# nvaccess/NVSpeechPlayer

Measured on AMD Instinct MI355X. Metric: audio samples/sec (whole node) at 22.05 kHz Klatt synth, batch-N utterances, higher is better.
Workload: dtype f64

## Files before the change

nvspeechplayer_amd/csrc/klatt_batchplan.h:

```cpp
#pragma once

#include <stddef.h>
#include <stdint.h>

#include <algorithm>
#include <numeric>
#include <unordered_map>
#include <utility>
#include <vector>

#include "klatt_consts.h"

namespace klatt {


template <class Meta>
inline bool list_length(const Meta* meta, long long n, uint32_t& length)
{
    unsigned long long len = 0;
    for (long long k = 0; k < n; ++k) {
        const unsigned long long m = meta[k].minSamples, f = meta[k].fadeSamples;
        len += std::max(m, f + 1) + 1;
    }
    length = len >= 0xFFFFFFFFull ? 0u : (uint32_t)len;
    return len < 0xFFFFFFFFull;
}

template <class Meta>
inline unsigned long long list_timing(const Meta* meta, long long n)
{
    unsigned long long h = 0x9E3779B97F4A7C15ull ^ (unsigned long long)n;
    for (long long k = 0; k < n; ++k) {
        h ^= ((unsigned long long)meta[k].minSamples << 32) ^ meta[k].fadeSamples ^ ((unsigned long long)(meta[k].flags & FRAME_NULL) << 63);
        h *= 0xFF51AFD7ED558CCDull; h ^= h >> 29;
    }
    return h;
}

template <class Meta, class Facts>
inline void classify_list(const Meta* meta, const Facts* facts, long long n, uint32_t& flags, unsigned char& shape)
{
    uint32_t fl = 0;
    for (long long k = 0; k < n; ++k)
        if (!(meta[k].flags & FRAME_NULL)) fl |= facts[k].flags;
    const bool finite = !(fl & FACT_NONFINITE), needsNoise = (fl & FACT_NOISE) || !finite;
    flags = (needsNoise ? UTT_NEEDS_NOISE : (!(fl & FACT_NASAL) ? UTT_NO_NASAL : 0u)) | (fl & kUttPresent);
    shape = finite ? (!(fl & FACT_UNBOUNDED) ? 3 : 1) : 0;
}


struct ListTable {
    std::vector<uint32_t> lens;
    std::vector<unsigned long long> timing;
    std::vector<uint32_t> flags;
    std::vector<unsigned char> shape;
    std::vector<uint32_t> weight;
    long long size() const { return (long long)flags.size(); }
    unsigned long long run_key(long long l) const { return timing[(size_t)l] ^ ((unsigned long long)lens[(size_t)l] * 0x9E3779B97F4A7C15ull); }
};

struct RouteOptions {
    int tracks = 1, direct = 1, layout = -1;
    bool fast = false;
    bool sortByLength = true;
    bool noTracks = false;
    int cus = 256;
    long long nFrames = 0;
    bool want_tracks() const { return tracks && !noTracks; }
    bool want_direct() const { return direct && layout != 0 && nFrames > 0 && nFrames < 0xFFFFFFFFll; }
    bool plans() const { return (want_tracks() || want_direct()) && nFrames > 0; }
};

constexpr long long kRunMin = 32;

struct RunShare {
    long long total = 0, inRuns = 0;
    std::unordered_map<unsigned long long, long long> runOf;
};
template <class Pred>
inline RunShare run_share(const ListTable& lists, Pred pred)
{
    RunShare s;
    for (long long l = 0; l < lists.size(); ++l)
        if (pred(l)) { s.total += lists.weight[(size_t)l]; s.runOf[lists.run_key(l)] += lists.weight[(size_t)l]; }
    for (const auto& kv : s.runOf) if (kv.second >= kRunMin) s.inRuns += kv.second;
    return s;
}

using Rerouted = std::vector<std::pair<long long, uint32_t>>;
inline Rerouted reroute_lonely_quiet(ListTable& lists, const RouteOptions& o)
{
    Rerouted rerouted;
    if (!o.plans() || o.layout != -1) return rerouted;
    auto quiet = [&](long long l) { return !(lists.flags[(size_t)l] & UTT_NEEDS_NOISE); };
    const RunShare runs = run_share(lists, quiet);
    if (runs.runOf.size() <= 1) return rerouted;
    for (long long l = 0; l < lists.size(); ++l)
        if (quiet(l) && runs.runOf.at(lists.run_key(l)) < kRunMin) {
            rerouted.emplace_back(l, lists.flags[(size_t)l]);
            lists.flags[(size_t)l] = (lists.flags[(size_t)l] | UTT_NEEDS_NOISE) & ~UTT_NO_NASAL;
        }
    return rerouted;
}

inline std::vector<unsigned char> eligible_lists(const ListTable& lists, const RouteOptions& o)
{
    std::vector<unsigned char> eligible;
    if (!o.plans()) return eligible;
    eligible.assign((size_t)lists.size(), 0);
    for (long long l = 0; l < lists.size(); ++l)
        if ((lists.flags[(size_t)l] & UTT_NEEDS_NOISE) && lists.weight[(size_t)l]) eligible[(size_t)l] = lists.shape[(size_t)l];
    return eligible;
}

inline bool tracks_pay(const ListTable& lists, const unsigned char* eligible, const unsigned char* tracked, unsigned long long trackBytes, const RouteOptions& o)
{
    if (!(o.want_direct() && o.direct == 1 && o.fast && trackBytes > (128ull << 20))) return true;
    long long direct = 0;
    const RunShare runs = run_share(lists, [&](long long l) { return tracked[l] != 0; });
    for (long long l = 0; l < lists.size(); ++l)
        if (tracked[l] && (eligible[l] & 2)) direct += lists.weight[(size_t)l];
    const long long groups = (runs.total + kLanes - 1) / kLanes;
    return !(o.sortByLength && runs.inRuns * 2 <= runs.total && direct == runs.total && groups > o.cus);
}

inline void mark_tracked(ListTable& lists, const unsigned char* tracked, const uint32_t* kinds)
{
    for (long long l = 0; l < lists.size(); ++l)
        if (tracked[l]) lists.flags[(size_t)l] |= UTT_TRACKED | (kinds[l] << kUttKindShift);
}

inline bool route_direct(ListTable& lists, const unsigned char* eligible, const RouteOptions& o)
{
    auto candidate = [&](long long l) { return (eligible[l] & 2) && !(lists.flags[(size_t)l] & UTT_TRACKED); };
    const RunShare runs = run_share(lists, candidate);
    const bool aligned = o.sortByLength && runs.inRuns * 2 > runs.total;
    const bool take = o.direct == 1 ? (!aligned || o.fast) : true;
    if (take)
        for (long long l = 0; l < lists.size(); ++l)
// ... 61 lines not shown
            if (order[(size_t)(w + i)] == kNoUtt) { order[(size_t)(w + i)] = live[(size_t)next]; next = (next + 1) % nLive; }
    }
}

template <class FlagsOf>
inline LanePacking pack_lanes(long long nUtt, FlagsOf flagsOf, const uint32_t* lens, const unsigned long long* timing, bool sortByLength, int width = kLanes)
{
    LanePacking p;
    std::vector<uint32_t>& order = p.order;
    order.resize((size_t)nUtt);
    std::iota(order.begin(), order.end(), 0u);
    auto quietEnd = std::stable_partition(order.begin(), order.end(), [&](uint32_t x) { return !(flagsOf(x) & UTT_NEEDS_NOISE); });
    p.nQuiet = quietEnd - order.begin();
    auto noNasalEnd = std::stable_partition(order.begin(), quietEnd, [&](uint32_t x) { return (flagsOf(x) & UTT_NO_NASAL) != 0; });
    p.nNoNasal = noNasalEnd - order.begin();
    auto trackedEnd = std::stable_partition(quietEnd, order.end(), [&](uint32_t x) { return (flagsOf(x) & UTT_TRACKED) != 0; });
    p.nTrackedUtt = trackedEnd - quietEnd;
    p.nTracked = p.nTrackedUtt;
    auto directEnd = std::stable_partition(trackedEnd, order.end(), [&](uint32_t x) { return (flagsOf(x) & UTT_DIRECT) != 0; });
    p.nDirectSlots = directEnd - trackedEnd;
    const bool untrackedFollow = directEnd != order.end();
    if (sortByLength) {
        auto before = [&](uint32_t x, uint32_t y) { return lens[x] != lens[y] ? lens[x] > lens[y] : timing[x] < timing[y]; };
        std::stable_sort(order.begin(), noNasalEnd, before);
        std::stable_sort(noNasalEnd, quietEnd, before);
        std::stable_sort(quietEnd, trackedEnd, before);
        std::stable_sort(trackedEnd, directEnd, before);
        std::stable_sort(directEnd, order.end(), before);
        const uint32_t* const o = order.data();
        const size_t q = (size_t)p.nQuiet, t = q + (size_t)p.nTrackedUtt, d = t + (size_t)p.nDirectSlots;
        std::vector<uint32_t> tracked, direct(o + t, o + d), untracked;
        pad_runs(o + q, o + t, lens, timing, width, tracked);
        if (!tracked.empty() && t != order.size()) tracked.insert(tracked.end(), lanes_to_boundary(tracked.size(), width), kNoUtt);
        if (!direct.empty() && untrackedFollow) direct.insert(direct.end(), lanes_to_boundary(direct.size(), width), kNoUtt);
        pad_runs(o + d, o + order.size(), lens, timing, width, untracked);
        p.nTracked = (long long)tracked.size();
        p.nDirectSlots = (long long)direct.size();
        order.resize(q);
        order.insert(order.end(), tracked.begin(), tracked.end());
        order.insert(order.end(), direct.begin(), direct.end());
        order.insert(order.end(), untracked.begin(), untracked.end());
    } else if (p.nDirectSlots > 0 && (untrackedFollow || p.nTrackedUtt > 0)) {
        const size_t padT = p.nTrackedUtt > 0 ? lanes_to_boundary((size_t)p.nTrackedUtt, width) : 0;
        order.insert(order.begin() + p.nQuiet + p.nTrackedUtt, padT, kNoUtt);
        p.nTracked = p.nTrackedUtt + (long long)padT;
        if (untrackedFollow) {
            const size_t padD = lanes_to_boundary((size_t)p.nDirectSlots, width);
            order.insert(order.begin() + p.nQuiet + p.nTracked + p.nDirectSlots, padD, kNoUtt);
            p.nDirectSlots += (long long)padD;
        }
    }
    p.nNoNasalSlots = p.nNoNasal + fill_tail(order, 0, p.nNoNasal, width);
    p.nQuietSlots = p.nQuiet + (p.nNoNasalSlots - p.nNoNasal);
    p.nQuietSlots += fill_tail(order, p.nNoNasalSlots, p.nQuietSlots, width);
    const long long noisy = (long long)order.size() - p.nQuietSlots;
    if (noisy % width != 0) {
        const long long ext = width - noisy % width;
        const long long untracked = noisy - p.nTracked - p.nDirectSlots;
        if (untracked <= 0) { if (p.nDirectSlots > 0) p.nDirectSlots += ext; else p.nTracked += ext; }
        order.insert(order.end(), (size_t)ext, kNoUtt);
    }
    fill_sparse_wavefronts(order, p.nQuietSlots, width);
    return p;
}

template <class FlagsOf>
inline void dead_wave_counts(const uint32_t* order, long long first, long long n, FlagsOf flagsOf, int built, long long counts[3], int width = kLanes)
{
    counts[0] = counts[1] = counts[2] = 0;
    for (long long w = first; w < first + n; w += width) {
        uint32_t present = 0;
        bool any = false;
        for (long long s = w; s < std::min(w + width, first + n); ++s)
            if (order[s] != kNoUtt) { present |= flagsOf(order[s]); any = true; }
        if (!any) continue;
        const bool noTurb = !(present & UTT_TURBULENCE), noAsp = noTurb && !(present & UTT_ASPIRATION);
        const int body = ((built & 4) && noAsp) ? 2 : (((built & 2) && noTurb) ? 1 : 0);
        counts[0] += ((built & 1) && !(present & UTT_PARALLEL1)) ? 1 : 0;
        counts[1] += body >= 1 ? 1 : 0;
        counts[2] += body >= 2 ? 1 : 0;
    }
}

}
```

nvspeechplayer_amd/csrc/klatt_consts.h:

```cpp
#pragma once

#include <stdint.h>

namespace klatt {

constexpr int kLanes = 64;

constexpr uint32_t FRAME_NULL = 1u;
constexpr uint32_t UTT_NEEDS_NOISE = 1u;
constexpr uint32_t UTT_NO_NASAL = 2u;
constexpr uint32_t UTT_TRACKED = 4u;
constexpr uint32_t UTT_DIRECT = 8u;
constexpr uint32_t UTT_TURBULENCE = 16u;
constexpr uint32_t UTT_ASPIRATION = 32u;
constexpr uint32_t UTT_PARALLEL1 = 64u;
constexpr uint32_t kUttPresent = UTT_TURBULENCE | UTT_ASPIRATION | UTT_PARALLEL1;
constexpr int kUttKindShift = 8;

constexpr uint32_t FACT_NOISE = 1u;
constexpr uint32_t FACT_NONFINITE = 2u;
constexpr uint32_t FACT_NASAL = 4u;
constexpr uint32_t FACT_UNBOUNDED = 8u;
constexpr uint32_t FACT_TURBULENCE = UTT_TURBULENCE;
constexpr uint32_t FACT_ASPIRATION = UTT_ASPIRATION;
constexpr uint32_t FACT_PARALLEL1 = UTT_PARALLEL1;

}
```

nvspeechplayer_amd/csrc/klatt_device.h:

```cpp
#pragma once

#include <hip/hip_runtime.h>
#include <stdint.h>
#include <type_traits>

#include "klatt_consts.h"
#include "klatt_layout.h"
#include "klatt_math.h"

namespace klatt {

constexpr int kTile = 32;
constexpr int kTileStride = kTile * 2 + 8;
constexpr int kSlots = 45;
constexpr int kBlock = 16;
constexpr int kStateDoubles = 240;

constexpr int MODE_EXACT = 0;
constexpr int MODE_FAST = 1;

constexpr int kTrackStages = 4;
#ifndef KLATT_FLAT_LAYOUT
#define KLATT_FLAT_LAYOUT 2
#endif
__host__ __device__ constexpr uint32_t track_stage_kinds(int s)
{
    return KLATT_FLAT_LAYOUT == 2 ? (s == 0 ? 0xF04003u : s == 1 ? 0x0000FCu : s == 2 ? 0x01B000u : 0x0E0F00u)
                                  : (s == 0 ? 0xF00000u : s == 1 ? 0x00403Fu : s == 2 ? 0x01B0C0u : 0x0E0F00u);
}
__host__ __device__ constexpr uint32_t track_stage_entries(int s)
{
    return KLATT_FLAT_LAYOUT == 2 ? (s == 0 ? 8u : s == 1 ? 6u : s == 2 ? 4u : 7u) : (s == 0 ? 4u : s == 1 ? 8u : s == 2 ? 6u : 7u);
}
constexpr int kTrackAntiStage = KLATT_FLAT_LAYOUT == 2 ? 0 : 1;
__host__ __device__ inline uint32_t track_stage_slots(uint32_t mask, int s) { return (uint32_t)__builtin_popcount(mask & track_stage_kinds(s)) + (s == kTrackAntiStage ? (mask & 1u) : 0u); }
__host__ __device__ inline uint32_t track_part(uint32_t mask, uint32_t F, int s)
{
    uint32_t at = 0;
    for (int k = 0; k < s; ++k) at += track_stage_entries(k) + (F - 1u) * track_stage_slots(mask, k);
    return at;
}

struct DirectHdr {
    uint32_t fadeSamples;
    uint32_t span;
    uint32_t bits;
    uint32_t pad;
};
constexpr uint32_t kDirectBwShift = 8, kDirectClsShift = 14, kDirectAllBits = 0x3FFFFFFu;
constexpr int kDirectStages = 8;
#ifndef KLATT_DIRECT_FAST_LAYOUT
#define KLATT_DIRECT_FAST_LAYOUT 1
#endif
__host__ __device__ constexpr int direct_layout(int mode) { return mode == MODE_FAST ? KLATT_DIRECT_FAST_LAYOUT : 0; }
__host__ __device__ constexpr int direct_stage_res(int s, int L = 0)
{
    return L == 1 ? (s < 2 ? 0 : (s == 3 || s == 4) ? 3 : 2) : (s == 0 ? 0 : 2);
}
__host__ __device__ constexpr int direct_stage_gains(int s, int L = 0)
{
    return L == 1 ? (s == 0 ? 1 : s == 1 ? 3 : s == 2 ? 1 : s == 5 ? 2 : s == 6 ? 1 : s == 7 ? 2 : 0)
                  : (s == 0 ? 4 : s == 1 ? 1 : s == 5 ? 2 : s == 6 ? 1 : s == 7 ? 2 : 0);
}
__host__ __device__ constexpr int direct_stage_entries(int s, int L = 0) { return 4 * direct_stage_res(s, L) + 3 * direct_stage_gains(s, L); }
__host__ __device__ constexpr int direct_stage_first(int s, int L = 0) { int at = 0; for (int k = 0; k < s; ++k) at += direct_stage_entries(k, L); return at; }
constexpr int kDirectEntries = direct_stage_first(kDirectStages);
static_assert(direct_stage_first(kDirectStages, 1) == kDirectEntries, "both layouts hold the same kinds");
__host__ __device__ constexpr int direct_stage_kind(int s, int e, int L = 0)
{
    constexpr int k0[kDirectStages][4] = {{20, 21, 22, 23}, {0, 1, 14, -1}, {2, 3, -1, -1}, {4, 5, -1, -1}, {6, 7, -1, -1}, {8, 9, 17, 18}, {10, 11, 19, -1}, {12, 13, 15, 16}};
    constexpr int k1[kDirectStages][4] = {{20, -1, -1, -1}, {21, 22, 23, -1}, {0, 1, 14, -1}, {2, 3, 4, -1}, {5, 6, 7, -1}, {8, 9, 17, 18}, {10, 11, 19, -1}, {12, 13, 15, 16}};
    return L == 1 ? k1[s][e] : k0[s][e];
}

struct KernelArgs {
    const DirectHdr* directHdr;
    const double2* directRec;
    const uint32_t* directFirst;
    uint32_t nDirect;
    const FlatRef* flatRef;
    const SourceRef* sourceRef;
    uint32_t trackBytes;
    const double2* track;
    const double* frames;
    const FrameMeta* meta;
    const UttDesc* utt;
    const uint32_t* order;
    int16_t* pcm;
    UttResult* result;
    double* state;
    double* const* statePtrs;
    const uint32_t* control;
    long long nSlots;
    uint32_t maxSamples;
    uint32_t ringMask;
    int sampleRate;
    double sampleRateF;
    double invSampleRate;
    double negPiOverSr;
    double twoPiOverSr;
    unsigned long long* debug;
    uint32_t* deadWaves;
    uint32_t deadTerms;
};

__device__ constexpr int kResF[kNumRes] = {13, 14, 12, 11, 10, 9, 8, 7, 25, 26, 27, 28, 29, 30};
__device__ constexpr int kResB[kNumRes] = {21, 22, 20, 19, 18, 17, 16, 15, 31, 32, 33, 34, 35, 36};
constexpr int kNumHot = 17;
__device__ constexpr int kHot[kNumHot] = {1, 2, 3, 4, 5, 6, 23, 24, 37, 38, 39, 40, 41, 42, 43, 44, 45};


__device__ __forceinline__ double div_by(double x, double b, double y)
{
    double q = x * y;
    double r = __builtin_fma(-b, q, x);
    return __builtin_fma(r, y, q);
}

__device__ __forceinline__ double frac_toward_zero(double x) { return x - __builtin_trunc(x); }

__device__ __forceinline__ double fade_value(double from, double to, double ratio)
{
    double v = from + ((to - from) * ratio);
    return (to != to) ? from : v;
}

__device__ __forceinline__ uint32_t mix32(uint32_t x)
{
    x ^= x >> 16; x *= 0x7FEB352Du; x ^= x >> 15; x *= 0x846CA68Bu; x ^= x >> 16;
    return x;
}
__device__ __forceinline__ uint32_t noise_key(uint32_t seed) { return mix32(seed ^ 0x9E3779B9u); }
__device__ __forceinline__ uint32_t noise_inc(uint32_t seed) { return (mix32(seed + 0x85EBCA6Bu) << 1) | 1u; }
constexpr uint32_t kNoiseA = 1664525u;
constexpr uint32_t kNoiseA2 = kNoiseA * kNoiseA;
__device__ __forceinline__ uint32_t noise_inc2(uint32_t inc) { return (kNoiseA + 1u) * inc; }
__device__ __forceinline__ uint32_t noise_step(uint32_t s, uint32_t inc) { return s * kNoiseA + inc; }
__device__ __forceinline__ uint32_t noise_step2(uint32_t s, uint32_t inc2) { return s * kNoiseA2 + inc2; }
__device__ __forceinline__ uint32_t noise_first(uint32_t key, uint32_t inc) { return noise_step(key, inc); }
__device__ __forceinline__ double noise_uniform(uint32_t s)
{
    const double r = (double)(s >> 1);
    return __builtin_fma(r, 0x1.00000002p-31, r * 0x1p-93);
}

template <int MODE>
__device__ __forceinline__ double dot3(double a, double x, double b, double y, double c, double z)
{
    if (MODE == MODE_FAST) return __builtin_fma(c, z, __builtin_fma(b, y, a * x));
    return a * x + b * y + c * z;
}

#ifdef KLATT_SIGNAL_F32
typedef float sig_t;
#else
typedef double sig_t;
#endif
template <int MODE>
__device__ __forceinline__ float dot3(float a, float x, float b, float y, float c, float z)
{
    return __builtin_fmaf(c, z, __builtin_fmaf(b, y, a * x));
}
__device__ __forceinline__ float fade_value(float from, float to, float ratio)
{
    float v = from + ((to - from) * ratio);
    return (to != to) ? from : v;
}

struct Coef { double a, b, c; };
enum { COEF_UNREDUCED = 0, COEF_QUADRANT_M1 = 1, COEF_UNKNOWN = 2 };
#ifndef KLATT_COLD_CALL
#define KLATT_COLD_CALL 2
#endif
struct RadCos { double rad, cs; };
#if KLATT_COLD_CALL
__device__ __attribute__((noinline)) RadCos exp_cos_reduced(double ex, double th)
{
    RadCos o;
#if KLATT_COLD_CALL == 1
    if (__builtin_fabs(ex) <= 700.0 && __builtin_fabs(th) <= 1.0e4) { o.rad = fast_exp(ex); o.cs = fast_cos(th); }
    else
#endif
    { o.rad = exp(ex); o.cs = cos(th); }
    return o;
}
#endif
// ... 451 lines not shown
```

nvspeechplayer_amd/csrc/klatt_engine.hip:

```cpp
#include "klatt_device.h"
#include "klatt_systolic.h"
#include "klatt_lanepipe.h"
#include "klatt_tracks.h"
#include "klatt_direct.h"
#include "klatt_plan.h"
#include "klatt_timeline.h"
#include "klatt_align.h"
#include "klatt_source.h"
#include "klatt_response.h"
#include "klatt_stems.h"
#include "klatt_spectrum.h"
#include "klatt_resample.h"
#include "klatt_convolve.h"
#include "klatt_filter.h"
#include "klatt_codec.h"
#include "klatt_lpc.h"
#include "klatt_pitch.h"
#include "klatt_tempo.h"
#include "klatt_mix.h"
#include "klatt_export.h"
#include "klatt_batchplan.h"
#include "klatt_hostpool.h"
#include "klatt_trackplan.h"
#include "klatt_live.h"
// ... 417 lines not shown
    switch (mode) {
    case MODE_EXACT: rc = go(klatt_lanepipe<MODE_EXACT, CH, WPS>); break;
    case MODE_FAST: rc = go(klatt_lanepipe<MODE_FAST, CH, WPS>); break;
    default: set_error("unknown arithmetic mode %d", mode); return -1;
    }
    if (rc) return rc;
    HIP_TRY(hipGetLastError());
    return 0;
}

#ifndef KLATT_NOISY_CH
#define KLATT_NOISY_CH 8
#endif
struct GroupPlan { bool systolic; int chunk; };
GroupPlan plan_group(int layout, bool noisy, long long nUttBatch, long long nNoisyBatch, int cus)
{
    const long long groups = (nUttBatch + kLanes - 1) / kLanes + 1;
    GroupPlan p;
    p.systolic = layout != 0;
    (void)nNoisyBatch;
    p.chunk = noisy ? (groups <= cus ? 16 : 8)
                    : (groups <= cus ? 32 : 16);
    return p;
}

template <bool STREAM, bool NOISE>
int launch(const KernelArgs& a, int mode, long long nWaves, hipStream_t stream)
{
    if (nWaves <= 0) return 0;
    if (nWaves > 0x7FFFFFFF) { set_error("too many wavefronts: %lld", nWaves); return -1; }
    constexpr int ldsBytes = LdsLayout<STREAM>::kBytes;
    auto go = [&](auto kernel) -> int {
        if (ensure_lds_limit(reinterpret_cast<const void*>(kernel), ldsBytes)) return -1;
        hipLaunchKernelGGL(kernel, dim3((unsigned)nWaves), dim3(kLanes), ldsBytes, stream, a);
        return 0;
    };
    int rc;
    switch (mode) {
    case MODE_EXACT: rc = go(klatt_synthesize<MODE_EXACT, STREAM, NOISE>); break;
    case MODE_FAST: rc = go(klatt_synthesize<MODE_FAST, STREAM, NOISE>); break;
    default:
        set_error("unknown arithmetic mode %d", mode);
        return -1;
    }
    if (rc) return rc;
    HIP_TRY(hipGetLastError());
    return 0;
}

int pick_device(int device)
{
    int n = 0;
    hipError_t e = hipGetDeviceCount(&n);
    if (e != hipSuccess || n <= 0) {
        set_error_code(SPEECHPLAYER_ERR_NO_DEVICE);
        set_error("no HIP device available (%s); this engine has no CPU path", e == hipSuccess ? "count 0" : hipGetErrorString(e));
        return -1;
    }
    if (device < 0) {
        const char* env = getenv("SPEECHPLAYER_DEVICE");
        if (env) device = atoi(env);
        else if (hipGetDevice(&device) != hipSuccess) device = 0;
    }
    if (device >= n) { set_error("device %d out of range (%d devices)", device, n); return -1; }
    return device;
}

struct Batch {
    int sampleRate = 0;
    int device = 0;
    int mode = MODE_EXACT;
    int sortByLength = 1;
    int layout = -1;
    int cus = 256;
    hipStream_t stream = nullptr;
    int tracks = 1;
    long long trackBudgetMB = 4096;
    hipStream_t side[6] = {nullptr, nullptr, nullptr, nullptr, nullptr, nullptr};
    hipEvent_t forkEvent = nullptr, join[6] = {nullptr, nullptr, nullptr, nullptr, nullptr, nullptr};
    int quietLast = 1;
    int deadTerms = 1;
    DeviceBuffer<uint32_t> dDeadWaves;
    long long planDeadWaves[3] = {0, 0, 0};
    long long nUtt = 0, nFrames = 0, nSlots = 0;
    long long nLists = 0, nFramesSpoken = 0;
    std::vector<long long> uttFrameStart;
    std::vector<uint32_t> uttFrames;
    bool launched = false;
    long long nQuiet = 0;
    long long nTracked = 0;
    long long nTrackedUtt = 0;
    long long nJobs = 0, trackEntries = 0;
    int directLean = -1;
    bool directAligned = false;
    int direct = 1;
    long long nDirect = 0;
    long long nDirectUtt = 0, nDirectFrames = 0;
    long long nNoNasal = 0;
    long long nNoNasalUtt = 0;
    long long totalSamples = 0, poolSamples = 0;
    std::vector<uint32_t> lens;
    std::vector<uint32_t> uttSeed;
    std::vector<long long> outStart;
    std::vector<UttResult> results;
    bool resultsFresh = false;
    DeviceBuffer<double> dFrames;
    DeviceBuffer<FrameMeta> dMeta;
    DeviceBuffer<UttDesc> dUtt;
    DeviceBuffer<uint32_t> dOrder;
    DeviceBuffer<int16_t> dPcm;
    DeviceBuffer<UttResult> dResult;
    DeviceBuffer<FlatRef> dFlatRef;
    DeviceBuffer<SourceRef> dSourceRef;
    DeviceBuffer<TrackJob> dJobs;
    DeviceBuffer<double> dShapes;
    DeviceBuffer<double2> dTrack;
    DeviceBuffer<DirectJob> dDirectJobs;
    DeviceBuffer<uint32_t> dDirectFirst;
    DeviceBuffer<DirectHdr> dDirectHdr;
    DeviceBuffer<double2> dDirectRec;
    DeviceBuffer<unsigned long long> dDebug;
    DeviceBuffer<float> dFloat;
    DeviceBuffer<unsigned long long> dDigest;
    PinnedPair bounce;
    DeviceBuffer<FrameRecord> dRecords;
    DeviceBuffer<double> dShapeTable;
    DeviceBuffer<uint32_t> dRep;
    DeviceBuffer<unsigned long long> dMismatch;
    DeviceBuffer<FrameFacts> dFacts;
    PinnedBlock hFacts;
    DeviceBuffer<int16_t> dDense;
    DeviceBuffer<long long> dDenseStart;
    std::vector<long long> denseStart;
    hipStream_t copyStream = nullptr;
    hipEvent_t denseReady = nullptr, copyDone = nullptr;
    bool copyPending = false;
    bool floatFresh = false;
    hipEvent_t inputReady = nullptr;
    DeviceBuffer<long long> dShapeIdx;
    DeviceBuffer<double> dShapeRows;
    hipEvent_t pcmReady = nullptr;
    struct ExportSlot { PinnedBlock host; DeviceBuffer<unsigned char> dev; hipEvent_t done = nullptr; bool used = false; };
    static constexpr int kExportSlots = 16;
    ExportSlot exportSlot[kExportSlots];
    unsigned exportNext = 0;
    struct SharedTable {
        hipEvent_t done = nullptr;
        bool used = false;
        int wait(hipStream_t st) { if (used) HIP_TRY(hipStreamWaitEvent(st, done, 0)); return 0; }
        int mark(hipStream_t st) { HIP_TRY(hipEventRecord(done, st)); used = true; return 0; }
    };
    std::vector<uint32_t> uttList;
    DeviceBuffer<long long> dListStart;
    DeviceBuffer<TimelineReq> dTimeline;
    hipEvent_t setDone = nullptr, setCopied = nullptr, timelineReady = nullptr;
    bool timelineFresh = false;
    ExportSlot trackSlot[kExportSlots];
    unsigned trackNext = 0;
    DeviceBuffer<double> dPitch;
    SharedTable pitchOrder;
    long long pitchBudgetMB = 256;
    DeviceBuffer<FrameLabel> dLabels;
    DeviceBuffer<uint32_t> dUnitFirst;
    std::vector<uint32_t> listUnits;
    bool hasLabels = false;
    DeviceBuffer<double> dSource;
// ... 181 lines not shown
constexpr bool kTimingOnlyBuild = false;
#endif
bool refuse_timing_only(const char* what)
{
    if (!kTimingOnlyBuild || getenv("SPEECHPLAYER_ALLOW_TIMING_ONLY_PCM")) return false;
    set_error_code(SPEECHPLAYER_ERR_ARGUMENT);
    set_error("%s: this library was built with a timing-only experiment switch; its PCM is not valid", what);
    return true;
}

long long tracked_count(const Batch* b) { return (b->tracks && b->layout != 0) ? b->nTracked : 0; }
long long direct_count(const Batch* b) { return b->nDirect; }
bool direct_lean(const Batch* b, long long nGroups)
{
    if (b->directLean >= 0) return b->directLean != 0;
    if (b->directAligned) return false;
    return b->mode == MODE_FAST ? true : nGroups > 2ll * b->cus;
}

int batch_launch(Batch* b)
{
    KernelArgs a = base_args(b->sampleRate);
    a.frames = b->dFrames.ptr; a.meta = b->dMeta.ptr; a.utt = b->dUtt.ptr;
    a.pcm = b->dPcm.ptr; a.result = b->dResult.ptr; a.state = nullptr; a.control = nullptr;
    if (wait_exports(b)) return -1;
    b->resultsFresh = false;
    b->floatFresh = false;
    b->launched = true;
#ifdef KLATT_STAMPS
    if (b->dDebug.reserve((size_t)(b->nSlots / kLpUPG + 2) * 32 * 2)) return -1;
    HIP_TRY(hipMemsetAsync(b->dDebug.ptr, 0, b->dDebug.cap * 8, b->stream));
    a.debug = b->dDebug.ptr;
#endif
    const long long nLp = lanepipe_count(b);
    const bool laneKernel = b->layout == 0;
    const long long nTr = tracked_count(b);
    const long long nDir = direct_count(b);
    const long long nNoisyHead = b->nTracked - nTr;
    const long long nNoisy = b->nSlots - b->nQuiet - b->nTracked - nDir;
    const long long nNn = laneKernel ? 0 : b->nNoNasal - nLp;
    const long long nQ = b->nQuiet - nLp - nNn;
    const int parts = (nLp > 0) + (nNn > 0) + (nQ > 0) + (nNoisy > 0) + (nNoisyHead > 0) + (nTr > 0) + (nDir > 0);
    const bool fork = parts > 1;
    if (fork) HIP_TRY(hipEventRecord(b->forkEvent, b->stream));
    int sideUsed = 0, seen = 0;
    auto next_stream = [&](bool = false) -> hipStream_t {
        if (!fork || ++seen == parts) return b->stream;
        hipStream_t st = b->side[sideUsed++];
        (void)hipStreamWaitEvent(st, b->forkEvent, 0);
        return st;
    };
    const GroupPlan plq = plan_group(b->layout, false, b->nSlots, nNoisy, b->cus);
    auto launch_quiet = [&]() -> int {
    if (nLp > 0) {
        hipStream_t st = next_stream(true);
        a.order = b->dOrder.ptr; a.nSlots = nLp;
        const long long g = (nLp + kLpUPG - 1) / kLpUPG;
        if (g <= b->cus ? launch_lanepipe<KLATT_LP_CH, 1>(a, b->mode, g, st) : launch_lanepipe<16, 2>(a, b->mode, g, st)) return -1;
    }
    if (nNn > 0) {
        hipStream_t st = next_stream(true);
        a.order = b->dOrder.ptr + nLp; a.nSlots = nNn;
        const long long g = (nNn + kLanes - 1) / kLanes;
        if (plq.chunk == 32 ? launch_systolic<false, 32, 1, false>(a, b->mode, g, st) : launch_systolic<false, 16, 2, false>(a, b->mode, g, st)) return -1;
    }
    if (nQ > 0) {
        hipStream_t st = next_stream(true);
        a.order = b->dOrder.ptr + nLp + nNn; a.nSlots = nQ;
        const long long g = (nQ + kLanes - 1) / kLanes;
        if (plq.systolic ? (plq.chunk == 32 ? launch_systolic<false, 32>(a, b->mode, g, st) : launch_systolic<false, 16>(a, b->mode, g, st))
                         : launch<false, false>(a, b->mode, g, st)) return -1;
    }
        return 0;
    };
    const bool quietLast = b->quietLast && (nTr > 0 || nDir > 0) && nNoisy == 0 && nNoisyHead == 0;
    if (!quietLast && launch_quiet()) return -1;
    if (nTr > 0) {
        hipStream_t st = next_stream();
        TrackArgs t;
        t.jobs = b->dJobs.ptr; t.nJobs = b->nJobs; t.shapes = b->dShapes.ptr; t.track = b->dTrack.ptr;
        t.negPiOverSr = a.negPiOverSr; t.twoPiOverSr = a.twoPiOverSr;
        const long long tg = b->nJobs;
        if (tg > 0x7FFFFFFF) { set_error("too many tracks: %lld", b->nJobs); return -1; }
        if (b->dDeadWaves.reserve(3)) return -1;
        HIP_TRY(hipMemsetAsync(b->dDeadWaves.ptr, 0, 3 * sizeof(uint32_t), st));
        hipLaunchKernelGGL(klatt_tracks, dim3((unsigned)tg), dim3(kLanes * kTrackWaves), 0, st, t);
        HIP_TRY(hipGetLastError());
        a.order = b->dOrder.ptr + b->nQuiet; a.nSlots = nTr;
        a.flatRef = b->dFlatRef.ptr; a.sourceRef = b->dSourceRef.ptr; a.track = b->dTrack.ptr;
        a.trackBytes = (uint32_t)std::min<unsigned long long>(((unsigned long long)b->trackEntries + kTrackPad) * sizeof(double2), 0xFFFFFFFFull);
        a.deadWaves = b->dDeadWaves.ptr; a.deadTerms = b->deadTerms ? kUttPresent : 0u;
        const GroupPlan pl = plan_group(b->layout, true, b->nSlots, nTr + nNoisy, b->cus);
        const long long g = (nTr + kLanes - 1) / kLanes;
        if (pl.chunk == 8 ? launch_systolic<true, KLATT_FLAT_CH, KLATT_FLAT_WPS, true, false, true>(a, b->mode, g, st)
                          : launch_systolic<true, 16, 1, true, false, true>(a, b->mode, g, st)) return -1;
        a.flatRef = nullptr; a.sourceRef = nullptr; a.track = nullptr; a.deadWaves = nullptr; a.deadTerms = 0u;
    }
    if (nDir > 0) {
        hipStream_t st = next_stream();
        SeedArgs sa;
        sa.jobs = b->dDirectJobs.ptr; sa.nJobs = (uint32_t)b->nDirectFrames; sa.frames = b->dFrames.ptr; sa.meta = b->dMeta.ptr;
        sa.hdr = b->dDirectHdr.ptr; sa.rec = b->dDirectRec.ptr; sa.negPiOverSr = a.negPiOverSr; sa.twoPiOverSr = a.twoPiOverSr;
        const dim3 sg((unsigned)((b->nDirectFrames + 255) / 256), (unsigned)kDirectStages);
        constexpr int kSeedLds = 14 * 257 * (int)sizeof(double2);
        if (b->mode == MODE_FAST) hipLaunchKernelGGL(klatt_seeds<MODE_FAST>, sg, dim3(256), kSeedLds, st, sa);
        else hipLaunchKernelGGL(klatt_seeds<MODE_EXACT>, sg, dim3(256), kSeedLds, st, sa);
        HIP_TRY(hipGetLastError());
        a.order = b->dOrder.ptr + b->nQuiet + b->nTracked; a.nSlots = nDir;
        a.directHdr = b->dDirectHdr.ptr; a.directRec = b->dDirectRec.ptr; a.directFirst = b->dDirectFirst.ptr; a.nDirect = (uint32_t)b->nDirectFrames;
        a.sourceRef = b->dSourceRef.ptr;
        const long long g = (nDir + kLanes - 1) / kLanes;
        if (launch_direct(a, b->mode, direct_lean(b, g), g, st)) return -1;
        a.directHdr = nullptr; a.directRec = nullptr; a.directFirst = nullptr; a.nDirect = 0; a.sourceRef = nullptr;
    }
    for (int half = 0; half < 2; ++half) {
        const long long n = half ? nNoisy : nNoisyHead;
        if (n <= 0) continue;
        hipStream_t st = next_stream();
        a.order = b->dOrder.ptr + b->nQuiet + (half ? b->nTracked + nDir : 0); a.nSlots = n;
        const GroupPlan pl = plan_group(b->layout, true, b->nSlots, nTr + nNoisy + nNoisyHead, b->cus);
        const long long g = (n + kLanes - 1) / kLanes;
        if (pl.systolic ? (pl.chunk == 8 ? launch_systolic<true, KLATT_NOISY_CH, 2>(a, b->mode, g, st) : launch_systolic<true, 16>(a, b->mode, g, st))
                        : launch<false, true>(a, b->mode, g, st)) return -1;
    }
    if (quietLast && launch_quiet()) return -1;
    for (int i = 0; i < sideUsed; ++i) {
        HIP_TRY(hipEventRecord(b->join[i], b->side[i]));
        HIP_TRY(hipStreamWaitEvent(b->stream, b->join[i], 0));
    }
    return 0;
}

constexpr size_t kLogEntries = 40960;
constexpr size_t kLogEager = 2560;

struct LogEntry {
    double p[kNumParams];
    FrameMeta meta;
    uint32_t target;
    uint32_t pad;
};
static_assert(sizeof(LogEntry) == 400, "LogEntry layout");

__global__ void __launch_bounds__(256) live_scatter(const LogEntry* __restrict__ log, uint32_t n, double* __restrict__ ringFrames,
                                                    FrameMeta* __restrict__ ringMeta)
{
    const uint32_t e = blockIdx.x * 4u + (threadIdx.x >> 6), j = threadIdx.x & 63u;
    if (e >= n) return;
    const uint32_t at = log[e].target;
    if (at == kNoTarget) return;
    if (j < (uint32_t)kNumParams) ringFrames[(size_t)at * kNumParams + j] = log[e].p[j];
    else if (j == (uint32_t)kNumParams) ringMeta[at] = log[e].meta;
}

struct LivePlace {
    FrameMeta meta;
    long long row;
    uint32_t target;
    uint32_t pad;
};
static_assert(sizeof(LivePlace) == 32, "LivePlace layout");

__global__ void __launch_bounds__(256) live_place(const double* __restrict__ frames, const LivePlace* __restrict__ place, long long n,
                                                  double* __restrict__ ringFrames, FrameMeta* __restrict__ ringMeta)
{
    const uint32_t j = threadIdx.x & 63u;
    const long long step = (long long)gridDim.x * 4;
    for (long long e = (long long)blockIdx.x * 4 + (threadIdx.x >> 6); e < n; e += step) {
        const LivePlace p = place[e];
        if (j < (uint32_t)kNumParams) ringFrames[(size_t)p.target * kNumParams + j] = p.row < 0 ? 0.0 : frames[p.row * kNumParams + j];
        else if (j == (uint32_t)kNumParams) ringMeta[p.target] = p.meta;
    }
}

struct Stream {
    int sampleRate = 0;
    int device = 0;
    int mode = MODE_EXACT;
    uint32_t seed = 0;
// ... 858 lines not shown
    begin_call();
    QueueCall q;
    q.what = "speechPlayer_queueFramesManyDevice"; q.handles = handles; q.n = nHandles; q.frameStart = frameStart; q.frames = deviceFrames;
    q.onDevice = true; q.minDur = minFrameDuration; q.fadeDur = fadeDuration; q.userIndex = userIndex; q.isNull = isNull; q.purge = purge;
    q.readyStream = static_cast<hipStream_t>(readyStream);
    return queue_frames(q);
}

int speechPlayer_handleDevice(speechPlayer_handle_t handle)
{
    begin_call();
    Stream* s = lookup(handle);
    if (!s) { set_error("speechPlayer_handleDevice: invalid handle"); return -1; }
    return s->device;
}

speechPlayer_batch_t speechPlayer_batch_create(int sampleRate, int device)
{
    begin_call();
    int dev = pick_device(device);
    if (dev < 0) return nullptr;
    Batch* b = new Batch;
    b->sampleRate = sampleRate;
    b->device = dev;
    { hipDeviceProp_t prop; if (hipGetDeviceProperties(&prop, dev) == hipSuccess && prop.multiProcessorCount > 0) b->cus = prop.multiProcessorCount; }
    bool ok = hipSetDevice(dev) == hipSuccess && hipStreamCreateWithFlags(&b->stream, hipStreamNonBlocking) == hipSuccess &&
              hipEventCreateWithFlags(&b->forkEvent, hipEventDisableTiming) == hipSuccess &&
              hipStreamCreateWithFlags(&b->copyStream, hipStreamNonBlocking) == hipSuccess &&
              hipEventCreateWithFlags(&b->denseReady, hipEventDisableTiming) == hipSuccess &&
              hipEventCreateWithFlags(&b->copyDone, hipEventDisableTiming) == hipSuccess &&
              hipEventCreateWithFlags(&b->inputReady, hipEventDisableTiming) == hipSuccess &&
              hipEventCreateWithFlags(&b->pcmReady, hipEventDisableTiming) == hipSuccess;
    for (auto& s : b->exportSlot) ok = ok && hipEventCreateWithFlags(&s.done, hipEventDisableTiming) == hipSuccess;
    for (auto& s : b->trackSlot) ok = ok && hipEventCreateWithFlags(&s.done, hipEventDisableTiming) == hipSuccess;
    for (hipEvent_t* e : {&b->setDone, &b->setCopied, &b->timelineReady, &b->pitchOrder.done, &b->sourceOrder.done, &b->resampleOrder.done, &b->bankOrder.done}) ok = ok && hipEventCreateWithFlags(e, hipEventDisableTiming) == hipSuccess;
    { const char* e = getenv("SPEECHPLAYER_TRACKS"); if (e) b->tracks = atoi(e) ? 1 : 0; }
    { const char* e = getenv("SPEECHPLAYER_DIRECT"); if (e) b->direct = std::min(2, std::max(0, atoi(e))); }
    { const char* e = getenv("SPEECHPLAYER_DIRECT_LEAN"); if (e) b->directLean = std::min(1, std::max(-1, atoi(e))); }
    for (int i = 0; i < 6 && ok; ++i)
        ok = hipStreamCreateWithFlags(&b->side[i], hipStreamNonBlocking) == hipSuccess &&
             hipEventCreateWithFlags(&b->join[i], hipEventDisableTiming) == hipSuccess;
    { const char* e = getenv("SPEECHPLAYER_QUIET_LAST"); if (e) b->quietLast = atoi(e) ? 1 : 0; }
    if (!ok) {
        set_error("cannot create a stream on device %d", dev);
        speechPlayer_batch_destroy(b);
        return nullptr;
    }
    return b;
}

void speechPlayer_batch_destroy(speechPlayer_batch_t batch)
{
    Batch* b = static_cast<Batch*>(batch);
    if (!b) return;
    (void)hipSetDevice(b->device);
    (void)sync_exports(b);
    for (auto& s : b->exportSlot) {
        if (s.done) (void)hipEventDestroy(s.done);
        s.host.release(); s.dev.release();
    }
    (void)settle_track_exports(b, true);
    for (auto& s : b->trackSlot) {
        if (s.done) (void)hipEventDestroy(s.done);
        s.host.release(); s.dev.release();
    }
    for (hipEvent_t e : {b->setDone, b->setCopied, b->timelineReady, b->pitchOrder.done, b->sourceOrder.done, b->resampleOrder.done, b->bankOrder.done}) if (e) (void)hipEventDestroy(e);
    b->dListStart.release(); b->dTimeline.release(); b->dPitch.release(); b->dLabels.release(); b->dUnitFirst.release();
    b->dSource.release(); b->dEpochs.release(); b->dEpochCount.release(); b->dResample.release(); b->dBank.release();
    if (b->inputReady) (void)hipEventDestroy(b->inputReady);
    if (b->pcmReady) (void)hipEventDestroy(b->pcmReady);
    b->dShapeIdx.release(); b->dShapeRows.release();
    if (b->stream) { (void)hipStreamSynchronize(b->stream); (void)hipStreamDestroy(b->stream); }
    for (int i = 0; i < 6; ++i) {
        if (b->side[i]) { (void)hipStreamSynchronize(b->side[i]); (void)hipStreamDestroy(b->side[i]); }
        if (b->join[i]) (void)hipEventDestroy(b->join[i]);
    }
    if (b->forkEvent) (void)hipEventDestroy(b->forkEvent);
    if (b->copyStream) { (void)hipStreamSynchronize(b->copyStream); (void)hipStreamDestroy(b->copyStream); }
    if (b->denseReady) (void)hipEventDestroy(b->denseReady);
    if (b->copyDone) (void)hipEventDestroy(b->copyDone);
    b->dDense.release(); b->dDenseStart.release(); b->dFacts.release(); b->hFacts.release();
    b->dRecords.release(); b->dShapeTable.release(); b->dRep.release(); b->dMismatch.release();
    b->dFrames.release(); b->dMeta.release(); b->dUtt.release(); b->dOrder.release(); b->dPcm.release(); b->dResult.release();
    b->dFloat.release(); b->dDebug.release(); b->dDigest.release(); b->bounce.release(); b->dDeadWaves.release();
    b->dFlatRef.release(); b->dSourceRef.release(); b->dJobs.release(); b->dShapes.release(); b->dTrack.release();
    b->dDirectJobs.release(); b->dDirectFirst.release(); b->dDirectHdr.release(); b->dDirectRec.release();
    delete b;
}

int speechPlayer_batch_setOption(speechPlayer_batch_t batch, const char* name, int value)
{
    begin_call();
    Batch* b = static_cast<Batch*>(batch);
    if (!b || !name) return -1;
    if (!strcmp(name, "mode")) {
        if (value != MODE_EXACT && value != MODE_FAST) { set_error("mode %d not available", value); return -1; }
        b->mode = value;
        return 0;
    }
    if (!strcmp(name, "sort")) { b->sortByLength = value ? 1 : 0; return 0; }
    if (!strcmp(name, "quiet_last")) { b->quietLast = value ? 1 : 0; return 0; }
    if (!strcmp(name, "layout")) { b->layout = value < 0 ? -1 : (value > 2 ? 1 : value); return 0; }
    if (!strcmp(name, "tracks")) { b->tracks = value ? 1 : 0; return 0; }
    if (!strcmp(name, "dead_terms")) { b->deadTerms = value ? 1 : 0; return 0; }
    if (!strcmp(name, "track_budget_mb")) { b->trackBudgetMB = value < 0 ? 0 : value; return 0; }
    if (!strcmp(name, "direct")) { b->direct = value < 0 ? 0 : (value > 2 ? 2 : value); return 0; }
    if (!strcmp(name, "direct_lean")) { b->directLean = value < 0 ? -1 : (value ? 1 : 0); return 0; }
    if (!strcmp(name, "pitch_table_mb")) { b->pitchBudgetMB = value < 1 ? 1 : value; return 0; }
    if (!strcmp(name, "source_table_mb")) { b->sourceBudgetMB = value < 1 ? 1 : value; return 0; }
    if (!strcmp(name, "source_lane_lists")) { b->sourceLaneLists = value < 1 ? 1 : value; return 0; }
    set_error("unknown option %s", name);
    return -1;
}

struct SetInput {
    long long nLists = 0;
    const long long* listStart = nullptr;
    const speechPlayer_frame_t* frames = nullptr;
    const unsigned int* minDur = nullptr;
    const unsigned int* fadeDur = nullptr;
    const int* userIndex = nullptr;
    const unsigned char* isNull = nullptr;
    const speechPlayer_frameRecord_t* records = nullptr;
    long long nShapes = 0;
    const speechPlayer_frame_t* shapes = nullptr;
    long long nUtt = 0;
    const unsigned int* listOf = nullptr;
    const unsigned int* seeds = nullptr;
    const double* deviceFrames = nullptr;
    hipStream_t readyStream = nullptr;
    const speechPlayer_frameLabel_t* labels = nullptr;
    bool noTracks = false;
};
static_assert(sizeof(speechPlayer_frameRecord_t) == sizeof(FrameRecord), "record layout");
static_assert(sizeof(speechPlayer_frameLabel_t) == sizeof(FrameLabel), "label layout");
static_assert(SPEECHPLAYER_LABEL_GAP == kLabelGap && SPEECHPLAYER_LABEL_PUFF == kLabelPuff && SPEECHPLAYER_ALIGN_COLUMNS == kAlignColumns &&
              SPEECHPLAYER_UNIT_COLUMNS == kUnitColumns, "alignment constants");

static void batch_clear(Batch* b)
{
    b->nUtt = 0; b->nFrames = 0; b->nFramesSpoken = 0; b->nLists = 0; b->nSlots = 0; b->nQuiet = 0; b->nNoNasal = 0; b->nNoNasalUtt = 0; b->totalSamples = 0; b->poolSamples = 0;
    b->nTracked = 0; b->nTrackedUtt = 0; b->nJobs = 0; b->trackEntries = 0; b->nDirect = 0; b->nDirectUtt = 0; b->nDirectFrames = 0; b->directAligned = false;
    b->lens.clear(); b->outStart.assign(1, 0); b->results.clear(); b->resultsFresh = false; b->floatFresh = false;
    b->uttFrameStart.clear(); b->uttFrames.clear(); b->uttList.clear(); b->uttSeed.clear(); b->timelineFresh = false; b->epochFresh = false;
    b->hasLabels = false; b->listUnits.clear();
}

static int batch_set(Batch* b, const SetInput& in);

static int batch_set_guarded(const char* what, speechPlayer_batch_t batch, const SetInput& in)
{
    begin_call();
    try {
        return batch_set(static_cast<Batch*>(batch), in);
    } catch (const std::exception& e) {
        set_error("%s: %s", what, e.what());
        return -1;
    }
}

int speechPlayer_batch_setUtterances(speechPlayer_batch_t batch, long long nUtterances, const long long* frameStart,
                                     const speechPlayer_frame_t* frames, const unsigned int* minFrameDuration,
                                     const unsigned int* fadeDuration, const int* userIndex, const unsigned char* isNull,
                                     const unsigned int* noiseSeed)
{
    SetInput in;
    in.nLists = nUtterances; in.listStart = frameStart; in.frames = frames; in.minDur = minFrameDuration; in.fadeDur = fadeDuration;
// ... 84 lines not shown
                                          const unsigned int* noiseSeed)
{
    return batch_set_records(labels ? "setRecordsLabelled" : "setRecords", batch, nShapes, shapes, nLists, listStart, records, labels, nUtterances, listOf, noiseSeed);
}

int speechPlayer_batch_hasLabels(speechPlayer_batch_t batch) { return batch ? (static_cast<Batch*>(batch)->hasLabels ? 1 : 0) : -1; }

static int device_shape_table(Batch* b, long long nL, const long long* listStart, const FrameMeta* meta, const FrameFacts* facts,
                              const unsigned char* eligible, HashMask mask, RawVector<uint32_t>& rowOf, std::vector<long long>& rep, std::vector<double>& rows)
{
    shape_table_rows(nL, listStart, meta, facts, eligible, mask, rowOf, rep);
    const size_t nRows = rep.size();
    rows.assign(nRows * kNumParams, 0.0);
    if (nRows == 0) return 0;
    if (b->dShapeIdx.reserve(nRows) || b->dShapeRows.reserve(nRows * kNumParams)) return -1;
    HIP_TRY(hipMemcpyAsync(b->dShapeIdx.ptr, rep.data(), nRows * sizeof(long long), hipMemcpyHostToDevice, b->copyStream));
    const unsigned grid = (unsigned)std::min<long long>(((long long)nRows * kNumParams + 255) / 256, 1 << 16);
    hipLaunchKernelGGL(klatt_gather_frames, dim3(grid), dim3(256), 0, b->copyStream, b->dFrames.ptr, b->dShapeIdx.ptr, (long long)nRows, b->dShapeRows.ptr);
    HIP_TRY(hipGetLastError());
    HIP_TRY(hipMemcpyAsync(rows.data(), b->dShapeRows.ptr, nRows * kNumParams * sizeof(double), hipMemcpyDeviceToHost, b->copyStream));
    HIP_TRY(hipStreamSynchronize(b->copyStream));
    return 0;
}

struct FirstBad {
    std::atomic<long long> at{-1};
    void mark(long long i) { long long none = -1; at.compare_exchange_strong(none, i); }
    long long get() const { return at.load(); }
};

constexpr long long kScratchKeepFrames = 4000000;
struct SetScratch {
    RawVector<FrameMeta> meta;
    RawVector<FlatRef> flatRef;
    RawVector<DirectJob> directJobs;
    RawVector<FrameFacts> facts;
};
static SetScratch& set_scratch()
{
    static thread_local SetScratch scratch;
    return scratch;
}

struct SetCall {
    Batch* const b;
    const SetInput& in;
    const long long nL, nU;
    const long long* const listStart;
    const bool byRecords, byDevice;
    long long nF = 0;
    const std::chrono::steady_clock::time_point tSet = std::chrono::steady_clock::now();

    SetScratch& scratch = set_scratch();
    struct ScratchRelease {
        SetScratch& s;
        long long nF = 0;
        ~ScratchRelease()
        {
            if (nF > kScratchKeepFrames) {
                RawVector<FrameMeta>().swap(s.meta); RawVector<FlatRef>().swap(s.flatRef); RawVector<FrameFacts>().swap(s.facts);
                RawVector<DirectJob>().swap(s.directJobs);
            }
        }
    } scratchRelease{scratch};
    std::vector<uint32_t> unitFirst, listUnits;
    bool framesPinned = false, earlyStarted = false;
    int earlyRc = 0;
    std::string earlyErr;
    struct CopyGuard { Batch* b; bool armed = false; ~CopyGuard() { if (armed) (void)hipStreamSynchronize(b->copyStream); } } copyGuard{b};
    std::thread early;
    struct JoinEarly { std::thread& t; ~JoinEarly() { if (t.joinable()) t.join(); } } joinEarly{early};
    const FrameFacts* facts = nullptr;
    bool factsOnDevice = false;
    ListTable lists;
    RouteOptions route;
    std::vector<uint32_t> lens;
    std::vector<long long> outStart, denseStart;
    long long total = 0, pool = 0, spoken = 0;
    TrackPlan plan;
    std::vector<uint32_t> directFirst;
    long long nDirectUtt = 0;
    bool directAligned = false;
    std::vector<UttDesc> utt;
    std::vector<long long> uttFrameStart;
    std::vector<uint32_t> uttFrames, uttList, uttSeed;
    LanePacking lanes;
    bool verify = false;
    unsigned long long mismatchAt = ~0ull;

    SetCall(Batch* b_, const SetInput& in_)
        : b(b_), in(in_), nL(in_.nLists), nU(in_.nUtt), listStart(in_.listStart), byRecords(in_.records != nullptr), byDevice(in_.deviceFrames != nullptr) {}
    long long list_of(long long u) const { return in.listOf ? (long long)in.listOf[u] : u; }
    void lap(const char* what) const
    {
        static const bool setTrace = getenv("SPEECHPLAYER_SET_TRACE") != nullptr;
        if (setTrace) fprintf(stderr, "[speechPlayer/set] %s: %.1f ms since the start\n", what, std::chrono::duration<double, std::milli>(std::chrono::steady_clock::now() - tSet).count());
    }
};

static int set_validate(SetCall& c)
{
    const SetInput& in = c.in;
    const long long nL = c.nL, nU = c.nU;
    const long long* const listStart = c.listStart;
    if (listStart[0] != 0) { set_error("set: frameStart[0] must be 0"); return -1; }
    for (long long l = 0; l < nL; ++l)
        if (listStart[l + 1] < listStart[l]) { set_error("set: frameStart not monotone at %lld", l); return -1; }
    const long long nF = c.nF = listStart[nL];
    if (nF > 0 && !c.byRecords && ((!in.frames && !c.byDevice) || !in.minDur || !in.fadeDur)) { set_error("set: bad frame arrays"); return -1; }
    if (in.listOf) {
        FirstBad bad;
        parallel_ranges(nU, 1 << 16, [&](long long a, long long e) {
            for (long long u = a; u < e; ++u) if ((long long)in.listOf[u] >= nL) bad.mark(u);
        });
        if (bad.get() >= 0) { set_error("set: listOf[%lld] is not a list", bad.get()); return -1; }
    }
    if (c.byRecords) {
        FirstBad bad;
        parallel_ranges(nF, 1 << 16, [&](long long a, long long e) {
            for (long long k = a; k < e; ++k)
                if (in.records[k].shape != SPEECHPLAYER_RECORD_SILENCE && (long long)in.records[k].shape >= in.nShapes) bad.mark(k);
        });
        if (bad.get() >= 0) { set_error("setRecords: record %lld names shape %u of %lld", bad.get(), in.records[bad.get()].shape, in.nShapes); return -1; }
    }
    if (in.labels) {
        if (nF >= 0xFFFFFFFFll) { set_error("setRecordsLabelled: too many frames"); return -1; }
        c.unitFirst.resize((size_t)(nF + nL)); c.listUnits.assign((size_t)nL, 0);
        FirstBad bad;
        parallel_ranges(nL, 256, [&](long long la, long long le) {
            for (long long l = la; l < le; ++l) {
                uint32_t* uf = c.unitFirst.data() + listStart[l] + l;
                int units = 0;
                for (long long k = listStart[l]; k < listStart[l + 1]; ++k) {
                    const int u = in.labels[k].unit;
                    if (in.labels[k].phoneme < 0 || (u != units && !(units > 0 && u == units - 1))) { bad.mark(k); break; }
                    if (u == units) uf[units++] = (uint32_t)(k - listStart[l]);
                }
                uf[units] = (uint32_t)(listStart[l + 1] - listStart[l]);
                c.listUnits[(size_t)l] = (uint32_t)units;
            }
        });
        if (bad.get() >= 0) {
            set_error("setRecordsLabelled: label %lld (phoneme %d, unit %d): the units of a list count from 0 and rise by at most one, ids are not negative",
                      bad.get(), in.labels[bad.get()].phoneme, in.labels[bad.get()].unit);
            return -1;
        }
    }
    return 0;
}

static int set_meta_words(SetCall& c)
{
    const SetInput& in = c.in;
    const long long nL = c.nL, nF = c.nF;
    const long long* const listStart = c.listStart;
    c.scratchRelease.nF = nF;
    RawVector<FrameMeta>& meta = c.scratch.meta;
    meta.resize((size_t)nF);
    parallel_ranges(nF, 1 << 16, [&](long long a, long long e) {
        if (c.byRecords)
            for (long long k = a; k < e; ++k) {
                const speechPlayer_frameRecord_t& r = in.records[k];
                meta[k].minSamples = r.minFrameDuration;
                meta[k].fadeSamples = std::max(r.fadeDuration, 1u);
                meta[k].userIndex = r.userIndex;
                meta[k].flags = r.shape == SPEECHPLAYER_RECORD_SILENCE ? FRAME_NULL : 0u;
            }
        else
            for (long long k = a; k < e; ++k) {
                meta[k].minSamples = in.minDur[k];
                meta[k].fadeSamples = std::max(in.fadeDur[k], 1u);
                meta[k].userIndex = in.userIndex ? in.userIndex[k] : -1;
                meta[k].flags = (in.isNull && in.isNull[k]) ? FRAME_NULL : 0u;
            }
    });
    c.lists.lens.assign((size_t)nL, 0);
    FirstBad tooLong;
    parallel_ranges(nL, 4096, [&](long long la, long long le) {
        for (long long l = la; l < le; ++l)
            if (!list_length(meta.data() + listStart[l], listStart[l + 1] - listStart[l], c.lists.lens[(size_t)l])) tooLong.mark(l);
    });
    if (tooLong.get() >= 0) { set_error("utterance (frame list %lld) too long (4294967295 samples or more)", tooLong.get()); return -1; }
    return 0;
}

static int set_start_frames(SetCall& c)
{
    Batch* const b = c.b;
    const SetInput& in = c.in;
    const long long nL = c.nL, nF = c.nF;
    c.framesPinned = !c.byRecords && nF > 0 && is_pinned(in.frames);
    {
        const bool grows = (size_t)nF * kNumParams > b->dFrames.cap || (size_t)nF > b->dMeta.cap || (size_t)nL + 1 > b->dListStart.cap ||
                           (in.labels && ((size_t)nF > b->dLabels.cap || (size_t)(nF + nL) > b->dUnitFirst.cap));
        const bool unordered = !c.byRecords && !c.byDevice && !c.framesPinned;
        if (settle_track_exports(b, grows || unordered)) return -1;
    }
    if (c.byRecords) {
        if (b->dFrames.reserve(std::max<size_t>((size_t)nF * kNumParams, 1)) || b->dMeta.reserve(std::max<size_t>((size_t)nF, 1)) ||
            b->dRecords.reserve(std::max<size_t>((size_t)nF, 1)) || b->dShapeTable.reserve(std::max<size_t>((size_t)in.nShapes * kNumParams, 1))) { batch_clear(b); return -1; }
        batch_clear(b);
        c.copyGuard.armed = true;
        if (in.nShapes) HIP_TRY(hipMemcpyAsync(b->dShapeTable.ptr, in.shapes, (size_t)in.nShapes * sizeof(speechPlayer_frame_t), hipMemcpyHostToDevice, b->copyStream));
        if (nF) {
            HIP_TRY(hipMemcpyAsync(b->dRecords.ptr, in.records, (size_t)nF * sizeof(FrameRecord), hipMemcpyHostToDevice, b->copyStream));
            const unsigned grid = (unsigned)std::min<long long>((nF + 63) / 64, 8192);
            hipLaunchKernelGGL(klatt_expand_frames, dim3(grid), dim3(256), 0, b->copyStream, b->dRecords.ptr, b->dShapeTable.ptr, b->dFrames.ptr, b->dMeta.ptr, nF);
            HIP_TRY(hipGetLastError());
        }
        c.earlyStarted = true;
    } else if (c.byDevice && nF > 0) {
        if (in.readyStream) {
            HIP_TRY(hipEventRecord(b->inputReady, in.readyStream));
            HIP_TRY(hipStreamWaitEvent(b->copyStream, b->inputReady, 0));
        }
        if (b->dFrames.reserve((size_t)nF * kNumParams)) { batch_clear(b); return -1; }
        batch_clear(b);
        c.copyGuard.armed = true;
        HIP_TRY(hipMemcpyAsync(b->dFrames.ptr, in.deviceFrames, (size_t)nF * kNumParams * sizeof(double), hipMemcpyDeviceToDevice, b->copyStream));
        c.earlyStarted = true;
    } else if (nF > 0 && (c.framesPinned || (size_t)nF * kNumParams * sizeof(double) >= (32u << 20))) {
        if (b->dFrames.reserve((size_t)nF * kNumParams)) { batch_clear(b); return -1; }
        batch_clear(b);
        if (c.framesPinned) {
            c.copyGuard.armed = true;
            HIP_TRY(hipMemcpyAsync(b->dFrames.ptr, in.frames, (size_t)nF * kNumParams * sizeof(double), hipMemcpyHostToDevice, b->copyStream));
            c.earlyStarted = true;
        } else
        try {
            c.early = std::thread([&c, frames = in.frames, nF, dev = b->device, dst = b->dFrames.ptr]() {
                hipError_t e = hipSetDevice(dev);
                if (e == hipSuccess) e = hipMemcpy(dst, frames, (size_t)nF * kNumParams * sizeof(double), hipMemcpyHostToDevice);
                if (e != hipSuccess) { c.earlyRc = -1; c.earlyErr = hipGetErrorString(e); }
            });
            c.earlyStarted = true;
        } catch (const std::system_error&) {}
    }
    return 0;
}

static int set_frame_facts(SetCall& c)
{
    Batch* const b = c.b;
    const SetInput& in = c.in;
    const long long nF = c.nF;
    const double maxBwDirect = 690.0 * b->sampleRate / M_PI, maxFDirect = 9900.0 * b->sampleRate / (2.0 * M_PI);
    c.factsOnDevice = (c.framesPinned || c.byDevice) && c.earlyStarted;
    RawVector<FrameFacts>& fv = c.scratch.facts;
    if (c.byRecords) {
        std::vector<uint32_t> shapeFl((size_t)in.nShapes);
        for (long long s = 0; s < in.nShapes; ++s) shapeFl[(size_t)s] = shape_flags(reinterpret_cast<const double*>(in.shapes + s), maxFDirect, maxBwDirect);
        fv.resize((size_t)nF);
        parallel_ranges(nF, 1 << 15, [&](long long a, long long e) {
            for (long long k = a; k < e; ++k) {
                const speechPlayer_frameRecord_t& r = in.records[k];
                FrameFacts f;
                f.h0 = r.shape; f.h1 = ~0ull; f.pad = 0;
                f.flags = r.shape == SPEECHPLAYER_RECORD_SILENCE ? 0u : (shapeFl[r.shape] | pitch_flags(r.voicePitch, r.endVoicePitch));
                fv[k] = f;
            }
        });
        c.facts = fv.data();
    } else if (c.factsOnDevice) {
        if (b->dFacts.reserve((size_t)nF) || b->hFacts.ensure((size_t)nF * sizeof(FrameFacts))) return -1;
        const unsigned grid = (unsigned)std::min<long long>((nF + 255) / 256, 1 << 16);
        hipLaunchKernelGGL(klatt_frame_facts, dim3(grid), dim3(256), 0, b->copyStream, b->dFrames.ptr, b->dFacts.ptr, nF, maxFDirect, maxBwDirect);
        HIP_TRY(hipGetLastError());
        HIP_TRY(hipMemcpyAsync(b->hFacts.ptr, b->dFacts.ptr, (size_t)nF * sizeof(FrameFacts), hipMemcpyDeviceToHost, b->copyStream));
        c.facts = static_cast<const FrameFacts*>(b->hFacts.ptr);
    } else if (nF > 0) {
        fv.resize((size_t)nF);
        parallel_ranges(nF, 1 << 13, [&](long long a, long long e) {
            for (long long k = a; k < e; ++k) fv[k] = frame_facts(reinterpret_cast<const double*>(in.frames + k), maxFDirect, maxBwDirect);
        });
        c.facts = fv.data();
    }
    return 0;
}

static int set_plan(SetCall& c)
{
    Batch* const b = c.b;
    const SetInput& in = c.in;
    const long long nL = c.nL, nU = c.nU, nF = c.nF;
    const long long* const listStart = c.listStart;
    const FrameMeta* const meta = c.scratch.meta.data();
    ListTable& lists = c.lists;
    c.lens.assign((size_t)nU, 0);
    c.outStart.assign((size_t)nU + 1, 0);
    c.denseStart.resize((size_t)nU + 1);
    for (long long u = 0; u < nU; ++u) {
        const long long l = c.list_of(u);
        c.lens[u] = lists.lens[l];
        c.outStart[u] = c.pool;
        c.denseStart[u] = c.total;
        c.total += (long long)c.lens[u];
        c.pool += ((long long)c.lens[u] + kTile - 1) / kTile * kTile;
        c.spoken += listStart[l + 1] - listStart[l];
    }
    c.outStart[nU] = c.pool;
    c.denseStart[nU] = c.total;
    lists.weight.assign((size_t)nL, in.listOf ? 0u : 1u);
    if (in.listOf) for (long long u = 0; u < nU; ++u) ++lists.weight[in.listOf[u]];
    c.lap("meta, lengths, frame facts started");
    lists.timing.resize((size_t)nL);
    parallel_ranges(nL, 4096, [&](long long la, long long le) {
        for (long long l = la; l < le; ++l) lists.timing[l] = list_timing(meta + listStart[l], listStart[l + 1] - listStart[l]);
    });
    if (c.factsOnDevice) HIP_TRY(hipStreamSynchronize(b->copyStream));
    const FrameFacts* const facts = c.facts;
    lists.shape.assign((size_t)nL, 0);
    lists.flags.assign((size_t)nL, 0);
    parallel_ranges(nL, 4096, [&](long long la, long long le) {
        for (long long l = la; l < le; ++l)
            classify_list(meta + listStart[l], facts + listStart[l], listStart[l + 1] - listStart[l], lists.flags[l], lists.shape[l]);
    });
    c.lap("classification");
    RouteOptions& route = c.route;
    route.tracks = b->tracks; route.direct = b->direct; route.layout = b->layout;
    route.fast = b->mode == MODE_FAST; route.sortByLength = b->sortByLength != 0; route.noTracks = in.noTracks;
    route.cus = b->cus; route.nFrames = nF;
    const Rerouted rerouted = reroute_lonely_quiet(lists, route);
    c.lap("timing hashes, quiet runs");
    const std::vector<unsigned char> eligible = eligible_lists(lists, route);
    c.lap("eligibility");
    TrackPlan& plan = c.plan;
    FrameSource source{in.frames, in.records, in.shapes};
    RawVector<uint32_t> rowOf;
    std::vector<long long> shapeRep;
    std::vector<double> shapeRows;
    const bool wantTracks = route.want_tracks() && nF > 0;
    const HashMask hashMask = plan_hash_mask();
    if (wantTracks && c.byDevice) {
        if (device_shape_table(b, nL, listStart, meta, facts, eligible.data(), hashMask, rowOf, shapeRep, shapeRows)) return -1;
        source.shapes = reinterpret_cast<const speechPlayer_frame_t*>(shapeRows.data());
        source.rowOf = rowOf.data();
        c.lap("shape table");
    }
    if (wantTracks) {
        plan_tracks(nL, listStart, source, facts, meta, eligible.data(), track_budget_entries(b->trackBudgetMB), hashMask, plan);
        if (source.rowOf && !plan.rep.empty()) {
            parallel_ranges(nL, 4096, [&](long long la, long long le) {
                for (long long l = la; l < le; ++l) {
                    if (!eligible[l]) continue;
                    for (long long k = listStart[l]; k < listStart[l + 1]; ++k) {
                        if (meta[k].flags & FRAME_NULL) continue;
                        const long long r = shapeRep[rowOf[k]];
                        plan.rep[k] = r == k ? 0xFFFFFFFFu : (uint32_t)r;
                    }
                }
            });
        }
        c.lap("tracks planned");
        if (tracks_pay(lists, eligible.data(), plan.tracked.data(), plan.entries * sizeof(double2), route)) mark_tracked(lists, plan.tracked.data(), plan.kinds.data());
        else { plan.jobs.clear(); plan.entries = 0; plan.tracked.assign((size_t)nL, 0); }
    }
    if (route.want_direct()) c.directAligned = route_direct(lists, eligible.data(), route);
    restore_rerouted(lists, rerouted);
    return 0;
}

static void set_direct_jobs_and_refs(SetCall& c)
{
    const long long nL = c.nL, nU = c.nU, nF = c.nF;
    const long long* const listStart = c.listStart;
    const RawVector<FrameMeta>& meta = c.scratch.meta;
    const TrackPlan& plan = c.plan;
    RawVector<DirectJob>& directJobs = c.scratch.directJobs;
    directJobs.clear();
    if (c.route.want_direct()) {
        std::vector<uint32_t> directFirstL((size_t)nL, 0u);
        for (long long l = 0; l < nL; ++l) {
            if (!(c.lists.flags[l] & UTT_DIRECT)) continue;
            c.nDirectUtt += c.lists.weight[l];
            directFirstL[l] = (uint32_t)directJobs.size();
            walk_fade_ends(listStart[l], listStart[l + 1], meta.data(), directJobs);
        }
        c.directFirst.resize((size_t)nU);
        parallel_ranges(nU, 1 << 16, [&](long long a, long long e) { for (long long u = a; u < e; ++u) c.directFirst[u] = directFirstL[c.list_of(u)]; });
    }
    RawVector<FlatRef>& flatRef = c.scratch.flatRef;
    if (!plan.jobs.empty()) {
        flatRef.resize((size_t)nF);
        parallel_ranges(nF, 1 << 16, [&](long long ka, long long ke) {
        for (long long k = ka; k < ke; ++k) {
            const unsigned long long m = meta[k].minSamples, f = meta[k].fadeSamples;
            flatRef[k] = FlatRef{(uint32_t)plan.ref[k].off, plan.ref[k].mask, meta[k].fadeSamples, (uint32_t)std::min<unsigned long long>(std::max(m, f + 1) + 1, 0xFFFFFFFFull)};
        }
        });
    }
    c.lap("direct jobs, flat / source references");
}

static void set_lanes(SetCall& c)
{
    const SetInput& in = c.in;
    const long long nU = c.nU;
    const long long* const listStart = c.listStart;
    c.utt.resize((size_t)nU); c.uttFrameStart.resize((size_t)nU); c.uttFrames.resize((size_t)nU); c.uttList.resize((size_t)nU); c.uttSeed.resize((size_t)nU);
    parallel_ranges(nU, 1 << 15, [&](long long a, long long e) {
        for (long long u = a; u < e; ++u) {
            const long long l = c.list_of(u);
            UttDesc d;
            d.frameStart = listStart[l];
            d.outStart = c.outStart[u];
            d.nFrames = (uint32_t)(listStart[l + 1] - listStart[l]);
            d.seed = in.seeds ? in.seeds[u] : (uint32_t)u;
            d.flags = c.lists.flags[l];
            d.length = c.lists.lens[l];
            c.utt[u] = d;
            c.uttFrameStart[u] = d.frameStart; c.uttFrames[u] = d.nFrames; c.uttList[u] = (uint32_t)l; c.uttSeed[u] = d.seed;
        }
    });
    std::vector<unsigned long long> timing;
    if (in.listOf) { timing.resize((size_t)nU); for (long long u = 0; u < nU; ++u) timing[u] = c.lists.timing[in.listOf[u]]; }
    else timing.swap(c.lists.timing);
    c.lanes = pack_lanes(nU, [&](uint32_t u) { return c.utt[u].flags; }, c.lens.data(), timing.data(), c.b->sortByLength != 0);
    c.lap("lane packing");
}

static int set_upload(SetCall& c)
{
    Batch* const b = c.b;
    const SetInput& in = c.in;
    const long long nL = c.nL, nU = c.nU, nF = c.nF, pool = c.pool, nSlotsAll = (long long)c.lanes.order.size();
    const long long nTrackedUtt = c.lanes.nTrackedUtt, nDirectUtt = c.nDirectUtt;
    const TrackPlan& plan = c.plan;
    const RawVector<DirectJob>& directJobs = c.scratch.directJobs;
    if ((size_t)pool > b->dPcm.cap && sync_exports(b)) return -1;
    if (b->dFrames.reserve(std::max<size_t>((size_t)nF * kNumParams, 1)) || b->dMeta.reserve(std::max<size_t>(nF, 1)) ||
        b->dUtt.reserve(std::max<size_t>(nU, 1)) || b->dOrder.reserve(std::max<size_t>(nSlotsAll, 1)) ||
        b->dResult.reserve(std::max<size_t>(nU, 1)) || b->dPcm.reserve(std::max<size_t>(pool, 1)) || b->dListStart.reserve((size_t)nL + 1))
        return -1;
    HIP_TRY(hipMemcpyAsync(b->dListStart.ptr, c.listStart, ((size_t)nL + 1) * sizeof(long long), hipMemcpyHostToDevice, b->stream));
    if (nTrackedUtt > 0) {
        if (b->dFlatRef.reserve((size_t)nF) || b->dJobs.reserve(plan.jobs.size()) || b->dShapes.reserve(plan.shapes.size()) ||
            b->dTrack.reserve((size_t)plan.entries + kTrackPad)) return -1;
        HIP_TRY(hipMemcpyAsync(b->dShapes.ptr, plan.shapes.data(), plan.shapes.size() * sizeof(double), hipMemcpyHostToDevice, b->stream));
        HIP_TRY(hipMemcpyAsync(b->dFlatRef.ptr, c.scratch.flatRef.data(), (size_t)nF * sizeof(FlatRef), hipMemcpyHostToDevice, b->stream));
        HIP_TRY(hipMemcpyAsync(b->dJobs.ptr, plan.jobs.data(), plan.jobs.size() * sizeof(TrackJob), hipMemcpyHostToDevice, b->stream));
    }
    if (nTrackedUtt > 0 || nDirectUtt > 0) {
        if (b->dSourceRef.reserve((size_t)nF)) return -1;
    }
    if (nDirectUtt > 0) {
        const size_t nD = directJobs.size();
        if (b->dDirectJobs.reserve(nD) || b->dDirectFirst.reserve((size_t)nU) || b->dDirectHdr.reserve((size_t)kDirectStages * nD) ||
            b->dDirectRec.reserve((size_t)kDirectEntries * nD)) return -1;
        HIP_TRY(hipMemcpyAsync(b->dDirectJobs.ptr, directJobs.data(), nD * sizeof(DirectJob), hipMemcpyHostToDevice, b->stream));
        HIP_TRY(hipMemcpyAsync(b->dDirectFirst.ptr, c.directFirst.data(), (size_t)nU * sizeof(uint32_t), hipMemcpyHostToDevice, b->stream));
    }
    if (nF) {
        if (!c.earlyStarted) HIP_TRY(hipMemcpyAsync(b->dFrames.ptr, in.frames, (size_t)nF * kNumParams * sizeof(double), hipMemcpyHostToDevice, b->stream));
        if (!c.byRecords) HIP_TRY(hipMemcpyAsync(b->dMeta.ptr, c.scratch.meta.data(), (size_t)nF * sizeof(FrameMeta), hipMemcpyHostToDevice, b->stream));
    }
    if (nU) {
        HIP_TRY(hipMemcpyAsync(b->dUtt.ptr, c.utt.data(), (size_t)nU * sizeof(UttDesc), hipMemcpyHostToDevice, b->stream));
        HIP_TRY(hipMemcpyAsync(b->dOrder.ptr, c.lanes.order.data(), (size_t)nSlotsAll * sizeof(uint32_t), hipMemcpyHostToDevice, b->stream));
        HIP_TRY(hipMemsetAsync(b->dResult.ptr, 0, (size_t)nU * sizeof(UttResult), b->stream));
        if (b->dDenseStart.reserve((size_t)nU + 1)) return -1;
        HIP_TRY(hipMemcpyAsync(b->dDenseStart.ptr, c.denseStart.data(), ((size_t)nU + 1) * sizeof(long long), hipMemcpyHostToDevice, b->stream));
    }
    if (c.verify) {
        if (b->dRep.reserve((size_t)nF) || b->dMismatch.reserve(1)) return -1;
        HIP_TRY(hipMemcpyAsync(b->dRep.ptr, plan.rep.data(), (size_t)nF * sizeof(uint32_t), hipMemcpyHostToDevice, b->stream));
        HIP_TRY(hipMemsetAsync(b->dMismatch.ptr, 0xFF, sizeof(unsigned long long), b->stream));
    }
    if (in.labels) {
        if (b->dLabels.reserve(std::max<size_t>((size_t)nF, 1)) || b->dUnitFirst.reserve(std::max<size_t>((size_t)(nF + nL), 1))) return -1;
        c.copyGuard.armed = true;
        if (nF) HIP_TRY(hipMemcpyAsync(b->dLabels.ptr, in.labels, (size_t)nF * sizeof(FrameLabel), hipMemcpyHostToDevice, b->copyStream));
        if (nF + nL) HIP_TRY(hipMemcpyAsync(b->dUnitFirst.ptr, c.unitFirst.data(), (size_t)(nF + nL) * sizeof(uint32_t), hipMemcpyHostToDevice, b->copyStream));
    }
    HIP_TRY(hipStreamSynchronize(b->stream));
    if (c.copyGuard.armed) { HIP_TRY(hipStreamSynchronize(b->copyStream)); c.copyGuard.armed = false; }
    if (c.early.joinable()) c.early.join();
    if (c.earlyRc) { set_error_code(SPEECHPLAYER_ERR_HIP); set_error("set: uploading the frames failed: %s", c.earlyErr.c_str()); return -1; }
    const unsigned grid = (unsigned)std::min<long long>((nF + 255) / 256, 1 << 16);
    if (c.verify) {
        hipLaunchKernelGGL(klatt_verify_shared, dim3(grid), dim3(256), 0, b->stream, b->dFrames.ptr, b->dRep.ptr, nF, b->dMismatch.ptr);
        HIP_TRY(hipGetLastError());
        HIP_TRY(hipMemcpyAsync(&c.mismatchAt, b->dMismatch.ptr, sizeof c.mismatchAt, hipMemcpyDeviceToHost, b->stream));
    }
    if (nTrackedUtt > 0 || nDirectUtt > 0) {
        hipLaunchKernelGGL(klatt_source_refs, dim3(grid), dim3(256), 0, b->stream, b->dFrames.ptr, b->dMeta.ptr, b->dSourceRef.ptr, nF);
        HIP_TRY(hipGetLastError());
    }
    if (c.verify || nTrackedUtt > 0 || nDirectUtt > 0) HIP_TRY(hipStreamSynchronize(b->stream));
    return 0;
}

static int set_commit(SetCall& c)
{
    Batch* const b = c.b;
    const LanePacking& lanes = c.lanes;
    b->hasLabels = c.in.labels != nullptr;
    b->listUnits.swap(c.listUnits);
    b->nUtt = c.nU; b->nFrames = c.nF; b->nFramesSpoken = c.spoken; b->nLists = c.nL; b->nSlots = (long long)lanes.order.size();
    b->nNoNasalUtt = lanes.nNoNasal;
    b->nQuiet = lanes.nQuietSlots; b->nNoNasal = lanes.nNoNasalSlots;
    b->nTracked = lanes.nTrackedUtt > 0 ? lanes.nTracked : 0; b->nTrackedUtt = lanes.nTrackedUtt;
    dead_wave_counts(lanes.order.data(), lanes.nQuietSlots, b->nTracked, [&](uint32_t u) { return c.utt[u].flags; }, KLATT_DEAD_TERMS, b->planDeadWaves);
    b->nJobs = lanes.nTrackedUtt > 0 ? (long long)c.plan.jobs.size() : 0; b->trackEntries = lanes.nTrackedUtt > 0 ? (long long)c.plan.entries : 0;
    b->nDirect = c.nDirectUtt > 0 ? lanes.nDirectSlots : 0; b->nDirectUtt = c.nDirectUtt; b->nDirectFrames = (long long)c.scratch.directJobs.size();
    b->directAligned = c.nDirectUtt > 0 && c.directAligned;
    b->totalSamples = c.total; b->poolSamples = c.pool;
    b->lens.swap(c.lens); b->outStart.swap(c.outStart); b->denseStart.swap(c.denseStart);
    b->uttFrameStart.swap(c.uttFrameStart); b->uttFrames.swap(c.uttFrames); b->uttList.swap(c.uttList); b->uttSeed.swap(c.uttSeed);
    b->timelineFresh = false; b->epochFresh = false;
    HIP_TRY(hipEventRecord(b->setDone, b->stream));
    HIP_TRY(hipEventRecord(b->setCopied, b->copyStream));
    b->results.clear();
    b->resultsFresh = false;
    b->floatFresh = false;
    b->launched = false;
    return 0;
}

static int batch_set(Batch* b, const SetInput& in)
{
    if (!b || in.nLists < 0 || in.nUtt < 0 || !in.listStart) { set_error("set: bad arguments"); return -1; }
    if (in.nUtt >= 0xFFFFFFFFll || in.nLists >= 0xFFFFFFFFll) { set_error("set: too many utterances"); return -1; }
    if (!in.listOf && in.nUtt != in.nLists) { set_error("set: %lld utterances for %lld lists and no listOf", in.nUtt, in.nLists); return -1; }
    SetCall c(b, in);
    HIP_TRY(hipSetDevice(b->device));
    if (set_validate(c) || set_meta_words(c)) return -1;
    if (set_start_frames(c) || set_frame_facts(c) || set_plan(c)) return -1;
    set_direct_jobs_and_refs(c);
    set_lanes(c);
    c.verify = !c.byRecords && c.lanes.nTrackedUtt > 0 && !c.plan.rep.empty();
    if (set_upload(c)) {
        batch_clear(b);
        return -1;
    }
    c.lap("uploads");
    if (c.verify && c.mismatchAt != ~0ull) {
        const unsigned long long k = c.mismatchAt;
        if (c.early.joinable()) c.early.join();
        SetInput again = in;
        again.noTracks = true;
        const uint32_t first = c.plan.rep[(size_t)k];
        const int rc = batch_set(b, again);
        if (rc == 0) {
            set_error("set: frames %llu and %u carry one 128-bit shape hash and different values; the batch runs without tracks", k, first);
            set_error_code(SPEECHPLAYER_OK);
        }
        return rc;
    }
    return set_commit(c);
}

long long speechPlayer_batch_frames(speechPlayer_batch_t batch, long long u, speechPlayer_frame_t* frames, unsigned int* minFrameDuration,
                                    unsigned int* fadeDuration, int* userIndex, unsigned char* isNull, long long capacity)
{
    begin_call();
    Batch* b = static_cast<Batch*>(batch);
    if (!b || u < 0 || u >= b->nUtt) { set_error("batch_frames: no such utterance"); return -1; }
    HIP_TRY(hipSetDevice(b->device));
    const long long n = b->uttFrames[(size_t)u], k0 = b->uttFrameStart[(size_t)u];
    if (n > capacity || n == 0) return n;
    if (frames) HIP_TRY(hipMemcpy(frames, b->dFrames.ptr + k0 * kNumParams, (size_t)n * sizeof(speechPlayer_frame_t), hipMemcpyDeviceToHost));
    if (minFrameDuration || fadeDuration || userIndex || isNull) {
        std::vector<FrameMeta> m((size_t)n);
        HIP_TRY(hipMemcpy(m.data(), b->dMeta.ptr + k0, (size_t)n * sizeof(FrameMeta), hipMemcpyDeviceToHost));
        for (long long k = 0; k < n; ++k) {
            if (minFrameDuration) minFrameDuration[k] = m[(size_t)k].minSamples;
            if (fadeDuration) fadeDuration[k] = m[(size_t)k].fadeSamples;
            if (userIndex) userIndex[k] = m[(size_t)k].userIndex;
            if (isNull) isNull[k] = (m[(size_t)k].flags & FRAME_NULL) ? 1 : 0;
        }
    }
    return n;
}

long long speechPlayer_batch_utteranceSamples(speechPlayer_batch_t batch, long long u)
{
    Batch* b = static_cast<Batch*>(batch);
    if (!b || u < 0 || u >= b->nUtt) return -1;
    return b->lens[u];
}
long long speechPlayer_batch_lengths(speechPlayer_batch_t batch, long long* lengths, long long capacity)
{
    begin_call();
    Batch* b = static_cast<Batch*>(batch);
    if (!b) { set_error("batch_lengths: no batch"); return -1; }
// ... 658 lines not shown
    int n = (int)std::min<size_t>(b->dDebug.cap, (size_t)capacity);
    if (n > 0) HIP_TRY(hipMemcpy(out, b->dDebug.ptr, (size_t)n * 8, hipMemcpyDeviceToHost));
    return n;
}

int speechPlayer_batch_kernelInfo(speechPlayer_batch_t batch, int* info, int nInfo)
{
    begin_call();
    Batch* b = static_cast<Batch*>(batch);
    if (!b || !info || nInfo < 6) return -1;
    HIP_TRY(hipSetDevice(b->device));
    hipFuncAttributes fa;
    const long long nNoisy = b->nSlots - b->nQuiet, nLp = lanepipe_count(b);
    const long long nNn = b->layout == 0 ? 0 : b->nNoNasal - nLp, nQ = b->nQuiet - nLp - nNn;
    const bool lanepipe = nLp > 0 && nLp >= nQ && nLp >= nNoisy && nLp >= nNn;
    const bool nasalFree = !lanepipe && nNn > 0 && nNn >= nQ && nNn >= nNoisy;
    const bool noisy = !lanepipe && !nasalFree && nNoisy >= nQ;
    const GroupPlan pl = plan_group(b->layout, noisy, b->nSlots, nNoisy, b->cus);
    const bool fast = b->mode == MODE_FAST;
    const long long nTr = tracked_count(b);
    const long long nDir = direct_count(b);
    const bool directG = noisy && nDir > 0 && nDir >= nTr && nDir >= nNoisy - nTr - nDir;
    const bool tracked = noisy && !directG && nTr > 0 && nTr >= nNoisy - nTr - nDir;
    const void* fn;
    int ldsBytes = LdsLayout<false>::kBytes, chunk = 0, wavesPerGroup = 1;
    long long groups = (nNn + kLanes - 1) / kLanes + (nQ + kLanes - 1) / kLanes + (nNoisy + kLanes - 1) / kLanes;
    if (nasalFree) {
        if (pl.chunk == 32) { fn = fast ? (const void*)klatt_systolic<MODE_FAST, false, 32, 1, false> : (const void*)klatt_systolic<MODE_EXACT, false, 32, 1, false>; ldsBytes = SysLds<false, 32>::kBytes; }
        else { fn = fast ? (const void*)klatt_systolic<MODE_FAST, false, 16, 2, false> : (const void*)klatt_systolic<MODE_EXACT, false, 16, 2, false>; ldsBytes = SysLds<false, 16>::kBytes; }
        chunk = pl.chunk;
        wavesPerGroup = kStages;
    } else if (lanepipe) {
        const long long g = (nLp + kLpUPG - 1) / kLpUPG;
        if (g <= b->cus) { fn = fast ? (const void*)klatt_lanepipe<MODE_FAST, KLATT_LP_CH, 1> : (const void*)klatt_lanepipe<MODE_EXACT, KLATT_LP_CH, 1>; ldsBytes = LpLds<KLATT_LP_CH>::kBytes; chunk = KLATT_LP_CH; }
        else { fn = fast ? (const void*)klatt_lanepipe<MODE_FAST, 16, 2> : (const void*)klatt_lanepipe<MODE_EXACT, 16, 2>; ldsBytes = LpLds<16>::kBytes; chunk = 16; }
        wavesPerGroup = kStages;
        groups = g;
    } else if (directG) {
        if (direct_lean(b, (nDir + kLanes - 1) / kLanes)) {
            fn = fast ? (const void*)klatt_direct<MODE_FAST, kDirectLeanChunk, 4> : (const void*)klatt_direct<MODE_EXACT, kDirectLeanChunk, 4>;
            ldsBytes = DirectLds<kDirectLeanChunk>::kBytes; chunk = kDirectLeanChunk;
        } else {
            fn = fast ? (const void*)klatt_direct<MODE_FAST, kDirectChunk, 2> : (const void*)klatt_direct<MODE_EXACT, kDirectChunk, 2>;
            ldsBytes = DirectLds<kDirectChunk>::kBytes; chunk = kDirectChunk;
        }
        wavesPerGroup = kDirectStages;
    } else if (tracked) {
        if (pl.chunk == 8) { fn = fast ? (const void*)klatt_systolic<MODE_FAST, true, KLATT_FLAT_CH, KLATT_FLAT_WPS, true, false, true> : (const void*)klatt_systolic<MODE_EXACT, true, KLATT_FLAT_CH, KLATT_FLAT_WPS, true, false, true>; ldsBytes = SysLds<true, KLATT_FLAT_CH, true>::kBytes; chunk = KLATT_FLAT_CH; }
        else { fn = fast ? (const void*)klatt_systolic<MODE_FAST, true, 16, 1, true, false, true> : (const void*)klatt_systolic<MODE_EXACT, true, 16, 1, true, false, true>; ldsBytes = SysLds<true, 16, true>::kBytes; chunk = 16; }
        wavesPerGroup = kStages;
    } else if (pl.systolic) {
        if (noisy && pl.chunk == 8) { fn = fast ? (const void*)klatt_systolic<MODE_FAST, true, 8, 2> : (const void*)klatt_systolic<MODE_EXACT, true, 8, 2>; ldsBytes = SysLds<true, 8>::kBytes; }
        else if (noisy) { fn = fast ? (const void*)klatt_systolic<MODE_FAST, true, 16> : (const void*)klatt_systolic<MODE_EXACT, true, 16>; ldsBytes = SysLds<true, 16>::kBytes; }
        else if (pl.chunk == 32) { fn = fast ? (const void*)klatt_systolic<MODE_FAST, false, 32> : (const void*)klatt_systolic<MODE_EXACT, false, 32>; ldsBytes = SysLds<false, 32>::kBytes; }
        else { fn = fast ? (const void*)klatt_systolic<MODE_FAST, false, 16> : (const void*)klatt_systolic<MODE_EXACT, false, 16>; ldsBytes = SysLds<false, 16>::kBytes; }
        chunk = pl.chunk;
        wavesPerGroup = kStages;
    } else {
        fn = fast ? (noisy ? (const void*)klatt_synthesize<MODE_FAST, false, true> : (const void*)klatt_synthesize<MODE_FAST, false, false>)
                  : (noisy ? (const void*)klatt_synthesize<MODE_EXACT, false, true> : (const void*)klatt_synthesize<MODE_EXACT, false, false>);
    }
    HIP_TRY(hipFuncGetAttributes(&fa, fn));
    hipDeviceProp_t prop;
    HIP_TRY(hipGetDeviceProperties(&prop, b->device));
    info[0] = fa.numRegs;
    info[1] = ldsBytes;
    info[2] = (int)(groups * wavesPerGroup);
    info[3] = prop.multiProcessorCount;
    info[4] = (int)(prop.sharedMemPerMultiprocessor / ldsBytes);
    info[5] = (int)fa.localSizeBytes;
    if (nInfo >= 8) { info[6] = chunk; info[7] = noisy ? 1 : 0; }
    if (nInfo >= 10) { info[8] = lanepipe ? 1 : 0; info[9] = (int)std::min<long long>(nLp > 0 ? b->nNoNasalUtt : 0, 0x7FFFFFFF); }
    if (nInfo >= 12) { info[10] = nasalFree ? 1 : 0; info[11] = (int)std::min<long long>(nNn > 0 ? b->nNoNasalUtt : 0, 0x7FFFFFFF); }
    if (nInfo >= 16) {
        info[12] = (int)std::min<long long>(nTr > 0 ? b->nTrackedUtt : 0, 0x7FFFFFFF); info[13] = (int)std::min<long long>(b->nJobs, 0x7FFFFFFF);
        info[14] = (int)std::min<long long>(b->trackEntries * (long long)sizeof(double2) >> 20, 0x7FFFFFFF); info[15] = tracked ? 1 : 0;
    }
    if (nInfo >= 20) {
        info[16] = (int)std::min<long long>(b->nDirectUtt, 0x7FFFFFFF); info[17] = directG ? 1 : 0;
        info[18] = (int)std::min<long long>(b->nDirectFrames * (long long)(kDirectEntries * sizeof(double2) + kDirectStages * sizeof(DirectHdr)) >> 20, 0x7FFFFFFF);
        info[19] = 0;
    }
    if (nInfo >= 23) {
        uint32_t dead[3] = {0u, 0u, 0u};
        if (b->launched && nTr > 0 && b->dDeadWaves.ptr) {
            HIP_TRY(hipStreamSynchronize(b->stream));
            HIP_TRY(hipMemcpy(dead, b->dDeadWaves.ptr, sizeof dead, hipMemcpyDeviceToHost));
        } else if (nTr > 0 && b->deadTerms) {
            for (int k = 0; k < 3; ++k) dead[k] = (uint32_t)std::min<long long>(b->planDeadWaves[k], 0x7FFFFFFFll);
        }
        for (int k = 0; k < 3; ++k) info[20 + k] = (int)std::min<uint32_t>(dead[k], 0x7FFFFFFFu);
    }
    return 0;
}


static long long plan_tracks_view(long long nUtterances, const long long* frameStart, const speechPlayer_frame_t* frames,
                                  const unsigned int* fadeDuration, const unsigned char* isNull, const unsigned char* eligible,
                                  long long budgetMB, const void* facts24, unsigned long long* trackOff, unsigned int* trackMask, unsigned char* tracked,
                                  unsigned long long* nEntries, long long* collisionAt, unsigned int* kinds = nullptr)
{
    begin_call();
    if (nUtterances < 0 || !frameStart || frameStart[0] != 0) { set_error("planTracks: bad arguments"); return -1; }
    for (long long u = 0; u < nUtterances; ++u)
        if (frameStart[u + 1] < frameStart[u]) { set_error("planTracks: frameStart not monotone at %lld", u); return -1; }
    const long long nF = frameStart[nUtterances];
    if (nF > 0 && (!frames || !fadeDuration)) { set_error("planTracks: bad frame arrays"); return -1; }
    std::vector<FrameMeta> meta((size_t)nF);
    for (long long k = 0; k < nF; ++k) {
        meta[k].minSamples = 0; meta[k].userIndex = -1;
        meta[k].fadeSamples = std::max(fadeDuration[k], 1u);
        meta[k].flags = (isNull && isNull[k]) ? FRAME_NULL : 0u;
    }
    std::vector<unsigned char> all;
    if (!eligible) { all.assign((size_t)nUtterances, 1); eligible = all.data(); }
    TrackPlan plan;
    std::vector<FrameFacts> own;
    const FrameFacts* facts = static_cast<const FrameFacts*>(facts24);
    if (!facts) {
        own.resize((size_t)nF);
        parallel_ranges(nF, 1 << 14, [&](long long a, long long e) { for (long long k = a; k < e; ++k) own[k] = frame_facts(reinterpret_cast<const double*>(frames + k), 1e300, 1e300); });
        facts = own.data();
    }
    plan_tracks(nUtterances, frameStart, FrameSource{frames, nullptr, nullptr}, facts, meta.data(), eligible, track_budget_entries(budgetMB), plan_hash_mask(), plan);
    if (collisionAt) *collisionAt = -1;
    for (long long k = 0; k < nF && !plan.rep.empty(); ++k) {
        const uint32_t r = plan.rep[(size_t)k];
        if (r == 0xFFFFFFFFu || (long long)r == k) continue;
        if (!shape_values_equal(reinterpret_cast<const double*>(frames + k), reinterpret_cast<const double*>(frames + r))) {
            if (collisionAt) *collisionAt = k;
            set_error("planTracks: frames %lld and %u carry one 128-bit shape hash and different values", k, r);
            return -2;
        }
    }
    for (long long k = 0; k < nF; ++k) {
        if (trackOff) trackOff[k] = plan.ref[k].off;
        if (trackMask) trackMask[k] = plan.ref[k].mask;
    }
    for (long long u = 0; u < nUtterances; ++u) {
        if (tracked) tracked[u] = plan.tracked[u];
        if (kinds) kinds[u] = plan.tracked[u] ? plan.kinds[u] : 0u;
        if (!plan.tracked[u])
            for (long long k = frameStart[u]; k < frameStart[u + 1]; ++k) { if (trackOff) trackOff[k] = 0; if (trackMask) trackMask[k] = 0; }
    }
    if (nEntries) *nEntries = plan.entries;
    return (long long)plan.jobs.size();
}

long long speechPlayer_planTracks(long long nUtterances, const long long* frameStart, const speechPlayer_frame_t* frames,
                                  const unsigned int* fadeDuration, const unsigned char* isNull, const unsigned char* eligible,
                                  long long budgetMB, unsigned long long* trackOff, unsigned int* trackMask, unsigned char* tracked,
                                  unsigned long long* nEntries)
{
    try {
        return plan_tracks_view(nUtterances, frameStart, frames, fadeDuration, isNull, eligible, budgetMB, nullptr, trackOff, trackMask, tracked, nEntries, nullptr);
    } catch (const std::exception& e) { set_error("planTracks: %s", e.what()); return -1; }
}

long long speechPlayer_planTracksFacts(long long nUtterances, const long long* frameStart, const speechPlayer_frame_t* frames,
                                       const unsigned int* fadeDuration, const unsigned char* isNull, const unsigned char* eligible,
                                       long long budgetMB, const void* facts24, unsigned long long* trackOff, unsigned int* trackMask,
                                       unsigned char* tracked, unsigned long long* nEntries, long long* collisionAt)
{
    try {
        return plan_tracks_view(nUtterances, frameStart, frames, fadeDuration, isNull, eligible, budgetMB, facts24, trackOff, trackMask, tracked, nEntries, collisionAt);
    } catch (const std::exception& e) { set_error("planTracksFacts: %s", e.what()); return -1; }
}

long long speechPlayer_planTrackKinds(long long nUtterances, const long long* frameStart, const speechPlayer_frame_t* frames,
                                      const unsigned int* fadeDuration, const unsigned char* isNull, const unsigned char* eligible,
                                      long long budgetMB, unsigned long long* trackOff, unsigned int* trackMask, unsigned char* tracked,
                                      unsigned long long* nEntries, unsigned int* kinds)
{
    try {
        return plan_tracks_view(nUtterances, frameStart, frames, fadeDuration, isNull, eligible, budgetMB, nullptr, trackOff, trackMask, tracked, nEntries, nullptr, kinds);
    } catch (const std::exception& e) { set_error("planTrackKinds: %s", e.what()); return -1; }
}

void speechPlayer_internal_parallel(long long n, long long grain, void (*fn)(void* ctx, long long a, long long e), void* ctx)
{
    if (n <= 0 || !fn) return;
    parallel_ranges(n, grain, [&](long long a, long long e) { fn(ctx, a, e); });
}

long long speechPlayer_frameFacts(const speechPlayer_frame_t* frames, long long nFrames, int sampleRate, int onDevice, void* facts24)
{
    begin_call();
    if (nFrames < 0 || (nFrames > 0 && (!frames || !facts24)) || sampleRate <= 0) { set_error("frameFacts: bad arguments"); return -1; }
    const double maxBw = 690.0 * sampleRate / M_PI, maxF = 9900.0 * sampleRate / (2.0 * M_PI);
    FrameFacts* const out = static_cast<FrameFacts*>(facts24);
    constexpr uint32_t kRouting = FACT_NOISE | FACT_NONFINITE | FACT_NASAL | FACT_UNBOUNDED;
    if (!onDevice) {
        parallel_ranges(nFrames, 1 << 13, [&](long long a, long long e) {
            for (long long k = a; k < e; ++k) { out[k] = frame_facts(reinterpret_cast<const double*>(frames + k), maxF, maxBw); out[k].flags &= kRouting; }
        });
        return nFrames;
    }
    if (nFrames == 0) return 0;
    DeviceBuffer<double> dF;
    DeviceBuffer<FrameFacts> dO;
    struct Release { DeviceBuffer<double>& a; DeviceBuffer<FrameFacts>& b; ~Release() { a.release(); b.release(); } } release{dF, dO};
    if (dF.reserve((size_t)nFrames * kNumParams) || dO.reserve((size_t)nFrames)) return -1;
    HIP_TRY(hipMemcpy(dF.ptr, frames, (size_t)nFrames * kNumParams * sizeof(double), hipMemcpyHostToDevice));
    const unsigned grid = (unsigned)std::min<long long>((nFrames + 255) / 256, 1 << 16);
    hipLaunchKernelGGL(klatt_frame_facts, dim3(grid), dim3(256), 0, nullptr, dF.ptr, dO.ptr, nFrames, maxF, maxBw);
    HIP_TRY(hipGetLastError());
    HIP_TRY(hipMemcpy(out, dO.ptr, (size_t)nFrames * sizeof(FrameFacts), hipMemcpyDeviceToHost));
    for (long long k = 0; k < nFrames; ++k) out[k].flags &= kRouting;
    return nFrames;
}

long long speechPlayer_planDirect(long long nUtterances, const long long* frameStart, const unsigned char* isNull,
                                  unsigned int* from, unsigned int* to, unsigned int* flags)
{
    begin_call();
    if (nUtterances < 0 || !frameStart || frameStart[0] != 0) { set_error("planDirect: bad arguments"); return -1; }
    for (long long u = 0; u < nUtterances; ++u)
        if (frameStart[u + 1] < frameStart[u]) { set_error("planDirect: frameStart not monotone at %lld", u); return -1; }
    const long long nF = frameStart[nUtterances];
    if (nF >= 0xFFFFFFFFll) { set_error("planDirect: too many frames"); return -1; }
    std::vector<FrameMeta> meta((size_t)nF);
    for (long long k = 0; k < nF; ++k) { meta[k].minSamples = 0; meta[k].fadeSamples = 1; meta[k].userIndex = -1; meta[k].flags = (isNull && isNull[k]) ? FRAME_NULL : 0u; }
    std::vector<DirectJob> jobs;
    jobs.reserve((size_t)nF);
    for (long long u = 0; u < nUtterances; ++u) walk_fade_ends(frameStart[u], frameStart[u + 1], meta.data(), jobs);
    for (long long k = 0; k < nF; ++k) {
        if (from) from[k] = jobs[(size_t)k].from;
        if (to) to[k] = jobs[(size_t)k].to;
        if (flags) flags[k] = jobs[(size_t)k].flags;
    }
    return nF;
}

long long speechPlayer_planTimeline(long long nUtterances, const long long* frameStart, const unsigned int* minFrameDuration,
                                    const unsigned int* fadeDuration, long long* firstSample, long long* length)
{
    begin_call();
    if (nUtterances < 0 || !frameStart || frameStart[0] != 0) { set_error("planTimeline: bad arguments"); return -1; }
    for (long long u = 0; u < nUtterances; ++u)
        if (frameStart[u + 1] < frameStart[u]) { set_error("planTimeline: frameStart not monotone at %lld", u); return -1; }
    const long long nF = frameStart[nUtterances];
    if (nF > 0 && (!minFrameDuration || !fadeDuration)) { set_error("planTimeline: no durations"); return -1; }
    for (long long u = 0; u < nUtterances; ++u) {
        long long S = 0;
        for (long long k = frameStart[u]; k < frameStart[u + 1]; ++k) {
            if (firstSample) firstSample[k] = S;
            FrameMeta m;
            m.minSamples = minFrameDuration[k]; m.fadeSamples = std::max(fadeDuration[k], 1u);
            S += timeline_span(m);
        }
        if (length) length[u] = S;
    }
    return nF;
}

long long speechPlayer_batch_timeline(speechPlayer_batch_t batch, long long u, long long* firstSample, int* userIndex, long long capacity)
{
    begin_call();
    Batch* b = static_cast<Batch*>(batch);
    if (!b || u < 0 || u >= b->nUtt) { set_error("batch_timeline: no such utterance"); return -1; }
    HIP_TRY(hipSetDevice(b->device));
    const long long n = b->uttFrames[(size_t)u], k0 = b->uttFrameStart[(size_t)u];
    if (n > capacity || (!firstSample && !userIndex)) return n;
    std::vector<FrameMeta> m((size_t)n);
    if (n) HIP_TRY(hipMemcpy(m.data(), b->dMeta.ptr + k0, (size_t)n * sizeof(FrameMeta), hipMemcpyDeviceToHost));
    long long S = 0;
    for (long long k = 0; k < n; ++k) {
        if (firstSample) firstSample[k] = S;
        if (userIndex) userIndex[k] = m[(size_t)k].userIndex;
        S += timeline_span(m[(size_t)k]);
    }
    if (firstSample) firstSample[n] = S;
    return n;
}

static int export_output(Batch* b, const char* what, void* deviceOut, long long elements, size_t elSize)
{
    HIP_TRY(hipSetDevice(b->device));
    if (!deviceOut) { set_error("%s: no output buffer", what); return -1; }
    return device_range(deviceOut, (size_t)elements * elSize, b->device, elSize, what) ? 0 : -1;
}

static int export_synthesised(const Batch* b, const char* what)
{
    if (!b->launched) set_error("%s: the batch has not been synthesised since it was set", what);
    return b->launched ? 0 : -1;
}

static int step_request(const char* what, long long& hop, long long& phase, long long rowStride)
{
    if (hop <= 0 || phase < 0) { set_error("%s: hop %lld, phase %lld", what, hop, phase); return -1; }
// ... 2149 lines not shown
```

nvspeechplayer_amd/csrc/klatt_plan.h:

```cpp
#pragma once

#include <stdint.h>
#include <string.h>

#include "klatt_consts.h"
#include "klatt_layout.h"
#if defined(__HIPCC__)
#include "klatt_device.h"
#endif

namespace klatt {

struct FrameFacts {
    unsigned long long h0, h1;
    uint32_t flags;
    uint32_t pad;
};

KLATT_LAYOUT_HD inline bool fact_finite(double v)
{
    unsigned long long w;
    memcpy(&w, &v, 8);
    return (w & 0x7FF0000000000000ull) != 0x7FF0000000000000ull;
}
KLATT_LAYOUT_HD inline bool fact_plus_zero(double v)
{
    unsigned long long w;
    memcpy(&w, &v, 8);
    return w == 0ull;
}
KLATT_LAYOUT_HD inline double fact_abs(double v) { return v < 0 ? -v : v; }
KLATT_LAYOUT_HD constexpr unsigned long long fact_key(int n)
{
    unsigned long long z = (unsigned long long)(n + 1) * 0x9E3779B97F4A7C15ull;
    z = (z ^ (z >> 30)) * 0xBF58476D1CE4E5B9ull;
    z = (z ^ (z >> 27)) * 0x94D049BB133111EBull;
    return z ^ (z >> 31);
}
KLATT_LAYOUT_HD inline unsigned long long fact_fold(unsigned long long a, unsigned long long c)
{
#if defined(__HIP_DEVICE_COMPILE__)
    return (__umul64hi(a, c) ^ (a * c)) + a + ((c << 32) | (c >> 32));
#else
    const unsigned __int128 m = (unsigned __int128)a * c;
    return ((unsigned long long)(m >> 64) ^ (unsigned long long)m) + a + ((c << 32) | (c >> 32));
#endif
}

KLATT_LAYOUT_HD inline uint32_t pitch_flags(double p0, double p46)
{
    uint32_t fl = 0;
    if (!fact_finite(p0) || !fact_finite(p46)) fl |= 2u;
    if (!(fact_abs(p0) <= 1e30) || !(fact_abs(p46) <= 1e30)) fl |= 4u;
    return fl;
}
KLATT_LAYOUT_HD inline uint32_t shape_flags(const double* p, double maxF, double maxBw)
{
    uint32_t fl = 0;
    if (p[3] != 0.0 || p[6] != 0.0 || p[24] != 0.0) fl |= 1u;
    bool finite = true;
    for (int i = 1; i < kNumParams - 1; ++i) finite = finite && fact_finite(p[i]);
    if (!finite) fl |= 2u;
    for (int i = 25; i <= 30; ++i)
        if (!(fact_abs(p[i]) <= 1e6) || !(p[i + 6] >= 0.0) || !(p[i + 6] <= 1e6)) fl |= 1u;
    if (p[23] != 0.0 || !(p[21] >= 1.0) || !(p[22] >= 0.0) || !(p[21] <= 1e6) || !(p[22] <= 1e6) ||
        !(fact_abs(p[13]) <= 1e6) || !(fact_abs(p[14]) <= 1e6) || !(fact_abs(p[5]) <= 1e30) || !(fact_abs(p[44]) <= 1e30))
        fl |= 4u;
    if (!fact_plus_zero(p[3])) fl |= FACT_TURBULENCE;
    if (!fact_plus_zero(p[6])) fl |= FACT_ASPIRATION;
    if (p[37] != 0.0 || !(p[31] >= 1.0) || !(p[31] <= 1e6) || !(fact_abs(p[25]) <= 1e6) || !(fact_abs(p[24]) <= 1e30) || !(fact_abs(p[44]) <= 1e30))
        fl |= FACT_PARALLEL1;
    bool inRange = true;
    for (int i = 7; i <= 14; ++i) inRange = inRange && (fact_abs(p[i]) <= maxF) && (p[i + 8] >= 0.0) && (p[i + 8] <= maxBw);
    for (int i = 25; i <= 30; ++i) inRange = inRange && (fact_abs(p[i]) <= maxF) && (p[i + 6] >= 0.0) && (p[i + 6] <= maxBw);
    if (!inRange) fl |= 8u;
    return fl;
}
KLATT_LAYOUT_HD inline bool shape_values_equal(const double* a, const double* c)
{
    bool same = true;
    for (int i = 1; i < kNumParams - 1; ++i) {
        unsigned long long x, y;
        memcpy(&x, &a[i], 8); memcpy(&y, &c[i], 8);
        same = same && x == y;
    }
    return same;
}

KLATT_LAYOUT_HD inline FrameFacts frame_facts(const double* p, double maxF, double maxBw)
{
    FrameFacts o;
    const uint32_t fl = shape_flags(p, maxF, maxBw) | pitch_flags(p[0], p[46]);
    unsigned long long x = 0x9E3779B97F4A7C15ull, y = 0xC2B2AE3D27D4EB4Full;
#if defined(__HIPCC__)
#pragma unroll
#endif
    for (int i = 0; i < 46; i += 2) {
        unsigned long long w0, w1 = 0;
        memcpy(&w0, &p[1 + i], 8);
        if (i + 1 < kShapeValues) memcpy(&w1, &p[2 + i], 8);
        x ^= fact_fold(w0 ^ fact_key(2 * i), w1 ^ fact_key(2 * i + 1));
        y ^= fact_fold(w0 ^ fact_key(2 * i + 100), w1 ^ fact_key(2 * i + 101));
    }
    x ^= x >> 32; x *= 0xD6E8FEB86659FD93ull; x ^= x >> 32;
    y ^= y >> 31; y *= 0xBF58476D1CE4E5B9ull; y ^= y >> 29;
    o.h0 = x; o.h1 = y; o.flags = fl; o.pad = 0;
    return o;
}

#if defined(__HIPCC__)
__global__ void __launch_bounds__(256) klatt_frame_facts(const double* __restrict__ frames, FrameFacts* __restrict__ out, long long nFrames, double maxF, double maxBw)
{
    const long long stride = (long long)gridDim.x * blockDim.x;
    for (long long k = (long long)blockIdx.x * blockDim.x + threadIdx.x; k < nFrames; k += stride) {
        double p[kNumParams];
        const double* src = frames + k * kNumParams;
#pragma unroll
        for (int i = 0; i < kNumParams; ++i) p[i] = src[i];
        out[k] = frame_facts(p, maxF, maxBw);
    }
}

struct FrameRecord {
    double voicePitch, endVoicePitch;
    uint32_t shape;
    uint32_t minSamples, fadeSamples;
    int32_t userIndex;
};
constexpr uint32_t kRecordSilence = 0xFFFFFFFFu;
static_assert(sizeof(FrameRecord) == 32, "FrameRecord layout");

__global__ void __launch_bounds__(256) klatt_expand_frames(const FrameRecord* __restrict__ records, const double* __restrict__ shapes,
                                                           double* __restrict__ frames, FrameMeta* __restrict__ meta, long long nFrames)
{
    constexpr int kTileFrames = 64, kTilePairs = kTileFrames * kNumParams / 2;
    __shared__ FrameRecord rec[kTileFrames];
    const long long nTiles = (nFrames + kTileFrames - 1) / kTileFrames;
    for (long long tile = blockIdx.x; tile < nTiles; tile += gridDim.x) {
        const long long k0 = tile * kTileFrames;
        const int n = (int)((nFrames - k0) < (long long)kTileFrames ? (nFrames - k0) : (long long)kTileFrames);
        __syncthreads();
        if ((int)threadIdx.x < n) {
            const FrameRecord r = records[k0 + threadIdx.x];
            rec[threadIdx.x] = r;
            FrameMeta m;
            m.minSamples = r.minSamples;
            m.fadeSamples = r.fadeSamples > 1u ? r.fadeSamples : 1u;
            m.userIndex = r.userIndex;
            m.flags = r.shape == kRecordSilence ? FRAME_NULL : 0u;
            meta[k0 + threadIdx.x] = m;
        }
        __syncthreads();
        auto value = [&](int j) -> double {
            const int f = j / kNumParams, p = j - f * kNumParams;
            if (f >= n) return 0.0;
            const uint32_t shape = rec[f].shape;
            if (shape == kRecordSilence) return 0.0;
            return p == 0 ? rec[f].voicePitch : (p == kNumParams - 1 ? rec[f].endVoicePitch : shapes[(long long)shape * kNumParams + p]);
        };
        double2* const out = reinterpret_cast<double2*>(frames + k0 * kNumParams);
        const int pairs = (n * kNumParams + 1) / 2;
        for (int j = (int)threadIdx.x; j < kTilePairs && j < pairs; j += (int)blockDim.x) {
            const double x = value(2 * j), y = value(2 * j + 1);
            if (2 * j + 1 < n * kNumParams) out[j] = make_double2(x, y);
            else frames[k0 * kNumParams + 2 * j] = x;
        }
    }
}

__global__ void __launch_bounds__(256) klatt_verify_shared(const double* __restrict__ frames, const uint32_t* __restrict__ rep, long long nFrames,
                                                           unsigned long long* __restrict__ mismatch)
{
    const long long stride = (long long)gridDim.x * blockDim.x;
    for (long long k = (long long)blockIdx.x * blockDim.x + threadIdx.x; k < nFrames; k += stride) {
        const uint32_t r = rep[k];
        if (r == 0xFFFFFFFFu || (long long)r == k) continue;
        if (!shape_values_equal(frames + k * kNumParams, frames + (long long)r * kNumParams))
            atomicMin(mismatch, (unsigned long long)k);
    }
}
#endif

}
```

nvspeechplayer_amd/csrc/klatt_systolic.h:

```cpp
#pragma once

#include <type_traits>

#include "klatt_device.h"

namespace klatt {

#ifndef KLATT_UNROLL
#define KLATT_UNROLL 8
#endif
#ifndef KLATT_MINWAVES
#define KLATT_MINWAVES 1
#endif
#ifndef KLATT_PAIR
#define KLATT_PAIR 1
#endif
#ifndef KLATT_NOISY_RUNS
#define KLATT_NOISY_RUNS 0
#endif
#ifndef KLATT_FADE_TIGHT
#define KLATT_FADE_TIGHT 1
#endif
#ifndef KLATT_NOISY_TIGHT
#define KLATT_NOISY_TIGHT 1
#endif
#define KLATT_STR2(x) #x
#define KLATT_STR(x) KLATT_STR2(x)

#ifndef KLATT_FLAT_EXHAUSTIVE
#define KLATT_FLAT_EXHAUSTIVE 1
#endif
constexpr int kStages = 4;
#ifndef KLATT_DEAD_TERMS
#define KLATT_DEAD_TERMS 3
#endif
#ifndef KLATT_FLAT_SOURCE
#define KLATT_FLAT_SOURCE 1
#endif

template <bool NOISE, int CH, bool FLAT = false, int SPLIT = 0>
struct SysLds {
    static constexpr int MOVED = SPLIT & 3;
    static constexpr bool NP0 = (SPLIT >> 2) != 0;
    static constexpr int kBufs = 2;
    static constexpr int kBufsX = 2;
    static constexpr int kBufBytes = CH * kLanes * (FLAT ? (int)sizeof(sig_t) : 8);
    static constexpr int kPipeBytes = kBufs * kBufBytes;
    static constexpr int kNumPipes = NOISE ? 4 : 3;
    static constexpr int kPipeO = kBufsX * kBufBytes;
    static constexpr int kTileOff = kPipeO + (kNumPipes - 1) * kPipeBytes;
    static constexpr int kRowBase = kTileOff + kLanes * kTileStride;
    static constexpr int kRowCount = kRowBase + kLanes * 8;
    static constexpr int kMaxLen = kRowCount + kLanes * 4;
    static constexpr int kSync = kMaxLen + 16;
    static constexpr int kFrames = kSync + 32;
    static constexpr int kParams0 = (FLAT && KLATT_FLAT_SOURCE) ? 0 : (NP0 ? 12 : 7), kParams1 = FLAT ? 0 : (NOISE ? (NP0 ? 0 : 5) + 2 * (3 + MOVED) : 7), kParams2 = FLAT ? 0 : (NOISE ? 14 - 2 * MOVED : 6), kParams3 = FLAT ? 0 : (NOISE ? 14 : 5);
    static constexpr int kFrames1 = kFrames + 1 * kParams0 * kLanes * 8;
    static constexpr int kFrames2 = kFrames1 + 2 * kParams1 * kLanes * 8;
    static constexpr int kFrames3 = kFrames2 + 2 * kParams2 * kLanes * 8;
    static constexpr int kBytes = kFrames3 + 2 * kParams3 * kLanes * 8;
};

template <int NPARAM, int NRES, bool NWREG = false>
struct StageFrame {
    double* oldL;
    double* nwL;
    double nwR[NWREG && NPARAM > 0 ? NPARAM : 1];
    __device__ __forceinline__ double getNew(int k) const { return NWREG ? nwR[k] : nwL[k * kLanes]; }
    __device__ __forceinline__ void setNew(int k, double v) { if (NWREG) nwR[k] = v; else nwL[k * kLanes] = v; }
    double cur[NPARAM > 0 ? NPARAM : 1];
    double ra[NRES > 0 ? NRES : 1], rb[NRES > 0 ? NRES : 1], rc[NRES > 0 ? NRES : 1];
    double z1[NRES > 0 ? NRES : 1], z2[NRES > 0 ? NRES : 1];
    double invFade;
    uint32_t cnt, oldMin, newMin, newFade, nextFrame, resMask, parMask, produced;
    bool hasNew, oldNull, newNull, done;
};

struct PitchState {
    double cur0, old0, new0, oldInc, newInc;
};

template <int NPARAM, int NRES, bool NWREG>
__device__ __forceinline__ void stage_frame_init(StageFrame<NPARAM, NRES, NWREG>& f, bool live, unsigned char* region, int lane)
{
    f.oldL = reinterpret_cast<double*>(region) + lane;
    f.nwL = f.oldL + NPARAM * kLanes;
#pragma unroll
    for (int k = 0; k < NPARAM; ++k) { f.oldL[k * kLanes] = 0.0; f.setNew(k, 0.0); f.cur[k] = 0.0; }
#pragma unroll
    for (int r = 0; r < NRES; ++r) { f.ra[r] = 0.0; f.rb[r] = 2.0; f.rc[r] = -1.0; f.z1[r] = 0.0; f.z2[r] = 0.0; }
    f.invFade = 1.0;
    f.cnt = 0; f.oldMin = 0; f.newMin = 0; f.newFade = 1; f.nextFrame = 0; f.resMask = 0; f.parMask = 0; f.produced = 0;
    f.hasNew = false; f.oldNull = true; f.newNull = false; f.done = !live;
}

template <int NPARAM_, int NRES_, int GAIN_, bool PITCH_, bool ANTI0_, bool INLINE_COEF_ = false>
struct StageDesc {
    static constexpr int NPARAM = NPARAM_, NRES = NRES_, GAIN = GAIN_;
    static constexpr bool PITCH = PITCH_, ANTI0 = ANTI0_, INLINE_COEF = INLINE_COEF_;
};

struct StageCtx {
    const KernelArgs& A;
    const UttDesc& d;
    const double* myFrames;
    const FrameMeta* myMeta;
    uint32_t ringOff, ringMask;
    const FlatRef* myFlat;
    const SourceRef* mySrc;
    bool lone = false;
    double* loneLds = nullptr;
};
constexpr int kLoneLdsPerStage = 12288;
#ifndef KLATT_STREAM_SPLIT
#define KLATT_STREAM_SPLIT 5
#endif
#ifndef KLATT_LONE_SPLIT
// ... 623 lines not shown
    if (X.A.debug && (threadIdx.x & (kLanes - 1)) == 0) {
        unsigned long long* o = X.A.debug + (blockIdx.x * 4 + stampSlot) * 8;
        o[0] = st.work; o[1] = st.wait; o[2] = st.n[0]; o[3] = st.n[1]; o[4] = st.n[2]; o[5] = st.c[0]; o[6] = st.c[1]; o[7] = st.c[2];
    }
#endif
    (void)stampSlot;
}

template <int STAGE_, int NRES_, int NGAIN_, bool ANTI0_, uint32_t USUAL_ = 0, uint32_t USUAL2_ = 0, class R_ = sig_t, uint32_t SKIP_ = 0>
struct FlatDesc {
    using R = R_;
    static constexpr int STAGE = STAGE_;
    static constexpr int NRES = NRES_, NGAIN = NGAIN_, NE = NRES_ + NGAIN_;
    static constexpr bool ANTI0 = ANTI0_;
    static constexpr uint32_t USUAL = USUAL_, USUAL2 = USUAL2_, SKIP = SKIP_;
};

struct BarrierSync {
    __device__ __forceinline__ void begin(int) const {}
    __device__ __forceinline__ void end(int) const { __syncthreads(); }
    __device__ __forceinline__ void idle() const { __syncthreads(); }
};

#ifndef KLATT_MIX_UNROLL
#define KLATT_MIX_UNROLL 4
#endif
template <int E> using KindTag = std::integral_constant<int, E>;
typedef unsigned int flat_u4 __attribute__((ext_vector_type(4)));
typedef unsigned int flat_u2 __attribute__((ext_vector_type(2)));
typedef double flat_d2 __attribute__((ext_vector_type(2)));
template <class FD>
struct FlatState2 {
    static constexpr int NR = FD::NRES > 0 ? FD::NRES : 1;
    using R = typename FD::R;
    R ra[NR], rb[NR], rc[NR], z1[NR], z2[NR];
    R cur[2 * FD::NGAIN > 0 ? 2 * FD::NGAIN : 1];
    uint32_t idx[FD::NE], stride[FD::NE];
    uint32_t startAt, left, next, nFrames, length, produced;
    FlatRef nextRef;
    uint32_t wmask;
    bool live;
};
template <class R> struct ResPre { R a, p1, p2; };
template <class T> __device__ __forceinline__ void flat_pin(T v) { asm volatile("" :: "v"(v) : "memory"); }
template <class R> __device__ __forceinline__ void flat_pin(const ResPre<R>& q) { asm volatile("" :: "v"(q.a), "v"(q.p1), "v"(q.p2) : "memory"); }
template <int NE>
__device__ __forceinline__ uint32_t flat2_wave_kinds(uint32_t flags, bool live, const int* GE)
{
    const uint32_t mine = live ? (flags >> kUttKindShift) : 0u;
    uint32_t w = 0;
#pragma unroll
    for (int e = 0; e < NE; ++e) w |= __any((mine >> GE[e]) & 1u) ? (1u << e) : 0u;
    return w;
}
template <class FD>
__device__ __forceinline__ void flat2_init(FlatState2<FD>& f, bool live, const UttDesc& d, const StageCtx& X, const int* GE)
{
#pragma unroll
    for (int r = 0; r < FD::NRES; ++r) { f.ra[r] = 0; f.rb[r] = 2; f.rc[r] = -1; f.z1[r] = 0; f.z2[r] = 0; }
#pragma unroll
    for (int k = 0; k < 2 * FD::NGAIN; ++k) f.cur[k] = 0;
#pragma unroll
    for (int e = 0; e < FD::NE; ++e) { f.idx[e] = 0; f.stride[e] = 0; }
    f.live = live && d.length > 0u;
    f.nFrames = d.nFrames; f.length = d.length; f.next = 0; f.left = 0; f.produced = 0;
    const bool any = live && d.nFrames > 0u;
    f.startAt = any ? 1u : 0xFFFFFFFFu;
    f.nextRef = FlatRef{0u, 0u, 1u, 0u};
    if (any) f.nextRef = X.myFlat[0];
    f.wmask = (uint32_t)__builtin_amdgcn_readfirstlane((int)flat2_wave_kinds<FD::NE>(d.flags, live, GE));
}
template <class FD>
__device__ __forceinline__ void flat2_switch(FlatState2<FD>& f, const StageCtx& X, const int* GE)
{
    const FlatRef p = f.nextRef;
    const uint32_t part = p.off + track_part(p.mask, p.fadeSamples, FD::STAGE);
    const uint32_t nMove = track_stage_slots(p.mask, FD::STAGE), hdr = track_stage_entries(FD::STAGE) - nMove;
    uint32_t moving = 0, still = 0;
#pragma unroll
    for (int e = 0; e < FD::NE; ++e) {
        if constexpr (FD::SKIP != 0u) {
#pragma unroll
            for (int k = 0; k < kTrackEntries; ++k)
                if (((FD::SKIP >> k) & 1u) && k < GE[e] && (e == 0 || k > GE[e - 1])) { const bool mv = (p.mask >> k) & 1u; moving += mv ? 1u : 0u; still += mv ? 0u : 1u; }
        }
        const bool moves = (p.mask >> GE[e]) & 1u;
        f.idx[e] = (part + (moves ? hdr + moving : still)) * 16u;
        f.stride[e] = moves ? nMove * 16u : 0u;
        const uint32_t w = GE[e] == 0 ? 2u : 1u;
        moving += moves ? w : 0u; still += moves ? 0u : w;
    }
    f.left = nMove ? p.fadeSamples : 1u;
    f.next++;
    const bool more = f.next < f.nFrames;
    f.startAt = more ? f.startAt + p.span : 0xFFFFFFFFu;
#pragma unroll
    for (int e = 0; e < FD::NE; ++e) { flat_pin(f.idx[e]); flat_pin(f.stride[e]); }
    flat_pin(f.left); flat_pin(f.startAt);
    f.nextRef = X.myFlat[more ? f.next : f.nFrames - 1u];
}
template <class FD, uint32_t SET, bool ALLROWS = false>
struct FlatMid {
    FlatState2<FD>& f;
    __amdgpu_buffer_rsrc_t rsrc;
    bool has;
    template <class... T>
    __device__ __forceinline__ void operator()(T... firstHalf) const
    {
        using R = typename FD::R;
        (flat_pin(firstHalf), ...);
        if (ALLROWS || has) {
#pragma unroll
            for (int e = 0; e < FD::NE; ++e) {
                if (!(SET & (1u << e))) continue;
                const uint32_t off = f.idx[e];
                const flat_d2 v = __builtin_bit_cast(flat_d2, __builtin_amdgcn_raw_buffer_load_b128(rsrc, off, 0, 0));
                if (e < FD::NRES) {
                    f.rb[e < FD::NRES ? e : 0] = (R)v.x; f.rc[e < FD::NRES ? e : 0] = (R)v.y;
                    if (FD::ANTI0 && e == 0) f.ra[0] = (R)__builtin_bit_cast(double, __builtin_amdgcn_raw_buffer_load_b64(rsrc, off + 16u, 0, 0));
                } else {
                    const int g = e < FD::NRES ? 0 : e - FD::NRES;
                    f.cur[2 * g] = (R)v.x; f.cur[2 * g + 1] = (R)v.y;
                }
                f.idx[e] = off + f.stride[e];
            }
        }
    }
};
struct NoMid { template <class... T> __device__ __forceinline__ void operator()(T...) const {} };
template <int MODE, bool DERIVE, class R>
__device__ __forceinline__ ResPre<R> res_pre(R ra, R rb, R rc, R z1, R z2)
{
    ResPre<R> p;
    p.a = DERIVE ? (R)((R)1 - rb - rc) : ra;
    if (MODE == MODE_FAST || !std::is_same<R, double>::value) { p.p1 = rb; p.p2 = rc; }
    else { p.p1 = rb * z1; p.p2 = rc * z2; }
    return p;
}
template <int MODE, class R>
__device__ __forceinline__ R res_post(const ResPre<R>& p, R in, R& z1, R& z2)
{
    R y;
    if (MODE == MODE_FAST || !std::is_same<R, double>::value) y = dot3<MODE>(p.a, in, p.p1, z1, p.p2, z2);
    else y = p.a * in + p.p1 + p.p2;
    z2 = z1; z1 = y;
    return y;
}

template <class FD, int CH, class FBody, class FChunk, class FSync = BarrierSync>
__device__ __forceinline__ void flat2_loop(int depth, int nIter, int nChunks, int stampSlot, FlatState2<FD>& f, const StageCtx& X, const int* GE, FBody body, FChunk perChunk,
                                           const FSync& sync = FSync{})
{
#ifdef KLATT_STAMPS
    Stamps st;
#endif
    using R = typename FD::R;
    uint32_t staleG = 0;
    const __amdgpu_buffer_rsrc_t rsrc = __builtin_amdgcn_make_buffer_rsrc(const_cast<double2*>(X.A.track), 0, (int)X.A.trackBytes, 0x00020000);
    for (int iter = 0; iter < nIter; ++iter) {
        STAMP_BEGIN();
        STAMP_IDLE();
        const int c = iter - depth;
        const bool inRange = c >= 0 && c < nChunks;
        if (inRange) {
            sync.begin(c);
            const uint32_t t0 = (uint32_t)c * (uint32_t)CH, t1 = t0 + (uint32_t)CH;
            if (f.length <= t0) f.live = false;
// ... 90 lines not shown
{
    static_assert(!LONE || STREAM, "LONE: a live handle pulled alone");
    static_assert(NASAL || !NOISE, "only quiet launches have a nasal-free instantiation");
    static_assert(NOISE || !STREAM, "live handles take the noisy instantiation");
    static_assert(!FLAT || (NOISE && !STREAM), "tracks: noisy batch launches");
    constexpr int SPLIT = stream_split<STREAM, WPS, LONE>();
    constexpr int MOVED = SPLIT & 3;
    using L = SysLds<NOISE, CH, FLAT, SPLIT>;
    static_assert(SPLIT != 3, "eight resonators in the head stage: not built");
    constexpr int kChunk = CH;
    extern __shared__ __attribute__((aligned(16))) unsigned char lds[];
    using PipeT = typename std::conditional<FLAT, sig_t, double>::type;
    PipeT* const pipeX = reinterpret_cast<PipeT*>(lds);
    PipeT* const pipeO = reinterpret_cast<PipeT*>(lds + L::kPipeO);
    PipeT* const pipeA = reinterpret_cast<PipeT*>(lds + L::kPipeO + L::kPipeBytes);
    PipeT* const pipeB = reinterpret_cast<PipeT*>(lds + L::kPipeO + (NOISE ? 2 : 1) * L::kPipeBytes);
    constexpr int nbuf_pipeX = L::kBufsX, nbuf_pipeO = L::kBufs, nbuf_pipeA = L::kBufs, nbuf_pipeB = L::kBufs;
    (void)nbuf_pipeX; (void)nbuf_pipeO; (void)nbuf_pipeA; (void)nbuf_pipeB;
    unsigned char* const tile = lds + L::kTileOff;
    long long* const rowBase = reinterpret_cast<long long*>(lds + L::kRowBase);
    uint32_t* const rowCount = reinterpret_cast<uint32_t*>(lds + L::kRowCount);
    uint32_t* const maxLenP = reinterpret_cast<uint32_t*>(lds + L::kMaxLen);

    const int lane = threadIdx.x & (kLanes - 1);
    const int wave = __builtin_amdgcn_readfirstlane(threadIdx.x >> 6);
    const long long slot = (long long)blockIdx.x * kLanes + lane;
    const uint32_t u = (slot < A.nSlots) ? A.order[slot] : 0xFFFFFFFFu;
    const bool live = (u != 0xFFFFFFFFu);

    UttDesc d;
    d.frameStart = 0; d.outStart = 0; d.nFrames = 0; d.seed = 0; d.flags = 0; d.length = 0;
    if (live) d = A.utt[u];
    const FrameWindow fw = frame_window(A, d);
    const StageCtx X{A, d, A.frames + fw.base * kNumParams, A.meta + fw.base, fw.off, fw.mask,
                     FLAT ? A.flatRef + d.frameStart : nullptr, FLAT ? A.sourceRef + d.frameStart : nullptr, LONE,
                     LONE ? reinterpret_cast<double*>(lds + L::kBytes + wave * kLoneLdsPerStage) : nullptr};
    const uint32_t nkey = noise_key(d.seed), ninc = noise_inc(d.seed), ninc2 = noise_inc2(ninc);
    constexpr int FINAL = NOISE ? 2 : 3;
#ifndef KLATT_PRELOAD
#define KLATT_PRELOAD 1
#endif
    constexpr bool kPre = !NOISE && KLATT_PRELOAD;

    uint32_t* const stageMaskP = maxLenP + 1;
    uint32_t* const syncP = reinterpret_cast<uint32_t*>(lds + L::kSync);
    if (threadIdx.x == 0) { *maxLenP = 0; *stageMaskP = 0; }
    if (threadIdx.x < 8) syncP[threadIdx.x] = 0;
    __syncthreads();
    int cand = wave;
    if (KLATT_PAIR && WPS == 2 && (NOISE || !NASAL)) {
        const uint32_t hw = __builtin_amdgcn_s_getreg((4 << 0) | (0 << 6) | (31 << 11));
        const uint32_t simd = (hw >> 4) & 3u, odd = hw & 1u;
        cand = (int)(KLATT_PAIR == 2 ? (simd ^ odd) : KLATT_PAIR == 3 ? (simd ^ (odd ? 3u : 0u)) : ((simd + (odd ? 2u : 0u)) & 3u));
    }
    if (wave == 0) atomicMax(maxLenP, d.length);
    if (lane == 0) atomicOr(stageMaskP, 1u << cand);
    __syncthreads();
    const int stage = __builtin_amdgcn_readfirstlane((*stageMaskP == 0xFu) ? cand : wave);
    if (stage == FINAL) { rowBase[lane] = d.outStart; rowCount[lane] = 0; }
    const uint32_t maxLen = *maxLenP;
    const int nChunks = (int)((maxLen + kChunk - 1) / kChunk);
    const int nIter = nChunks + (NOISE ? 2 : 3);
    const int fullChunks = STREAM ? (int)(A.maxSamples / (uint32_t)kChunk) : nChunks;
    double* const streamState = (STREAM && live) ? (A.statePtrs ? A.statePtrs[u] : A.state + (size_t)u * kStateDoubles) : nullptr;
    const bool streamPurge = STREAM && live && A.control && (A.control[u] & 1u);
#define PIPE(p, c, i) (p)[(((nbuf_##p) == 2 ? ((c) & 1) : ((c) % (nbuf_##p))) * kChunk + (i)) * kLanes + lane]
    using KSrc = LoopKnobs<false, (!NOISE || KLATT_NOISY_RUNS), false, STREAM, NOISE, KLATT_UNROLL, LONE, (STREAM && WPS == 1 && !LONE)>;
    using KFil = LoopKnobs<kPre, (!NOISE || KLATT_NOISY_RUNS), false, STREAM, NOISE, KLATT_UNROLL, LONE, (STREAM && WPS == 1 && !LONE)>;
    uint32_t noDelay = 0;
    auto never = [&]() __attribute__((always_inline)) { return false; };
    auto noBegin = [&](int) __attribute__((always_inline)) { return false; };
    auto noAlt = [&](int) __attribute__((always_inline)) {};
    auto noAltSample = [&](int, int, double) __attribute__((always_inline)) {};
    auto noFadeAlt = [&](int, bool, bool) __attribute__((always_inline)) { return false; };
    auto nothing = [&](int) __attribute__((always_inline)) {};
    auto noChunk = [&]() __attribute__((always_inline)) {};
    uint32_t deadSet = 0;
    if (FLAT) {
        const uint32_t mine = live ? d.flags : 0u;
#pragma unroll
        for (uint32_t bit = UTT_TURBULENCE; bit <= UTT_PARALLEL1; bit <<= 1) deadSet |= __any((mine & bit) != 0u) ? 0u : bit;
        deadSet = (uint32_t)__builtin_amdgcn_readfirstlane((int)(deadSet & A.deadTerms));
    }

    auto make_sync = [&](auto, auto, auto, int, int, int) __attribute__((always_inline)) { return BarrierSync{}; };
    using I0 = std::integral_constant<int, 0>; using I1 = std::integral_constant<int, 1>; using I2 = std::integral_constant<int, 2>;
    if (FLAT && KLATT_FLAT_SOURCE && stage == 0) {
        if constexpr (FLAT) {
            auto sourceStage = [&](auto deadTag) __attribute__((always_inline)) {
            constexpr int DEAD = decltype(deadTag)::value;
            constexpr bool NOTURB = DEAD >= 1;
#if KLATT_FLAT_LAYOUT == 2
            using FD = FlatDesc<0, 2, NOTURB ? 4 : 5, true, 0, 0, double, NOTURB ? (1u << 21) : 0u>;
            constexpr int GE[7] = {0, 1, 14, 20, NOTURB ? 22 : 21, NOTURB ? 23 : 22, 23};
            constexpr int CB = 2;
            constexpr uint32_t kUsualS0 = NOTURB ? 0x37u : 0x67u, kAllS0 = NOTURB ? 0x3Fu : 0x7Fu, kVibBit = 8u;
            constexpr bool kHead = true;
#else
            using FD = FlatDesc<0, 0, NOTURB ? 3 : 4, false, 0, 0, double, NOTURB ? (1u << 21) : 0u>;
            constexpr int GE[4] = {20, NOTURB ? 22 : 21, NOTURB ? 23 : 22, 23};
            constexpr int CB = 0;
            constexpr uint32_t kUsualS0 = NOTURB ? 0x6u : 0xCu, kAllS0 = NOTURB ? 0x7u : 0xFu, kVibBit = 1u;
            constexpr bool kHead = false;
#endif
            constexpr int CA = CB + (NOTURB ? 2 : 4);
            if (A.deadWaves && lane == 0) {
                if (DEAD >= 1) atomicAdd(A.deadWaves + 1, 1u);
                if (DEAD >= 2) atomicAdd(A.deadWaves + 2, 1u);
            }
            bool staleNP = false;
            FlatState2<FD> f;
            flat2_init<FD>(f, live, d, X, GE);
            PitchState ps;
            ps.cur0 = 0.0; ps.old0 = 0.0; ps.new0 = 0.0; ps.oldInc = 0.0; ps.newInc = 0.0;
            double pitchPhase = 0.0, vibPhase = 0.0, aspNoise = 0.0, invFade = 1.0, nfD = 1.0;
            uint32_t noiseSt = noise_first(nkey, ninc), cntF = 0, nfU = 0;
            uint32_t fadeEndAt = 0xFFFFFFFFu;
            int32_t lastIndex = -1;
            bool oldNull = true, newNull = false;
            SourceRef nextSrc{0.0, 0.0, 1.0, -1, 0u};
            if (live && d.nFrames > 0u) nextSrc = X.mySrc[0];
            auto source = [&](bool waveVib, auto setTag, const auto& mid) __attribute__((always_inline)) -> double {
                constexpr uint32_t SET = decltype(setTag)::value;
                double vib = 1.0;
                if (waveVib) {
                    const double vs = f.cur[CB + 1];
                    const double adv = frac_toward_zero(div_by(vs, A.sampleRateF, A.invSampleRate) + vibPhase);
                    vibPhase = (vs != 0.0) ? adv : vibPhase;
                    vib = (sin(vibPhase * 6.283185307179586) * 0.06 * f.cur[CB + 0]) + 1.0;
                }
                const double voiceAmp = f.cur[CA + 0], aspAmp = f.cur[CA + 1], preGain = f.cur[CA + 2];
                (void)aspAmp; (void)aspNoise; (void)noiseSt;
                pitchPhase = frac_toward_zero(div_by(ps.cur0 * vib, A.sampleRateF, A.invSampleRate) + pitchPhase);
                double voice = (pitchPhase * 2.0) - 1.0;
                double asp = 0.0;
                if constexpr (DEAD < 2) {
                    aspNoise = noise_uniform(noiseSt) + 0.75 * aspNoise;
                    noiseSt = noise_step2(noiseSt, ninc2);
                    asp = aspNoise * 0.2;
                }
                if constexpr (!NOTURB) {
                    const double turbGain = f.cur[CB + 2], openQ = f.cur[CB + 3];
                    double turb = asp * turbGain;
                    turb = (pitchPhase >= openQ) ? turb : turb * 0.01;
                    voice += turb;
                }
                voice *= voiceAmp;
                if constexpr (DEAD < 2) asp *= aspAmp;
                const double src = asp + voice;
                const double out = (src * preGain) * 0.5;
                if constexpr (kHead) {
                    const ResPre<double> q0 = res_pre<MODE, false>(f.ra[0], f.rb[0], f.rc[0], f.z1[0], f.z2[0]);
                    const ResPre<double> q1 = res_pre<MODE, ((SET >> 1) & 1u) != 0u>(f.ra[1], f.rb[1], f.rc[1], f.z1[1], f.z2[1]);
                    const double caNP = f.cur[0];
                    mid(out, q0, q1, caNP);
                    double zin = f.z1[0];
                    const double n0 = res_post<MODE>(q0, out, zin, f.z2[0]);
                    f.z1[0] = out;
                    const double np = res_post<MODE>(q1, n0, f.z1[1], f.z2[1]);
                    return fade_value(out, np, caNP);
                } else {
                    mid(out);
                    return out;
                }
            };
            auto vib_live = [&]() __attribute__((always_inline)) -> bool { return f.cur[CB + 0] != 0.0 || f.cur[CB + 1] != 0.0 || vibPhase != vibPhase; };
            const __amdgpu_buffer_rsrc_t rsrc = __builtin_amdgcn_make_buffer_rsrc(const_cast<double2*>(A.track), 0, (int)A.trackBytes, 0x00020000);
#ifdef KLATT_STAMPS
            Stamps st;
#endif
            const auto sync = make_sync(std::integral_constant<int, L::kBufsX>{}, I0{}, I1{}, 0, 0, 0);
            for (int iter = 0; iter < nIter; ++iter) {
                STAMP_BEGIN();
                STAMP_IDLE();
                const int c = iter;
                int lastChunk = -1;
                if (c < nChunks) {
                    sync.begin(c);
                    lastChunk = c;
                    const uint32_t t0 = (uint32_t)c * (uint32_t)CH, t1 = t0 + (uint32_t)CH;
                    if (f.length <= t0) f.live = false;
                    const bool busy = f.left > 0u || f.startAt <= t1 || cntF < nfU || fadeEndAt < t1 || vib_live();
                    STAMP_KIND(__any(busy) ? -1 : 0);
                    if (!__any(busy)) {
                        uint32_t run = f.live ? (f.startAt - t0 - 1u) / (uint32_t)CH : 0xFFFFFFFFu;
#pragma unroll
                        for (int m = 32; m >= 1; m >>= 1) { const uint32_t o = (uint32_t)__shfl_xor((int)run, m, kLanes); run = o < run ? o : run; }
                        run = (uint32_t)__builtin_amdgcn_readfirstlane((int)run);
                        const uint32_t room = (uint32_t)(nChunks - c);
                        run = run < room ? run : room;
                        run = run < 1u ? 1u : run;
                        int cc = c;
                        if (kHead && staleNP) { f.ra[1] = 1.0 - f.rb[1] - f.rc[1]; staleNP = false; }
                        for (uint32_t q = 0; q < run; ++q) {
                            if (f.live) {
#pragma unroll
                                for (int i = 0; i < CH; ++i) { ps.cur0 += ps.oldInc; PIPE(pipeX, cc, i) = source(false, std::integral_constant<uint32_t, 0u>{}, NoMid{}); }
                                ps.old0 = ps.cur0;
                            }
                            if (q + 1 < run) { STAMP_WORKED(); sync.end(cc); STAMP_SYNCED(); STAMP_BEGIN(); ++iter; ++cc; sync.begin(cc); lastChunk = cc; }
                        }
                    } else {
                        auto mixedChunk = [&](auto setTag, auto allFadeTag) __attribute__((always_inline)) {
                        constexpr uint32_t SET = decltype(setTag)::value;
                        constexpr bool ALLFADE = decltype(allFadeTag)::value;
                        const bool vibChunk = (SET & kVibBit) != 0u || __any(vib_live());
                        staleNP = true;
#pragma unroll KLATT_MIX_UNROLL
                        for (int i = 0; i < CH; ++i) {
                            const uint32_t t = t0 + (uint32_t)i;
                            const bool deq = !ALLFADE && t + 1u == f.startAt;
                            if (!ALLFADE && __any(deq)) {
                                if (deq) {
                                    const SourceRef m = nextSrc;
                                    const uint32_t nf = f.nextRef.fadeSamples;
                                    newNull = (m.flags & FRAME_NULL) != 0;
                                    ps.new0 = newNull ? ps.cur0 : m.pitch;
                                    ps.newInc = newNull ? 0.0 : m.pitchInc;
                                    if (!newNull && oldNull) ps.old0 = m.pitch;
                                    oldNull = newNull;
                                    if (m.userIndex != -1) lastIndex = m.userIndex;
                                    nfD = (double)nf; nfU = nf;
                                    ps.new0 += ps.newInc * nfD;
                                    invFade = m.invFade;
                                    cntF = 0;
                                    fadeEndAt = t + nf + 1u;
                                    flat_pin(ps.new0); flat_pin(ps.newInc); flat_pin(ps.old0); flat_pin(invFade); flat_pin(lastIndex); flat_pin(oldNull);
                                    flat2_switch<FD>(f, X, GE);
                                    nextSrc = X.mySrc[f.next < f.nFrames ? f.next : f.nFrames - 1u];
                                }
                            }
                            if (ALLFADE) {
                                cntF++;
                                ps.cur0 = fade_value(ps.old0, ps.new0, div_by((double)cntF, nfD, invFade));
                            } else {
                            const bool fad = !deq && cntF < nfU;
                            const bool ending = !deq && !fad && t == fadeEndAt;
                            const bool glide = !deq && !fad && !ending;
                            const uint32_t cn = cntF + 1u;
                            const double ratio = div_by((double)cn, nfD, invFade);
                            const double fv = fade_value(ps.old0, ps.new0, ratio);
                            const double gv = ps.cur0 + ps.oldInc;
                            ps.cur0 = fad ? fv : (glide ? gv : ps.cur0);
                            ps.old0 = ending ? ps.new0 : (glide ? gv : ps.old0);
                            ps.oldInc = ending ? ps.newInc : ps.oldInc;
                            cntF = fad ? cn : cntF;
                            fadeEndAt = ending ? 0xFFFFFFFFu : fadeEndAt;
                            }
                            const bool waveVib = vibChunk && __any(vib_live());
                            const bool has = f.left > 0u;
                            PIPE(pipeX, c, i) = source(waveVib, setTag, FlatMid<FD, SET>{f, rsrc, has});
                            if (has) f.left--;
                        }
                        };
                        const bool usual = c != 0 && (f.wmask & ~kUsualS0) == 0u;
                        const bool allFade = usual && !__any(vib_live()) && __all(!f.live || (cntF + (uint32_t)CH <= nfU && f.startAt > t1));
                        if (allFade) mixedChunk(std::integral_constant<uint32_t, kUsualS0>{}, std::true_type{});
                        else if (usual) mixedChunk(std::integral_constant<uint32_t, kUsualS0>{}, std::false_type{});
                        else mixedChunk(std::integral_constant<uint32_t, kAllS0>{}, std::false_type{});
                    }
                }
                STAMP_WORKED();
                if (lastChunk >= 0) sync.end(lastChunk); else sync.idle();
                STAMP_SYNCED();
            }
#ifdef KLATT_STAMPS
            if (A.debug && lane == 0) {
                unsigned long long* o = A.debug + (blockIdx.x * 4 + 0) * 8;
                o[0] = st.work; o[1] = st.wait; o[2] = st.n[0]; o[3] = st.n[1]; o[4] = st.n[2]; o[5] = st.c[0]; o[6] = st.c[1]; o[7] = st.c[2];
            }
#endif
            if (live) {
                UttResult res;
                res.produced = d.length; res.framesTaken = f.next; res.lastIndex = lastIndex; res.drained = 1u;
                A.result[u] = res;
            }
            };
            if ((KLATT_DEAD_TERMS & 4) && (deadSet & (UTT_TURBULENCE | UTT_ASPIRATION)) == (UTT_TURBULENCE | UTT_ASPIRATION)) sourceStage(std::integral_constant<int, 2>{});
            else if ((KLATT_DEAD_TERMS & 2) && (deadSet & UTT_TURBULENCE)) sourceStage(std::integral_constant<int, 1>{});
            else sourceStage(std::integral_constant<int, 0>{});
        }
    } else if (stage == 0) {
        constexpr bool NP0 = (SPLIT >> 2) != 0;
        using D = StageDesc<NP0 ? 12 : 7, NP0 ? 2 : 0, 6, true, NP0, NP0>;
        constexpr int P[12] = {1, 2, 3, 4, 5, 6, 44, 13, 21, 14, 22, 23};
        constexpr int RF[2] = {7, 9}, RB[2] = {8, 10};
        StageFrame<D::NPARAM, D::NRES, true> f;
        PitchState ps;
        stage_frame_init(f, live, lds + L::kFrames, lane);
        ps.cur0 = 0.0; ps.old0 = 0.0; ps.new0 = 0.0; ps.oldInc = 0.0; ps.newInc = 0.0;
        double pitchPhase = 0.0, vibPhase = 0.0, aspNoise = 0.0;
        uint32_t noiseSt = noise_first(nkey, ninc);
        int32_t lastIndex = -1;
        bool vibFrames = false;
        constexpr int GR0[2] = {0, 1};
        if (STREAM && live) {
            if (streamState[239] != 0.0) {
                pitchPhase = streamState[208]; vibPhase = streamState[209]; aspNoise = streamState[210];
                lastIndex = (int32_t)streamState[220]; noiseSt = (uint32_t)streamState[221];
            }
            stage_state_load<D>(f, &ps, streamState, P, RF, RB, GR0, streamPurge);
            vibFrames = f.oldL[0] != 0.0 || f.oldL[kLanes] != 0.0 || f.getNew(0) != 0.0 || f.getNew(1) != 0.0;
        }

        auto source = [&](bool waveVib) __attribute__((always_inline)) -> double {
            double vib = 1.0;
            if (waveVib) {
                const double vs = f.cur[1];
                const double adv = frac_toward_zero(div_by(vs, A.sampleRateF, A.invSampleRate) + vibPhase);
                vibPhase = (vs != 0.0) ? adv : vibPhase;
                vib = (sin(vibPhase * 6.283185307179586) * 0.06 * f.cur[0]) + 1.0;
            }
            pitchPhase = frac_toward_zero(div_by(ps.cur0 * vib, A.sampleRateF, A.invSampleRate) + pitchPhase);
            double voice = (pitchPhase * 2.0) - 1.0;
            double src;
            if (NOISE) {
                aspNoise = noise_uniform(noiseSt) + 0.75 * aspNoise;
                noiseSt = noise_step2(noiseSt, ninc2);
                double asp = aspNoise * 0.2;
                double turb = asp * f.cur[2];
                turb = (pitchPhase >= f.cur[3]) ? turb : turb * 0.01;
                voice += turb;
                voice *= f.cur[4];
                asp *= f.cur[5];
                src = asp + voice;
            } else {
                src = voice * f.cur[4];
            }
            const double x = (src * f.cur[6]) * 0.5;
            if (!NP0) return x;
            const double n0 = dot3<MODE>(f.ra[0], x, f.rb[0], f.z1[0], f.rc[0], f.z2[0]);
            f.z2[0] = f.z1[0]; f.z1[0] = x;
            const double np = resonate<MODE>(f.z1[NP0 ? 1 : 0], f.z2[NP0 ? 1 : 0], f.ra[NP0 ? 1 : 0], f.rb[NP0 ? 1 : 0], f.rc[NP0 ? 1 : 0], n0);
            return fade_value(x, np, f.cur[NP0 ? 11 : 0]);
        };
        auto vib_live_now = [&]() __attribute__((always_inline)) -> bool {
            return vibFrames || f.cur[0] != 0.0 || f.cur[1] != 0.0 || vibPhase != vibPhase;
        };
        stage_loop<D, MODE, CH, KSrc>(0, nIter, nChunks, fullChunks, stage, f, &ps, &lastIndex, noDelay, P, RF, RB, X,
            [&]() __attribute__((always_inline)) { return __any(!f.done && vib_live_now()); },
            [&](int kind) __attribute__((always_inline)) -> bool { return !NOISE && kind == 0 && !__any(!f.done && ps.oldInc != 0.0); },
            [&](int c) __attribute__((always_inline)) {
                ps.cur0 += ps.oldInc;
                const double inc = div_by(ps.cur0 * 1.0, A.sampleRateF, A.invSampleRate);
                double ph[kChunk];
#pragma unroll
                for (int i = 0; i < kChunk; ++i) { pitchPhase = frac_toward_zero(inc + pitchPhase); ph[i] = pitchPhase; }
#pragma unroll
                for (int i = 0; i < kChunk; ++i) PIPE(pipeX, c, i) = ((((ph[i] * 2.0) - 1.0) * f.cur[4]) * f.cur[6]) * 0.5;
            },
            noAltSample,
            [&](int, int) __attribute__((always_inline)) { return 0.0; },
            [&](int c, int i, bool steady, double) __attribute__((always_inline)) {
                if (steady) ps.cur0 += ps.oldInc;
                PIPE(pipeX, c, i) = source(false);
            },
            [&](int c, bool lerp, bool gainOnly) __attribute__((always_inline)) -> bool {
                if (NOISE || !gainOnly) return false;
                constexpr int GI = 6;
                const double g0 = lerp ? f.oldL[GI * kLanes] : f.cur[GI], g1 = lerp ? f.getNew(GI) : f.cur[GI];
                if (__any(g1 != g1 || ps.new0 != ps.new0)) return false;
                const double gd = g1 - g0, p0 = ps.old0, pd = ps.new0 - p0, nf = (double)f.newFade;
                if (!__any(pd != 0.0 || p0 != p0)) {
// ... 15 lines not shown
                        const double ratio = div_by((double)f.cnt, nf, f.invFade);
                        ps.cur0 = p0 + (pd * ratio);
                        const double gain = g0 + (gd * ratio);
                        pitchPhase = frac_toward_zero(div_by(ps.cur0 * 1.0, A.sampleRateF, A.invSampleRate) + pitchPhase);
                        PIPE(pipeX, c, i) = ((((pitchPhase * 2.0) - 1.0) * f.cur[4]) * gain) * 0.5;
                        if (i == kChunk - 1) f.cur[GI] = gain;
                    }
                }
                return true;
            },
            [&](int c, int i, bool emit) __attribute__((always_inline)) {
                if (emit && f.hasNew && f.cnt == 0)
                    vibFrames = f.oldL[0] != 0.0 || f.oldL[kLanes] != 0.0 || f.getNew(0) != 0.0 || f.getNew(1) != 0.0;
                const bool waveVib = __any(emit && vib_live_now());
                if (emit) { PIPE(pipeX, c, i) = source(waveVib); f.produced++; }
            },
            [&](int n) __attribute__((always_inline)) { ps.old0 = ps.cur0; f.produced += n; },
            [&](int n) __attribute__((always_inline)) { f.produced += n; },
            noChunk);
        if (live) {
            UttResult res;
            res.produced = f.produced; res.framesTaken = f.nextFrame; res.lastIndex = lastIndex; res.drained = STREAM ? (f.done ? 1u : 0u) : 1u;
            A.result[u] = res;
        }
        if (STREAM && live) {
            stage_state_save<D>(f, &ps, streamState, P, GR0);
            streamState[208] = pitchPhase; streamState[209] = vibPhase; streamState[210] = aspNoise;
            streamState[220] = (double)lastIndex; streamState[221] = (double)noiseSt;
        }
    } else if (FLAT && stage == 1) {
        if constexpr (FLAT) {
#if KLATT_FLAT_LAYOUT == 2
            using FD = FlatDesc<1, 6, 0, false, 0x38u>;
            constexpr int GE[6] = {2, 3, 4, 5, 6, 7};
            FlatState2<FD> f;
            flat2_init<FD>(f, live, d, X, GE);
            flat2_loop<FD, CH>(1, nIter, nChunks, stage, f, X, GE,
                [&](int c, int i, auto setTag, const auto& mid) __attribute__((always_inline)) {
                    constexpr uint32_t SET = decltype(setTag)::value;
                    ResPre<sig_t> q[6];
#pragma unroll
                    for (int r = 0; r < 6; ++r) q[r] = ((SET >> r) & 1u) ? res_pre<MODE, true>(f.ra[r], f.rb[r], f.rc[r], f.z1[r], f.z2[r])
                                                                         : res_pre<MODE, false>(f.ra[r], f.rb[r], f.rc[r], f.z1[r], f.z2[r]);
                    mid(q[0], q[1], q[2], q[3], q[4], q[5]);
                    sig_t o = PIPE(pipeX, c, i);
#pragma unroll
                    for (int r = 0; r < 6; ++r) o = res_post<MODE>(q[r], o, f.z1[r], f.z2[r]);
                    PIPE(pipeO, c, i) = o;
                },
                noChunk, make_sync(std::integral_constant<int, L::kBufs>{}, I1{}, I1{}, 0, 0, 2));
#else
            using FD = FlatDesc<1, 6, 1, true, 0x63u>;
            constexpr int GE[7] = {0, 1, 2, 3, 4, 5, 14};
            FlatState2<FD> f;
            flat2_init<FD>(f, live, d, X, GE);
            flat2_loop<FD, CH>(1, nIter, nChunks, stage, f, X, GE,
                [&](int c, int i, auto setTag, const auto& mid) __attribute__((always_inline)) {
                    constexpr uint32_t SET = decltype(setTag)::value;
                    const ResPre<sig_t> q0 = res_pre<MODE, false>(f.ra[0], f.rb[0], f.rc[0], f.z1[0], f.z2[0]);
                    const ResPre<sig_t> q1 = res_pre<MODE, ((SET >> 1) & 1u) != 0u>(f.ra[1], f.rb[1], f.rc[1], f.z1[1], f.z2[1]);
                    const ResPre<sig_t> q2 = res_pre<MODE, ((SET >> 2) & 1u) != 0u>(f.ra[2], f.rb[2], f.rc[2], f.z1[2], f.z2[2]);
                    const ResPre<sig_t> q3 = res_pre<MODE, ((SET >> 3) & 1u) != 0u>(f.ra[3], f.rb[3], f.rc[3], f.z1[3], f.z2[3]);
                    const ResPre<sig_t> q4 = res_pre<MODE, ((SET >> 4) & 1u) != 0u>(f.ra[4], f.rb[4], f.rc[4], f.z1[4], f.z2[4]);
                    const ResPre<sig_t> q5 = res_pre<MODE, ((SET >> 5) & 1u) != 0u>(f.ra[5], f.rb[5], f.rc[5], f.z1[5], f.z2[5]);
                    const sig_t caNP = f.cur[0];
                    mid(q0, q1, q2, q3, q4, q5, caNP);
                    const sig_t x = PIPE(pipeX, c, i);
                    sig_t zin = f.z1[0];
                    const sig_t n0 = res_post<MODE>(q0, x, zin, f.z2[0]);
                    f.z1[0] = x;
                    const sig_t np = res_post<MODE>(q1, n0, f.z1[1], f.z2[1]);
                    sig_t o = fade_value(x, np, caNP);
                    o = res_post<MODE>(q2, o, f.z1[2], f.z2[2]);
                    o = res_post<MODE>(q3, o, f.z1[3], f.z2[3]);
                    o = res_post<MODE>(q4, o, f.z1[4], f.z2[4]);
                    o = res_post<MODE>(q5, o, f.z1[5], f.z2[5]);
                    PIPE(pipeO, c, i) = o;
                },
                noChunk);
#endif
        }
    } else if (FLAT && stage == 3) {
        if constexpr (FLAT) {
            auto parallel = [&](auto noP1Tag) __attribute__((always_inline)) {
            constexpr bool NOP1 = decltype(noP1Tag)::value;
            constexpr int NR = NOP1 ? 3 : 4;
            using FD = FlatDesc<3, NR, 3, false, NOP1 ? 0x3Bu : 0x77u, 0, sig_t, NOP1 ? (1u << 8) : 0u>;
            constexpr int GE[7] = {NOP1 ? 9 : 8, NOP1 ? 10 : 9, NOP1 ? 11 : 10, NOP1 ? 17 : 11, NOP1 ? 18 : 17, NOP1 ? 19 : 18, 19};
            FlatState2<FD> f;
            flat2_init<FD>(f, live, d, X, GE);
            if (NOP1 && A.deadWaves && lane == 0) atomicAdd(A.deadWaves + 0, 1u);
            sig_t fricNoise = 0;
            uint32_t noiseSt = noise_step(noise_first(nkey, ninc), ninc);
            flat2_loop<FD, CH>(1, nIter, nChunks, stage, f, X, GE,
                [&](int c, int i, auto setTag, const auto& mid) __attribute__((always_inline)) {
                    constexpr uint32_t SET = decltype(setTag)::value;
                    const ResPre<sig_t> q0 = res_pre<MODE, ((SET >> 0) & 1u) != 0u>(f.ra[0], f.rb[0], f.rc[0], f.z1[0], f.z2[0]);
                    const ResPre<sig_t> q1 = res_pre<MODE, ((SET >> 1) & 1u) != 0u>(f.ra[1], f.rb[1], f.rc[1], f.z1[1], f.z2[1]);
                    const ResPre<sig_t> q2 = res_pre<MODE, ((SET >> 2) & 1u) != 0u>(f.ra[2], f.rb[2], f.rc[2], f.z1[2], f.z2[2]);
                    constexpr int R3 = NR - 1;
                    ResPre<sig_t> q3{};
                    if constexpr (!NOP1) q3 = res_pre<MODE, ((SET >> 3) & 1u) != 0u>(f.ra[R3], f.rb[R3], f.rc[R3], f.z1[R3], f.z2[R3]);
                    fricNoise = (sig_t)noise_uniform(noiseSt) + (sig_t)0.75 * fricNoise;
                    noiseSt = noise_step2(noiseSt, ninc2);
                    const sig_t fric = fricNoise * (sig_t)0.3 * f.cur[0];
                    const sig_t y = (fric * f.cur[1]) * (sig_t)0.5;
                    const sig_t pa1 = f.cur[2], pa2 = f.cur[3], pa3 = f.cur[4], pa4 = f.cur[5];
                    if constexpr (NOP1) {
                        mid(q0, q1, q2, y, pa2, pa3, pa4);
                        sig_t w = res_post<MODE>(q0, y, f.z1[0], f.z2[0]);
                        sig_t par = (w - y) * pa2;
                        w = res_post<MODE>(q1, y, f.z1[1], f.z2[1]);
                        par += (w - y) * pa3;
                        w = res_post<MODE>(q2, y, f.z1[2], f.z2[2]);
                        par += (w - y) * pa4;
                        PIPE(pipeA, c, i) = y; PIPE(pipeB, c, i) = par;
                    } else {
                        mid(q0, q1, q2, q3, y, pa1, pa2, pa3, pa4);
                        sig_t par = 0;
                        sig_t w = res_post<MODE>(q0, y, f.z1[0], f.z2[0]);
                        par += (w - y) * pa1;
                        w = res_post<MODE>(q1, y, f.z1[1], f.z2[1]);
                        par += (w - y) * pa2;
                        w = res_post<MODE>(q2, y, f.z1[2], f.z2[2]);
                        par += (w - y) * pa3;
                        w = res_post<MODE>(q3, y, f.z1[R3], f.z2[R3]);
                        par += (w - y) * pa4;
                        PIPE(pipeA, c, i) = y; PIPE(pipeB, c, i) = par;
                    }
                },
                noChunk, make_sync(std::integral_constant<int, L::kBufs>{}, I0{}, I1{}, 0, 0, 4));
            };
            if ((KLATT_DEAD_TERMS & 1) && (deadSet & UTT_PARALLEL1)) parallel(std::true_type{}); else parallel(std::false_type{});
        }
    } else if (FLAT && (KLATT_FLAT_EXHAUSTIVE || stage == 2)) {
        if constexpr (FLAT) {
#if KLATT_FLAT_LAYOUT == 2
            constexpr int GE[4] = {12, 13, 15, 16};
            using FD = FlatDesc<2, 2, 2, false, 0xEu>;
            constexpr int RS = 0;
#else
            constexpr int GE[6] = {6, 7, 12, 13, 15, 16};
            using FD = FlatDesc<2, 4, 2, false, 0x3Bu>;
            constexpr int RS = 2;
#endif
            FlatState2<FD> f;
            flat2_init<FD>(f, live, d, X, GE);
            int16_t* const myRow = reinterpret_cast<int16_t*>(tile + lane * kTileStride);
            uint32_t it = 0;
            auto flush_tile = [&](uint32_t tileStart, uint32_t validTo) __attribute__((always_inline)) {
                rowCount[lane] = f.produced;
                asm volatile("s_waitcnt lgkmcnt(0)" ::: "memory");
                constexpr int kChunksPerRow = kTile / 8;
                constexpr int kRowsPerPass = kLanes / kChunksPerRow;
                constexpr int kPasses = kLanes / kRowsPerPass;
                const int chunk = lane % kChunksPerRow;
                const uint32_t first = tileStart + (uint32_t)chunk * 8u;
                uint2 lo[kPasses], hi[kPasses];
                uint32_t cnt[kPasses];
                long long base[kPasses];
#pragma unroll
                for (int p = 0; p < kPasses; ++p) {
                    const int row = p * kRowsPerPass + lane / kChunksPerRow;
                    const uint2* src = reinterpret_cast<const uint2*>(tile + row * kTileStride + chunk * 16);
                    lo[p] = src[0]; hi[p] = src[1];
                    cnt[p] = rowCount[row];
                    base[p] = rowBase[row];
                }
#pragma unroll
                for (int p = 0; p < kPasses; ++p) {
                    if (cnt[p] > first && first < validTo) {
                        uint4* dst = reinterpret_cast<uint4*>(A.pcm + base[p] + first);
                        *dst = make_uint4(lo[p].x, lo[p].y, hi[p].x, hi[p].y);
                    }
                }
                asm volatile("s_waitcnt lgkmcnt(0)" ::: "memory");
            };
            flat2_loop<FD, CH>(2, nIter, nChunks, stage, f, X, GE,
                [&](int c, int i, auto setTag, const auto& mid) __attribute__((always_inline)) {
                    constexpr uint32_t SET = decltype(setTag)::value;
                    constexpr int NR = 2 + RS;
                    ResPre<sig_t> q[4];
#pragma unroll
                    for (int r = 0; r < NR; ++r) q[r] = ((SET >> r) & 1u) ? res_pre<MODE, true>(f.ra[r], f.rb[r], f.rc[r], f.z1[r], f.z2[r])
                                                                          : res_pre<MODE, false>(f.ra[r], f.rb[r], f.rc[r], f.z1[r], f.z2[r]);
                    const sig_t pa5 = f.cur[0], pa6 = f.cur[1], bypass = f.cur[2], outGain = f.cur[3];
                    if constexpr (RS == 2) mid(q[0], q[1], q[2], q[3], pa5, pa6, bypass, outGain);
                    else mid(q[0], q[1], pa5, pa6, bypass, outGain);
                    sig_t o = PIPE(pipeO, c, i);
                    const sig_t y = PIPE(pipeA, c, i);
#pragma unroll
                    for (int r = 0; r < RS; ++r) o = res_post<MODE>(q[r], o, f.z1[r], f.z2[r]);
                    sig_t par = PIPE(pipeB, c, i);
                    sig_t w = res_post<MODE>(q[RS], y, f.z1[RS], f.z2[RS]);
                    par += (w - y) * pa5;
                    w = res_post<MODE>(q[RS + 1], y, f.z1[RS + 1], f.z2[RS + 1]);
                    par += (w - y) * pa6;
                    par = fade_value(par, y, bypass);
                    const sig_t mix = o + par;
                    const sig_t v = (mix * outGain) * (sig_t)4000.0;
                    const sig_t lo = (v < (sig_t)32000.0) ? v : (sig_t)32000.0;
                    const sig_t cl = (lo > (sig_t)-32000.0) ? lo : (sig_t)-32000.0;
                    myRow[(it % kTile) + i] = (int16_t)(uint32_t)(int)cl;
                },
                [&]() __attribute__((always_inline)) { it += kChunk; if ((it % kTile) == 0) flush_tile(it - kTile, it); },
                make_sync(std::integral_constant<int, L::kBufs>{}, I2{}, I0{}, 2, 4, 0));
            if ((it % kTile) != 0) flush_tile(it - (it % kTile), it);
        }
    } else if (!NOISE && !NASAL && (stage == 1 || stage == 2)) {
        using D = StageDesc<6, 3, -1, false, false>;
        const bool s1 = (stage == 1);
        const int P[6] = {s1 ? 12 : 9, s1 ? 20 : 17, s1 ? 11 : 8, s1 ? 19 : 16, s1 ? 10 : 7, s1 ? 18 : 15};
        constexpr int RF[3] = {0, 2, 4}, RB[3] = {1, 3, 5};
        StageFrame<6, 3> f;
        stage_frame_init(f, live, lds + (s1 ? L::kFrames1 : L::kFrames2), lane);
        PipeT* const pin = s1 ? pipeX : pipeO;
        PipeT* const pout = s1 ? pipeO : pipeA;
        constexpr int nbuf_pin = 2, nbuf_pout = 2;
        auto dsp = [&](double o) __attribute__((always_inline)) -> double {
#pragma unroll
            for (int r = 0; r < 3; ++r) o = resonate<MODE>(f.z1[r], f.z2[r], f.ra[r], f.rb[r], f.rc[r], o);
            return o;
        };
        auto run = [&](int depth) __attribute__((always_inline)) {
            stage_loop<D, MODE, CH, KFil>(depth, nIter, nChunks, fullChunks, stage, f, nullptr, nullptr, noDelay, P, RF, RB, X, never, noBegin, noAlt, noAltSample,
                [&](int c, int i) __attribute__((always_inline)) { return PIPE(pin, c, i); },
                [&](int c, int i, bool steady, double pre) __attribute__((always_inline)) { PIPE(pout, c, i) = dsp((kPre && steady) ? pre : PIPE(pin, c, i)); },
                noFadeAlt,
                [&](int c, int i, bool emit) __attribute__((always_inline)) { if (emit) PIPE(pout, c, i) = dsp(PIPE(pin, c, i)); },
                nothing, nothing, noChunk);
        };
        if (s1) run(1); else run(2);
    } else if (stage == 1) {
        constexpr bool HEAD = (SPLIT >> 2) == 0;
        constexpr int NCASC = NOISE ? 3 + MOVED : 1;
        constexpr int NR = (HEAD ? 2 : 0) + NCASC;
        using D = StageDesc<HEAD ? 2 * NR + 1 : 2 * NR, NR, -1, false, HEAD, NOISE>;
        constexpr int P[15] = {head_param(HEAD, NCASC, 0), head_param(HEAD, NCASC, 1), head_param(HEAD, NCASC, 2), head_param(HEAD, NCASC, 3), head_param(HEAD, NCASC, 4),
                               head_param(HEAD, NCASC, 5), head_param(HEAD, NCASC, 6), head_param(HEAD, NCASC, 7), head_param(HEAD, NCASC, 8), head_param(HEAD, NCASC, 9),
                               head_param(HEAD, NCASC, 10), head_param(HEAD, NCASC, 11), head_param(HEAD, NCASC, 12), head_param(HEAD, NCASC, 13), head_param(HEAD, NCASC, 14)};
        constexpr int RF[7] = {0, 2, 4, 6, 8, 10, 12};
        constexpr int RB[7] = {1, 3, 5, 7, 9, 11, 13};
        constexpr int CANP = HEAD ? 2 * NR : 0;
        StageFrame<D::NPARAM, NR> f;
        stage_frame_init(f, live, lds + L::kFrames1, lane);
        constexpr int GR1[7] = {HEAD ? 0 : 2, HEAD ? 1 : 3, HEAD ? 2 : 4, HEAD ? 3 : 5, HEAD ? 4 : 6, HEAD ? 5 : 7, 6};
        if (STREAM && live) stage_state_load<D>(f, nullptr, streamState, P, RF, RB, GR1, streamPurge);
        auto dsp = [&](double x) __attribute__((always_inline)) -> double {
            double o = x;
            if (HEAD) {
                const double n0 = dot3<MODE>(f.ra[0], x, f.rb[0], f.z1[0], f.rc[0], f.z2[0]);
                f.z2[0] = f.z1[0]; f.z1[0] = x;
                const double np = resonate<MODE>(f.z1[1], f.z2[1], f.ra[1], f.rb[1], f.rc[1], n0);
                o = fade_value(x, np, f.cur[CANP]);
            }
#pragma unroll
            for (int r = HEAD ? 2 : 0; r < NR; ++r) o = resonate<MODE>(f.z1[r], f.z2[r], f.ra[r], f.rb[r], f.rc[r], o);
            return o;
        };
        stage_loop<D, MODE, CH, KFil>(1, nIter, nChunks, fullChunks, stage, f, nullptr, nullptr, noDelay, P, RF, RB, X, never, noBegin, noAlt, noAltSample,
            [&](int c, int i) __attribute__((always_inline)) { return PIPE(pipeX, c, i); },
            [&](int c, int i, bool steady, double pre) __attribute__((always_inline)) { PIPE(pipeO, c, i) = dsp((kPre && steady) ? pre : PIPE(pipeX, c, i)); },
            noFadeAlt,
            [&](int c, int i, bool emit) __attribute__((always_inline)) { if (emit) PIPE(pipeO, c, i) = dsp(PIPE(pipeX, c, i)); },
            nothing, nothing, noChunk);
        if (STREAM && live) stage_state_save<D>(f, nullptr, streamState, P, GR1);
    } else if (NOISE && stage == 3) {
        using D = StageDesc<14, 4, 9, false, false, true>;
        constexpr int P[14] = {25, 31, 26, 32, 27, 33, 28, 34, 24, 44, 37, 38, 39, 40};
        constexpr int RF[4] = {0, 2, 4, 6}, RB[4] = {1, 3, 5, 7};
        StageFrame<14, 4> f;
        stage_frame_init(f, live, lds + L::kFrames3, lane);
        double fricNoise = 0.0;
        uint32_t noiseSt = noise_step(noise_first(nkey, ninc), ninc);
        constexpr int GR3[4] = {8, 9, 10, 11};
        if (STREAM && live) {
            if (streamState[239] != 0.0) { fricNoise = streamState[211]; noiseSt = noise_step((uint32_t)streamState[221], ninc); }
            stage_state_load<D>(f, nullptr, streamState, P, RF, RB, GR3, streamPurge);
        }
        auto dsp = [&](int c, int i) __attribute__((always_inline)) {
            fricNoise = noise_uniform(noiseSt) + 0.75 * fricNoise;
            noiseSt = noise_step2(noiseSt, ninc2);
            const double fric = fricNoise * 0.3 * f.cur[8];
            const double y = (fric * f.cur[9]) * 0.5;
            double par = 0.0;
#pragma unroll
            for (int r = 0; r < 4; ++r) {
                const double w = resonate<MODE>(f.z1[r], f.z2[r], f.ra[r], f.rb[r], f.rc[r], y);
                par += (w - y) * f.cur[10 + r];
            }
// ... 116 lines not shown
```

nvspeechplayer_amd/speechPlayer.py:

```python
import math
from ctypes import POINTER, Structure, byref, c_double, c_int, c_short, c_void_p, cast
from ctypes import c_longlong as ctypes_longlong

import numpy as np

from . import _native

speechPlayer_frameParam_t = c_double

FRAME_FIELDS = [
    'voicePitch',
    'vibratoPitchOffset',
    'vibratoSpeed',
    'voiceTurbulenceAmplitude',
    'glottalOpenQuotient',
    'voiceAmplitude',
    'aspirationAmplitude',
    'cf1', 'cf2', 'cf3', 'cf4', 'cf5', 'cf6', 'cfN0', 'cfNP',
    'cb1', 'cb2', 'cb3', 'cb4', 'cb5', 'cb6', 'cbN0', 'cbNP',
    'caNP',
    'fricationAmplitude',
    'pf1', 'pf2', 'pf3', 'pf4', 'pf5', 'pf6',
    'pb1', 'pb2', 'pb3', 'pb4', 'pb5', 'pb6',
    'pa1', 'pa2', 'pa3', 'pa4', 'pa5', 'pa6',
# ... 1907 lines not shown
        sd = None if noiseSeed is None else np.ascontiguousarray(noiseSeed, dtype=np.uint32)
        self._check(self._dll.speechPlayer_batch_setText(self._h, n, ptrs, None if not espeakVoice else espeakVoice.encode("utf8"), float(speed),
                                                         pitch.ctypes.data, float(inflection), None if not voice else voice.encode("utf8"),
                                                         None if sd is None else sd.ctypes.data))
        self.nUtterances = n

    @property
    def totalSamples(self):
        return self._dll.speechPlayer_batch_totalSamples(self._h)

    @property
    def totalFrames(self):
        return self._dll.speechPlayer_batch_totalFrames(self._h)

    def utteranceSamples(self, u):
        return self._dll.speechPlayer_batch_utteranceSamples(self._h, u)

    def synthesize(self, wait=True):
        self._check(self._dll.speechPlayer_batch_synthesize(self._h))
        if wait:
            self._check(self._dll.speechPlayer_batch_wait(self._h))

    def wait(self):
        self._check(self._dll.speechPlayer_batch_wait(self._h))

    def read(self, u):
        n = self.utteranceSamples(u)
        buf = np.zeros(max(n, 1), dtype=np.int16)
        got = self._check(self._dll.speechPlayer_batch_read(self._h, u, buf.ctypes.data, n))
        return buf[:got]

    def readFloat(self, u):
        n = self.utteranceSamples(u)
        buf = np.zeros(max(n, 1), dtype=np.float32)
        got = self._check(self._dll.speechPlayer_batch_readFloat(self._h, u, buf.ctypes.data, n))
        return buf[:got]

    def writeWav(self, u, path):
        import wave
        pcm = self.read(u)
        with wave.open(path, "wb") as w:
            w.setnchannels(1); w.setsampwidth(2); w.setframerate(self.sampleRate)
            w.writeframes(pcm.astype("<i2").tobytes())

    def readAll(self, out=None):
        total = self.totalSamples
        if out is not None:
            if out.dtype != np.int16 or not out.flags["C_CONTIGUOUS"] or out.size < total:
                raise ValueError("readAll: out must be a contiguous int16 array of at least %d samples" % total)
            buf = out
        else:
            buf = np.empty(max(total, 1), dtype=np.int16)
        starts = np.zeros(self.nUtterances + 1, dtype=np.int64)
        got = self._check(self._dll.speechPlayer_batch_readAll(self._h, buf.ctypes.data, total, starts.ctypes.data))
        return buf[:got], starts

    def readAllAsync(self, out):
        total = self.totalSamples
        if out.dtype != np.int16 or not out.flags["C_CONTIGUOUS"] or out.size < total:
            raise ValueError("readAllAsync: out must be a contiguous int16 array of at least %d samples" % total)
        starts = np.zeros(self.nUtterances + 1, dtype=np.int64)
        got = self._check(self._dll.speechPlayer_batch_readAllAsync(self._h, out.ctypes.data, out.size, starts.ctypes.data))
        return out[:got], starts

    def readWait(self):
        self._check(self._dll.speechPlayer_batch_readWait(self._h))

    def digest(self, per_utterance=False):
        import ctypes
        whole = ctypes.c_ulonglong(0)
        per = np.zeros(max(self.nUtterances, 1), dtype=np.uint64) if per_utterance else None
        self._check(self._dll.speechPlayer_batch_digest(self._h, None if per is None else per.ctypes.data, ctypes.byref(whole)))
        return (int(whole.value), per[:self.nUtterances]) if per_utterance else int(whole.value)

    def getLastIndex(self, u):
        return self._dll.speechPlayer_batch_getLastIndex(self._h, u)

    def time(self, launches):
        ms = np.zeros(launches, dtype=np.float32)
        self._check(self._dll.speechPlayer_batch_time(self._h, launches, ms.ctypes.data))
        return ms

    def kernelInfo(self):
        info = np.zeros(23, dtype=np.int32)
        self._check(self._dll.speechPlayer_batch_kernelInfo(self._h, info.ctypes.data, len(info)))
        dead = dict(waves_without_parallel1=int(info[20]), waves_without_turbulence=int(info[21]), waves_without_aspiration=int(info[22]))
        return dict(vgprs=int(info[0]), lds_bytes=int(info[1]), wavefronts=int(info[2]), cus=int(info[3]),
                    workgroups_per_cu_by_lds=int(info[4]), scratch_bytes=int(info[5]),
                    stage_parallel_chunk=int(info[6]), noisy_group=bool(info[7]),
                    lane_pipelined=bool(info[8]), lane_pipelined_utterances=int(info[9]),
                    nasal_free=bool(info[10]), nasal_free_utterances=int(info[11]),
                    tracked_utterances=int(info[12]), tracks=int(info[13]), track_mbytes=int(info[14]), tracked=bool(info[15]),
                    direct_utterances=int(info[16]), direct=bool(info[17]), direct_mbytes=int(info[18]), **dead)

    def devicePcm(self):
        return self._dll.speechPlayer_batch_devicePcm(self._h)

    def deviceOffset(self, u):
        return self._dll.speechPlayer_batch_deviceOffset(self._h, u)

    def close(self):
        if getattr(self, "_h", None):
            self._dll.speechPlayer_batch_destroy(self._h)
            self._h = None

    def __del__(self):
        try:
            self.close()
        except Exception:
            pass


class NodePlayer(object):

    def __init__(self, sampleRate, devices, mode=0, layout=None):
        self.sampleRate = sampleRate
        self._dll = _native.load()
        dev = np.ascontiguousarray(devices, dtype=np.int32)
        self._h = self._dll.speechPlayer_node_create(sampleRate, len(dev), dev.ctypes.data)
        if not self._h:
            raise RuntimeError("speechPlayer_node_create failed: %s" % _native.last_error())
        self._check(self._dll.speechPlayer_node_setOption(self._h, b"mode", mode))
        if layout is not None:
            self._check(self._dll.speechPlayer_node_setOption(self._h, b"layout", layout))
        self.nUtterances = 0
        self._lens = None

    def _check(self, rc):
        if rc is None or rc < 0:
            raise RuntimeError("speechPlayer node call failed: %s" % _native.last_error())
        return rc

    def setUtterances(self, frameStart, frames, minSamples, fadeSamples, userIndex=None, isNull=None, noiseSeed=None):
        fs = np.ascontiguousarray(frameStart, dtype=np.int64)
        fr = np.ascontiguousarray(frames, dtype=np.float64).reshape(-1, 47)
        m = np.ascontiguousarray(minSamples, dtype=np.uint32)
        f = np.ascontiguousarray(fadeSamples, dtype=np.uint32)
        assert fs[-1] == len(fr) == len(m) == len(f)
        ix = None if userIndex is None else np.ascontiguousarray(userIndex, dtype=np.int32)
        nu = None if isNull is None else np.ascontiguousarray(isNull, dtype=np.uint8)
        sd = None if noiseSeed is None else np.ascontiguousarray(noiseSeed, dtype=np.uint32)
        p = lambda a: None if a is None else a.ctypes.data
        self._check(self._dll.speechPlayer_node_setUtterances(self._h, len(fs) - 1, p(fs), p(fr), p(m), p(f), p(ix), p(nu), p(sd)))
        self.nUtterances = len(fs) - 1
        per = np.maximum(m.astype(np.int64), np.maximum(f.astype(np.int64), 1) + 1) + 1
        c = np.concatenate([[0], np.cumsum(per)])
        self._lens = c[fs[1:]] - c[fs[:-1]]

    def setIpa(self, texts, speed=1, basePitch=100, inflection=0.5, clauseType=None, noiseSeed=None, voice=None,
               trailing_silence_ms=150.0, textOf=None):
        from .ipa import _text_pointers, _clauses
        ptrs, n, keep = _text_pointers(texts, textOf)
        pitch = np.ascontiguousarray(np.broadcast_to(np.asarray(basePitch, dtype=np.float64), (n,)))
        sd = None if noiseSeed is None else np.ascontiguousarray(noiseSeed, dtype=np.uint32)
        by_name = voice is None or isinstance(voice, str)
        vo = None if by_name else np.ascontiguousarray(np.broadcast_to(np.asarray(voice, dtype=np.int32), (n,)))
        self._check(self._dll.speechPlayer_node_setIpa(self._h, int(self.sampleRate), n, ptrs.ctypes.data, float(speed), pitch.ctypes.data, float(inflection),
                                                       _clauses(clauseType, n), None if vo is None else vo.ctypes.data,
                                                       (voice.encode("utf8") if (by_name and voice) else None),
                                                       -1.0 if trailing_silence_ms is None else float(trailing_silence_ms), None if sd is None else sd.ctypes.data))
        del keep
        self.nUtterances = n
        self._lens = None

    def utteranceSamples(self, u):
        for d in range(self._dll.speechPlayer_node_devices(self._h)):
            mem = self.shardUtterances(d)
            at = np.flatnonzero(mem == u)
            if len(at):
# ... 69 lines not shown
```

Measured before the change: 190.0 billion.

## Skip dead parallel-branch and nasal resonators per wavefront in flat tracked stages

Adds a second per-utterance presence mask covering parallel formants 2-6 and nasal, computed from shape data on the host and uploaded for tracked utterances. In the flat systolic kernel each wavefront ORs these masks with a wave-wide vote and picks lighter compiled stage bodies that drop resonators whose amplitude is zero for every lane (parallel 2-4, 5, or 5 and 6). The goal is to cut double-precision resonator work and track-entry loads for inactive branches. In exchange it adds more template instantiations, which can raise code size and register pressure, plus extra host classification work.

```diff
diff --git a/nvspeechplayer_amd/csrc/klatt_batchplan.h b/nvspeechplayer_amd/csrc/klatt_batchplan.h
--- a/nvspeechplayer_amd/csrc/klatt_batchplan.h
+++ b/nvspeechplayer_amd/csrc/klatt_batchplan.h
@@ -47,6 +47,15 @@
     flags = (needsNoise ? UTT_NEEDS_NOISE : (!(fl & FACT_NASAL) ? UTT_NO_NASAL : 0u)) | (fl & kUttPresent);
     shape = finite ? (!(fl & FACT_UNBOUNDED) ? 3 : 1) : 0;
 }
+template <class Meta, class Facts>
+inline void classify_list(const Meta* meta, const Facts* facts, long long n, uint32_t& flags, unsigned char& shape, uint32_t& present2)
+{
+    classify_list(meta, facts, n, flags, shape);
+    uint32_t p2 = 0;
+    for (long long k = 0; k < n; ++k)
+        if (!(meta[k].flags & FRAME_NULL)) p2 |= facts[k].present2;
+    present2 = p2 & kUtt2Present;
+}
 
 
 struct ListTable {
@@ -55,6 +64,7 @@
     std::vector<uint32_t> flags;
     std::vector<unsigned char> shape;
     std::vector<uint32_t> weight;
+    std::vector<uint32_t> present2;
     long long size() const { return (long long)flags.size(); }
     unsigned long long run_key(long long l) const { return timing[(size_t)l] ^ ((unsigned long long)lens[(size_t)l] * 0x9E3779B97F4A7C15ull); }
 };
@@ -282,4 +292,24 @@
     }
 }
 
-}
+template <class FlagsOf, class Present2Of>
+inline void dead2_wave_counts(const uint32_t* order, long long first, long long n, FlagsOf flagsOf, Present2Of present2Of, int built, long long counts[kDead2Counts],
+                              int width = kLanes)
+{
+    for (int k = 0; k < kDead2Counts; ++k) counts[k] = 0;
+    for (long long w = first; w < first + n; w += width) {
+        uint32_t present = 0, present2 = 0;
+        bool any = false;
+        for (long long s = w; s < std::min(w + width, first + n); ++s)
+            if (order[s] != kNoUtt) { present |= flagsOf(order[s]); present2 |= present2Of(order[s]); any = true; }
+        if (!any) continue;
+        const bool no5 = !(present2 & UTT2_PARALLEL5), no56 = no5 && !(present2 & UTT2_PARALLEL6);
+        const int fin = ((built & 32) && no56) ? 2 : (((built & 16) && no5) ? 1 : 0);
+        counts[0] += ((built & 8) && !(present & UTT_TURBULENCE) && !(present2 & UTT2_NASAL)) ? 1 : 0;
+        counts[1] += fin >= 1 ? 1 : 0;
+        counts[2] += fin >= 2 ? 1 : 0;
+        counts[3] += ((built & 64) && !(present & UTT_PARALLEL1) && !(present2 & kUtt2Parallel234)) ? 1 : 0;
+    }
+}
+
+}
diff --git a/nvspeechplayer_amd/csrc/klatt_consts.h b/nvspeechplayer_amd/csrc/klatt_consts.h
--- a/nvspeechplayer_amd/csrc/klatt_consts.h
+++ b/nvspeechplayer_amd/csrc/klatt_consts.h
@@ -25,4 +25,14 @@
 constexpr uint32_t FACT_ASPIRATION = UTT_ASPIRATION;
 constexpr uint32_t FACT_PARALLEL1 = UTT_PARALLEL1;
 
+constexpr uint32_t UTT2_PARALLEL2 = 1u;
+constexpr uint32_t UTT2_PARALLEL3 = 2u;
+constexpr uint32_t UTT2_PARALLEL4 = 4u;
+constexpr uint32_t UTT2_PARALLEL5 = 8u;
+constexpr uint32_t UTT2_PARALLEL6 = 16u;
+constexpr uint32_t UTT2_NASAL = 32u;
+constexpr uint32_t kUtt2Present = 63u;
+constexpr uint32_t kUtt2Parallel234 = UTT2_PARALLEL2 | UTT2_PARALLEL3 | UTT2_PARALLEL4;
+constexpr int kDead2Counts = 4;
+
 }
diff --git a/nvspeechplayer_amd/csrc/klatt_device.h b/nvspeechplayer_amd/csrc/klatt_device.h
--- a/nvspeechplayer_amd/csrc/klatt_device.h
+++ b/nvspeechplayer_amd/csrc/klatt_device.h
@@ -102,6 +102,8 @@
     unsigned long long* debug;
     uint32_t* deadWaves;
     uint32_t deadTerms;
+    uint32_t deadTerms2;
+    const uint32_t* present2;
 };
 
 __device__ constexpr int kResF[kNumRes] = {13, 14, 12, 11, 10, 9, 8, 7, 25, 26, 27, 28, 29, 30};
diff --git a/nvspeechplayer_amd/csrc/klatt_engine.hip b/nvspeechplayer_amd/csrc/klatt_engine.hip
--- a/nvspeechplayer_amd/csrc/klatt_engine.hip
+++ b/nvspeechplayer_amd/csrc/klatt_engine.hip
@@ -523,6 +523,8 @@
     int deadTerms = 1;
     DeviceBuffer<uint32_t> dDeadWaves;
     long long planDeadWaves[3] = {0, 0, 0};
+    long long planDead2Waves[kDead2Counts] = {0, 0, 0, 0};
+    DeviceBuffer<uint32_t> dPresent2;
     long long nUtt = 0, nFrames = 0, nSlots = 0;
     long long nLists = 0, nFramesSpoken = 0;
     std::vector<long long> uttFrameStart;
@@ -870,19 +872,21 @@
         t.negPiOverSr = a.negPiOverSr; t.twoPiOverSr = a.twoPiOverSr;
         const long long tg = b->nJobs;
         if (tg > 0x7FFFFFFF) { set_error("too many tracks: %lld", b->nJobs); return -1; }
-        if (b->dDeadWaves.reserve(3)) return -1;
-        HIP_TRY(hipMemsetAsync(b->dDeadWaves.ptr, 0, 3 * sizeof(uint32_t), st));
+        if (b->dDeadWaves.reserve(8)) return -1;
+        static_assert(3 + kDead2Counts <= 8, "the counters' block");
+        HIP_TRY(hipMemsetAsync(b->dDeadWaves.ptr, 0, 8 * sizeof(uint32_t), st));
         hipLaunchKernelGGL(klatt_tracks, dim3((unsigned)tg), dim3(kLanes * kTrackWaves), 0, st, t);
         HIP_TRY(hipGetLastError());
         a.order = b->dOrder.ptr + b->nQuiet; a.nSlots = nTr;
         a.flatRef = b->dFlatRef.ptr; a.sourceRef = b->dSourceRef.ptr; a.track = b->dTrack.ptr;
         a.trackBytes = (uint32_t)std::min<unsigned long long>(((unsigned long long)b->trackEntries + kTrackPad) * sizeof(double2), 0xFFFFFFFFull);
         a.deadWaves = b->dDeadWaves.ptr; a.deadTerms = b->deadTerms ? kUttPresent : 0u;
+        a.present2 = b->dPresent2.ptr; a.deadTerms2 = (b->deadTerms && b->dPresent2.ptr) ? kUtt2Present : 0u;
         const GroupPlan pl = plan_group(b->layout, true, b->nSlots, nTr + nNoisy, b->cus);
         const long long g = (nTr + kLanes - 1) / kLanes;
         if (pl.chunk == 8 ? launch_systolic<true, KLATT_FLAT_CH, KLATT_FLAT_WPS, true, false, true>(a, b->mode, g, st)
                           : launch_systolic<true, 16, 1, true, false, true>(a, b->mode, g, st)) return -1;
-        a.flatRef = nullptr; a.sourceRef = nullptr; a.track = nullptr; a.deadWaves = nullptr; a.deadTerms = 0u;
+        a.flatRef = nullptr; a.sourceRef = nullptr; a.track = nullptr; a.deadWaves = nullptr; a.deadTerms = 0u; a.present2 = nullptr; a.deadTerms2 = 0u;
     }
     if (nDir > 0) {
         hipStream_t st = next_stream();
@@ -1907,7 +1911,7 @@
     b->dDense.release(); b->dDenseStart.release(); b->dFacts.release(); b->hFacts.release();
     b->dRecords.release(); b->dShapeTable.release(); b->dRep.release(); b->dMismatch.release();
     b->dFrames.release(); b->dMeta.release(); b->dUtt.release(); b->dOrder.release(); b->dPcm.release(); b->dResult.release();
-    b->dFloat.release(); b->dDebug.release(); b->dDigest.release(); b->bounce.release(); b->dDeadWaves.release();
+    b->dFloat.release(); b->dDebug.release(); b->dDigest.release(); b->bounce.release(); b->dDeadWaves.release(); b->dPresent2.release();
     b->dFlatRef.release(); b->dSourceRef.release(); b->dJobs.release(); b->dShapes.release(); b->dTrack.release();
     b->dDirectJobs.release(); b->dDirectFirst.release(); b->dDirectHdr.release(); b->dDirectRec.release();
     delete b;
@@ -2158,6 +2162,7 @@
     long long nDirectUtt = 0;
     bool directAligned = false;
     std::vector<UttDesc> utt;
+    std::vector<uint32_t> present2;
     std::vector<long long> uttFrameStart;
     std::vector<uint32_t> uttFrames, uttList, uttSeed;
     LanePacking lanes;
@@ -2324,15 +2329,19 @@
     c.factsOnDevice = (c.framesPinned || c.byDevice) && c.earlyStarted;
     RawVector<FrameFacts>& fv = c.scratch.facts;
     if (c.byRecords) {
-        std::vector<uint32_t> shapeFl((size_t)in.nShapes);
-        for (long long s = 0; s < in.nShapes; ++s) shapeFl[(size_t)s] = shape_flags(reinterpret_cast<const double*>(in.shapes + s), maxFDirect, maxBwDirect);
+        std::vector<uint32_t> shapeFl((size_t)in.nShapes), shapeP2((size_t)in.nShapes);
+        for (long long s = 0; s < in.nShapes; ++s) {
+            shapeFl[(size_t)s] = shape_flags(reinterpret_cast<const double*>(in.shapes + s), maxFDirect, maxBwDirect);
+            shapeP2[(size_t)s] = shape_present2(reinterpret_cast<const double*>(in.shapes + s));
+        }
         fv.resize((size_t)nF);
         parallel_ranges(nF, 1 << 15, [&](long long a, long long e) {
             for (long long k = a; k < e; ++k) {
                 const speechPlayer_frameRecord_t& r = in.records[k];
                 FrameFacts f;
-                f.h0 = r.shape; f.h1 = ~0ull; f.pad = 0;
+                f.h0 = r.shape; f.h1 = ~0ull;
                 f.flags = r.shape == SPEECHPLAYER_RECORD_SILENCE ? 0u : (shapeFl[r.shape] | pitch_flags(r.voicePitch, r.endVoicePitch));
+                f.present2 = r.shape == SPEECHPLAYER_RECORD_SILENCE ? 0u : present2_of(f.flags, shapeP2[r.shape]);
                 fv[k] = f;
             }
         });
@@ -2387,9 +2396,10 @@
     const FrameFacts* const facts = c.facts;
     lists.shape.assign((size_t)nL, 0);
     lists.flags.assign((size_t)nL, 0);
+    lists.present2.assign((size_t)nL, 0);
     parallel_ranges(nL, 4096, [&](long long la, long long le) {
         for (long long l = la; l < le; ++l)
-            classify_list(meta + listStart[l], facts + listStart[l], listStart[l + 1] - listStart[l], lists.flags[l], lists.shape[l]);
+            classify_list(meta + listStart[l], facts + listStart[l], listStart[l + 1] - listStart[l], lists.flags[l], lists.shape[l], lists.present2[l]);
     });
     c.lap("classification");
     RouteOptions& route = c.route;
@@ -2473,7 +2483,7 @@
     const SetInput& in = c.in;
     const long long nU = c.nU;
     const long long* const listStart = c.listStart;
-    c.utt.resize((size_t)nU); c.uttFrameStart.resize((size_t)nU); c.uttFrames.resize((size_t)nU); c.uttList.resize((size_t)nU); c.uttSeed.resize((size_t)nU);
+    c.utt.resize((size_t)nU); c.present2.resize((size_t)nU); c.uttFrameStart.resize((size_t)nU); c.uttFrames.resize((size_t)nU); c.uttList.resize((size_t)nU); c.uttSeed.resize((size_t)nU);
     parallel_ranges(nU, 1 << 15, [&](long long a, long long e) {
         for (long long u = a; u < e; ++u) {
             const long long l = c.list_of(u);
@@ -2485,6 +2495,7 @@
             d.flags = c.lists.flags[l];
             d.length = c.lists.lens[l];
             c.utt[u] = d;
+            c.present2[u] = c.lists.present2[l];
             c.uttFrameStart[u] = d.frameStart; c.uttFrames[u] = d.nFrames; c.uttList[u] = (uint32_t)l; c.uttSeed[u] = d.seed;
         }
     });
@@ -2519,6 +2530,10 @@
     if (nTrackedUtt > 0 || nDirectUtt > 0) {
         if (b->dSourceRef.reserve((size_t)nF)) return -1;
     }
+    if (nTrackedUtt > 0) {
+        if (b->dPresent2.reserve((size_t)nU)) return -1;
+        HIP_TRY(hipMemcpyAsync(b->dPresent2.ptr, c.present2.data(), (size_t)nU * sizeof(uint32_t), hipMemcpyHostToDevice, b->stream));
+    }
     if (nDirectUtt > 0) {
         const size_t nD = directJobs.size();
         if (b->dDirectJobs.reserve(nD) || b->dDirectFirst.reserve((size_t)nU) || b->dDirectHdr.reserve((size_t)kDirectStages * nD) ||
@@ -2577,6 +2592,8 @@
     b->nQuiet = lanes.nQuietSlots; b->nNoNasal = lanes.nNoNasalSlots;
     b->nTracked = lanes.nTrackedUtt > 0 ? lanes.nTracked : 0; b->nTrackedUtt = lanes.nTrackedUtt;
     dead_wave_counts(lanes.order.data(), lanes.nQuietSlots, b->nTracked, [&](uint32_t u) { return c.utt[u].flags; }, KLATT_DEAD_TERMS, b->planDeadWaves);
+    dead2_wave_counts(lanes.order.data(), lanes.nQuietSlots, b->nTracked, [&](uint32_t u) { return c.utt[u].flags; }, [&](uint32_t u) { return c.present2[u]; },
+                      KLATT_DEAD_TERMS, b->planDead2Waves);
     b->nJobs = lanes.nTrackedUtt > 0 ? (long long)c.plan.jobs.size() : 0; b->trackEntries = lanes.nTrackedUtt > 0 ? (long long)c.plan.entries : 0;
     b->nDirect = c.nDirectUtt > 0 ? lanes.nDirectSlots : 0; b->nDirectUtt = c.nDirectUtt; b->nDirectFrames = (long long)c.scratch.directJobs.size();
     b->directAligned = c.nDirectUtt > 0 && c.directAligned;
@@ -3401,14 +3418,17 @@
         info[19] = 0;
     }
     if (nInfo >= 23) {
-        uint32_t dead[3] = {0u, 0u, 0u};
+        constexpr int kAll = 3 + kDead2Counts;
+        uint32_t dead[kAll] = {};
         if (b->launched && nTr > 0 && b->dDeadWaves.ptr) {
             HIP_TRY(hipStreamSynchronize(b->stream));
             HIP_TRY(hipMemcpy(dead, b->dDeadWaves.ptr, sizeof dead, hipMemcpyDeviceToHost));
         } else if (nTr > 0 && b->deadTerms) {
             for (int k = 0; k < 3; ++k) dead[k] = (uint32_t)std::min<long long>(b->planDeadWaves[k], 0x7FFFFFFFll);
-        }
-        for (int k = 0; k < 3; ++k) info[20 + k] = (int)std::min<uint32_t>(dead[k], 0x7FFFFFFFu);
+            for (int k = 0; k < kDead2Counts; ++k) dead[3 + k] = (uint32_t)std::min<long long>(b->planDead2Waves[k], 0x7FFFFFFFll);
+        }
+        const int n = nInfo >= 20 + kAll ? kAll : 3;
+        for (int k = 0; k < n; ++k) info[20 + k] = (int)std::min<uint32_t>(dead[k], 0x7FFFFFFFu);
     }
     return 0;
 }
@@ -3511,7 +3531,7 @@
     constexpr uint32_t kRouting = FACT_NOISE | FACT_NONFINITE | FACT_NASAL | FACT_UNBOUNDED;
     if (!onDevice) {
         parallel_ranges(nFrames, 1 << 13, [&](long long a, long long e) {
-            for (long long k = a; k < e; ++k) { out[k] = frame_facts(reinterpret_cast<const double*>(frames + k), maxF, maxBw); out[k].flags &= kRouting; }
+            for (long long k = a; k < e; ++k) { out[k] = frame_facts(reinterpret_cast<const double*>(frames + k), maxF, maxBw); out[k].flags &= kRouting; out[k].present2 = 0u; }
         });
         return nFrames;
     }
@@ -3525,7 +3545,7 @@
     hipLaunchKernelGGL(klatt_frame_facts, dim3(grid), dim3(256), 0, nullptr, dF.ptr, dO.ptr, nFrames, maxF, maxBw);
     HIP_TRY(hipGetLastError());
     HIP_TRY(hipMemcpy(out, dO.ptr, (size_t)nFrames * sizeof(FrameFacts), hipMemcpyDeviceToHost));
-    for (long long k = 0; k < nFrames; ++k) out[k].flags &= kRouting;
+    for (long long k = 0; k < nFrames; ++k) { out[k].flags &= kRouting; out[k].present2 = 0u; }
     return nFrames;
 }
 
diff --git a/nvspeechplayer_amd/csrc/klatt_plan.h b/nvspeechplayer_amd/csrc/klatt_plan.h
--- a/nvspeechplayer_amd/csrc/klatt_plan.h
+++ b/nvspeechplayer_amd/csrc/klatt_plan.h
@@ -14,7 +14,7 @@
 struct FrameFacts {
     unsigned long long h0, h1;
     uint32_t flags;
-    uint32_t pad;
+    uint32_t present2;
 };
 
 KLATT_LAYOUT_HD inline bool fact_finite(double v)
@@ -76,6 +76,18 @@
     if (!inRange) fl |= 8u;
     return fl;
 }
+KLATT_LAYOUT_HD inline uint32_t shape_present2(const double* p)
+{
+    uint32_t fl = !(fact_abs(p[6]) <= 1e30) ? UTT2_NASAL : 0u;
+    const bool bounded = (fact_abs(p[24]) <= 1e30) && (fact_abs(p[44]) <= 1e30);
+    for (int k = 2; k <= 6; ++k) {
+        const double pf = p[24 + k], pb = p[30 + k], pa = p[36 + k];
+        if (pa != 0.0 || !(pb >= 1.0) || !(pb <= 1e6) || !(fact_abs(pf) <= 1e6) || !bounded) fl |= 1u << (k - 2);
+    }
+    return fl;
+}
+KLATT_LAYOUT_HD inline uint32_t present2_of(uint32_t flags, uint32_t shapePresent2) { return shapePresent2 | ((flags & FACT_NASAL) ? UTT2_NASAL : 0u); }
+
 KLATT_LAYOUT_HD inline bool shape_values_equal(const double* a, const double* c)
 {
     bool same = true;
@@ -104,7 +116,7 @@
     }
     x ^= x >> 32; x *= 0xD6E8FEB86659FD93ull; x ^= x >> 32;
     y ^= y >> 31; y *= 0xBF58476D1CE4E5B9ull; y ^= y >> 29;
-    o.h0 = x; o.h1 = y; o.flags = fl; o.pad = 0;
+    o.h0 = x; o.h1 = y; o.flags = fl; o.present2 = present2_of(fl, shape_present2(p));
     return o;
 }
 
diff --git a/nvspeechplayer_amd/csrc/klatt_systolic.h b/nvspeechplayer_amd/csrc/klatt_systolic.h
--- a/nvspeechplayer_amd/csrc/klatt_systolic.h
+++ b/nvspeechplayer_amd/csrc/klatt_systolic.h
@@ -32,7 +32,7 @@
 #endif
 constexpr int kStages = 4;
 #ifndef KLATT_DEAD_TERMS
-#define KLATT_DEAD_TERMS 3
+#define KLATT_DEAD_TERMS 123
 #endif
 #ifndef KLATT_FLAT_SOURCE
 #define KLATT_FLAT_SOURCE 1
@@ -822,7 +822,11 @@
         if constexpr (FD::SKIP != 0u) {
 #pragma unroll
             for (int k = 0; k < kTrackEntries; ++k)
-                if (((FD::SKIP >> k) & 1u) && k < GE[e] && (e == 0 || k > GE[e - 1])) { const bool mv = (p.mask >> k) & 1u; moving += mv ? 1u : 0u; still += mv ? 0u : 1u; }
+                if (((FD::SKIP >> k) & 1u) && k < GE[e] && (e == 0 || k > GE[e - 1])) {
+                    const bool mv = (p.mask >> k) & 1u;
+                    const uint32_t ws = k == 0 ? 2u : 1u;
+                    moving += mv ? ws : 0u; still += mv ? 0u : ws;
+                }
         }
         const bool moves = (p.mask >> GE[e]) & 1u;
         f.idx[e] = (part + (moves ? hdr + moving : still)) * 16u;
@@ -1079,20 +1083,32 @@
         for (uint32_t bit = UTT_TURBULENCE; bit <= UTT_PARALLEL1; bit <<= 1) deadSet |= __any((mine & bit) != 0u) ? 0u : bit;
         deadSet = (uint32_t)__builtin_amdgcn_readfirstlane((int)(deadSet & A.deadTerms));
     }
+    uint32_t deadSet2 = 0;
+    if (FLAT && A.deadTerms2 != 0u) {
+        const uint32_t mine2 = live ? A.present2[u] : 0u;
+#pragma unroll
+        for (uint32_t bit = UTT2_PARALLEL2; bit <= UTT2_NASAL; bit <<= 1) deadSet2 |= __any((mine2 & bit) != 0u) ? 0u : bit;
+        deadSet2 = (uint32_t)__builtin_amdgcn_readfirstlane((int)(deadSet2 & A.deadTerms2));
+    }
+    (void)deadSet2;
 
     auto make_sync = [&](auto, auto, auto, int, int, int) __attribute__((always_inline)) { return BarrierSync{}; };
     using I0 = std::integral_constant<int, 0>; using I1 = std::integral_constant<int, 1>; using I2 = std::integral_constant<int, 2>;
     if (FLAT && KLATT_FLAT_SOURCE && stage == 0) {
         if constexpr (FLAT) {
-            auto sourceStage = [&](auto deadTag) __attribute__((always_inline)) {
+            auto sourceStage = [&](auto deadTag, auto noNasalTag) __attribute__((always_inline)) {
             constexpr int DEAD = decltype(deadTag)::value;
             constexpr bool NOTURB = DEAD >= 1;
+            constexpr bool NONASAL = decltype(noNasalTag)::value;
+            (void)NONASAL;
 #if KLATT_FLAT_LAYOUT == 2
-            using FD = FlatDesc<0, 2, NOTURB ? 4 : 5, true, 0, 0, double, NOTURB ? (1u << 21) : 0u>;
-            constexpr int GE[7] = {0, 1, 14, 20, NOTURB ? 22 : 21, NOTURB ? 23 : 22, 23};
-            constexpr int CB = 2;
-            constexpr uint32_t kUsualS0 = NOTURB ? 0x37u : 0x67u, kAllS0 = NOTURB ? 0x3Fu : 0x7Fu, kVibBit = 8u;
-            constexpr bool kHead = true;
+            constexpr bool kHead = !NONASAL;
+            constexpr uint32_t kSkipS0 = (NOTURB ? (1u << 21) : 0u) | (kHead ? 0u : 0x4003u);
+            using FD = FlatDesc<0, kHead ? 2 : 0, NOTURB ? (kHead ? 4 : 3) : (kHead ? 5 : 4), kHead, 0, 0, double, kSkipS0>;
+            constexpr int GE[7] = {kHead ? 0 : 20, kHead ? 1 : (NOTURB ? 22 : 21), kHead ? 14 : (NOTURB ? 23 : 22), kHead ? 20 : 23, NOTURB ? 22 : 21, NOTURB ? 23 : 22, 23};
+            constexpr int CB = kHead ? 2 : 0;
+            constexpr uint32_t kUsualS0 = kHead ? (NOTURB ? 0x37u : 0x67u) : (NOTURB ? 0x6u : 0xCu), kAllS0 = kHead ? (NOTURB ? 0x3Fu : 0x7Fu) : (NOTURB ? 0x7u : 0xFu);
+            constexpr uint32_t kVibBit = kHead ? 8u : 1u;
 #else
             using FD = FlatDesc<0, 0, NOTURB ? 3 : 4, false, 0, 0, double, NOTURB ? (1u << 21) : 0u>;
             constexpr int GE[4] = {20, NOTURB ? 22 : 21, NOTURB ? 23 : 22, 23};
@@ -1104,6 +1120,7 @@
             if (A.deadWaves && lane == 0) {
                 if (DEAD >= 1) atomicAdd(A.deadWaves + 1, 1u);
                 if (DEAD >= 2) atomicAdd(A.deadWaves + 2, 1u);
+                if (NONASAL) atomicAdd(A.deadWaves + 3, 1u);
             }
             bool staleNP = false;
             FlatState2<FD> f;
@@ -1188,7 +1205,7 @@
                         run = run < room ? run : room;
                         run = run < 1u ? 1u : run;
                         int cc = c;
-                        if (kHead && staleNP) { f.ra[1] = 1.0 - f.rb[1] - f.rc[1]; staleNP = false; }
+                        if constexpr (kHead) { if (staleNP) { f.ra[1] = 1.0 - f.rb[1] - f.rc[1]; staleNP = false; } }
                         for (uint32_t q = 0; q < run; ++q) {
                             if (f.live) {
 #pragma unroll
@@ -1273,9 +1290,10 @@
                 A.result[u] = res;
             }
             };
-            if ((KLATT_DEAD_TERMS & 4) && (deadSet & (UTT_TURBULENCE | UTT_ASPIRATION)) == (UTT_TURBULENCE | UTT_ASPIRATION)) sourceStage(std::integral_constant<int, 2>{});
-            else if ((KLATT_DEAD_TERMS & 2) && (deadSet & UTT_TURBULENCE)) sourceStage(std::integral_constant<int, 1>{});
-            else sourceStage(std::integral_constant<int, 0>{});
+            if ((KLATT_DEAD_TERMS & 8) && KLATT_FLAT_LAYOUT == 2 && (deadSet & UTT_TURBULENCE) && (deadSet2 & UTT2_NASAL)) sourceStage(std::integral_constant<int, 1>{}, std::true_type{});
+            else if ((KLATT_DEAD_TERMS & 4) && (deadSet & (UTT_TURBULENCE | UTT_ASPIRATION)) == (UTT_TURBULENCE | UTT_ASPIRATION)) sourceStage(std::integral_constant<int, 2>{}, std::false_type{});
+            else if ((KLATT_DEAD_TERMS & 2) && (deadSet & UTT_TURBULENCE)) sourceStage(std::integral_constant<int, 1>{}, std::false_type{});
+            else sourceStage(std::integral_constant<int, 0>{}, std::false_type{});
         }
     } else if (stage == 0) {
         constexpr bool NP0 = (SPLIT >> 2) != 0;
@@ -1457,23 +1475,36 @@
         }
     } else if (FLAT && stage == 3) {
         if constexpr (FLAT) {
-            auto parallel = [&](auto noP1Tag) __attribute__((always_inline)) {
-            constexpr bool NOP1 = decltype(noP1Tag)::value;
-            constexpr int NR = NOP1 ? 3 : 4;
-            using FD = FlatDesc<3, NR, 3, false, NOP1 ? 0x3Bu : 0x77u, 0, sig_t, NOP1 ? (1u << 8) : 0u>;
-            constexpr int GE[7] = {NOP1 ? 9 : 8, NOP1 ? 10 : 9, NOP1 ? 11 : 10, NOP1 ? 17 : 11, NOP1 ? 18 : 17, NOP1 ? 19 : 18, 19};
+            auto parallel = [&](auto noP1Tag, auto noneTag) __attribute__((always_inline)) {
+            constexpr bool NONE = decltype(noneTag)::value;
+            constexpr bool NOP1 = decltype(noP1Tag)::value || NONE;
+            constexpr int NR = NONE ? 0 : (NOP1 ? 3 : 4);
+            using FD = FlatDesc<3, NR, NONE ? 1 : 3, false, NONE ? 0u : (NOP1 ? 0x3Bu : 0x77u), 0, sig_t, NONE ? 0xC0F00u : (NOP1 ? (1u << 8) : 0u)>;
+            constexpr int GE[7] = {NONE ? 17 : (NOP1 ? 9 : 8), NOP1 ? 10 : 9, NOP1 ? 11 : 10, NOP1 ? 17 : 11, NOP1 ? 18 : 17, NOP1 ? 19 : 18, 19};
             FlatState2<FD> f;
             flat2_init<FD>(f, live, d, X, GE);
-            if (NOP1 && A.deadWaves && lane == 0) atomicAdd(A.deadWaves + 0, 1u);
+            if (A.deadWaves && lane == 0) {
+                if (NOP1) atomicAdd(A.deadWaves + 0, 1u);
+                if (NONE) atomicAdd(A.deadWaves + 6, 1u);
+            }
             sig_t fricNoise = 0;
             uint32_t noiseSt = noise_step(noise_first(nkey, ninc), ninc);
             flat2_loop<FD, CH>(1, nIter, nChunks, stage, f, X, GE,
                 [&](int c, int i, auto setTag, const auto& mid) __attribute__((always_inline)) {
                     constexpr uint32_t SET = decltype(setTag)::value;
+                    if constexpr (NONE) {
+                        fricNoise = (sig_t)noise_uniform(noiseSt) + (sig_t)0.75 * fricNoise;
+                        noiseSt = noise_step2(noiseSt, ninc2);
+                        const sig_t fric = fricNoise * (sig_t)0.3 * f.cur[0];
+                        const sig_t y = (fric * f.cur[1]) * (sig_t)0.5;
+                        mid(y);
+                        PIPE(pipeA, c, i) = y; PIPE(pipeB, c, i) = (sig_t)0;
+                    } else {
+                    constexpr int R1 = NR > 1 ? 1 : 0, R2 = NR > 2 ? 2 : 0;
                     const ResPre<sig_t> q0 = res_pre<MODE, ((SET >> 0) & 1u) != 0u>(f.ra[0], f.rb[0], f.rc[0], f.z1[0], f.z2[0]);
-                    const ResPre<sig_t> q1 = res_pre<MODE, ((SET >> 1) & 1u) != 0u>(f.ra[1], f.rb[1], f.rc[1], f.z1[1], f.z2[1]);
-                    const ResPre<sig_t> q2 = res_pre<MODE, ((SET >> 2) & 1u) != 0u>(f.ra[2], f.rb[2], f.rc[2], f.z1[2], f.z2[2]);
-                    constexpr int R3 = NR - 1;
+                    const ResPre<sig_t> q1 = res_pre<MODE, ((SET >> 1) & 1u) != 0u>(f.ra[R1], f.rb[R1], f.rc[R1], f.z1[R1], f.z2[R1]);
+                    const ResPre<sig_t> q2 = res_pre<MODE, ((SET >> 2) & 1u) != 0u>(f.ra[R2], f.rb[R2], f.rc[R2], f.z1[R2], f.z2[R2]);
+                    constexpr int R3 = NR > 0 ? NR - 1 : 0;
                     ResPre<sig_t> q3{};
                     if constexpr (!NOP1) q3 = res_pre<MODE, ((SET >> 3) & 1u) != 0u>(f.ra[R3], f.rb[R3], f.rc[R3], f.z1[R3], f.z2[R3]);
                     fricNoise = (sig_t)noise_uniform(noiseSt) + (sig_t)0.75 * fricNoise;
@@ -1485,9 +1516,9 @@
                         mid(q0, q1, q2, y, pa2, pa3, pa4);
                         sig_t w = res_post<MODE>(q0, y, f.z1[0], f.z2[0]);
                         sig_t par = (w - y) * pa2;
-                        w = res_post<MODE>(q1, y, f.z1[1], f.z2[1]);
+                        w = res_post<MODE>(q1, y, f.z1[R1], f.z2[R1]);
                         par += (w - y) * pa3;
-                        w = res_post<MODE>(q2, y, f.z1[2], f.z2[2]);
+                        w = res_post<MODE>(q2, y, f.z1[R2], f.z2[R2]);
                         par += (w - y) * pa4;
                         PIPE(pipeA, c, i) = y; PIPE(pipeB, c, i) = par;
                     } else {
@@ -1495,32 +1526,43 @@
                         sig_t par = 0;
                         sig_t w = res_post<MODE>(q0, y, f.z1[0], f.z2[0]);
                         par += (w - y) * pa1;
-                        w = res_post<MODE>(q1, y, f.z1[1], f.z2[1]);
+                        w = res_post<MODE>(q1, y, f.z1[R1], f.z2[R1]);
                         par += (w - y) * pa2;
-                        w = res_post<MODE>(q2, y, f.z1[2], f.z2[2]);
+                        w = res_post<MODE>(q2, y, f.z1[R2], f.z2[R2]);
                         par += (w - y) * pa3;
                         w = res_post<MODE>(q3, y, f.z1[R3], f.z2[R3]);
                         par += (w - y) * pa4;
                         PIPE(pipeA, c, i) = y; PIPE(pipeB, c, i) = par;
                     }
+                    }
                 },
                 noChunk, make_sync(std::integral_constant<int, L::kBufs>{}, I0{}, I1{}, 0, 0, 4));
             };
-            if ((KLATT_DEAD_TERMS & 1) && (deadSet & UTT_PARALLEL1)) parallel(std::true_type{}); else parallel(std::false_type{});
+            if ((KLATT_DEAD_TERMS & 64) && (deadSet & UTT_PARALLEL1) && (deadSet2 & kUtt2Parallel234) == kUtt2Parallel234) parallel(std::true_type{}, std::true_type{});
+            else if ((KLATT_DEAD_TERMS & 1) && (deadSet & UTT_PARALLEL1)) parallel(std::true_type{}, std::false_type{});
+            else parallel(std::false_type{}, std::false_type{});
         }
     } else if (FLAT && (KLATT_FLAT_EXHAUSTIVE || stage == 2)) {
         if constexpr (FLAT) {
+            auto finalStage = [&](auto goneTag) __attribute__((always_inline)) {
+            constexpr int GONE = decltype(goneTag)::value;
 #if KLATT_FLAT_LAYOUT == 2
-            constexpr int GE[4] = {12, 13, 15, 16};
-            using FD = FlatDesc<2, 2, 2, false, 0xEu>;
+            constexpr int GE[4] = {GONE == 2 ? 16 : (GONE == 1 ? 13 : 12), GONE == 1 ? 15 : 13, GONE == 1 ? 16 : 15, 16};
+            using FD = FlatDesc<2, 2 - GONE, GONE == 2 ? 1 : 2, false, GONE == 0 ? 0xEu : 0u, 0, sig_t,
+                                GONE == 2 ? ((1u << 12) | (1u << 13) | (1u << 15)) : (GONE == 1 ? (1u << 12) : 0u)>;
             constexpr int RS = 0;
 #else
+            static_assert(GONE == 0, "the final stage's lightened bodies: layout 2");
             constexpr int GE[6] = {6, 7, 12, 13, 15, 16};
             using FD = FlatDesc<2, 4, 2, false, 0x3Bu>;
             constexpr int RS = 2;
 #endif
             FlatState2<FD> f;
             flat2_init<FD>(f, live, d, X, GE);
+            if (A.deadWaves && lane == 0) {
+                if (GONE >= 1) atomicAdd(A.deadWaves + 4, 1u);
+                if (GONE >= 2) atomicAdd(A.deadWaves + 5, 1u);
+            }
             int16_t* const myRow = reinterpret_cast<int16_t*>(tile + lane * kTileStride);
             uint32_t it = 0;
             auto flush_tile = [&](uint32_t tileStart, uint32_t validTo) __attribute__((always_inline)) {
@@ -1554,23 +1596,32 @@
             flat2_loop<FD, CH>(2, nIter, nChunks, stage, f, X, GE,
                 [&](int c, int i, auto setTag, const auto& mid) __attribute__((always_inline)) {
                     constexpr uint32_t SET = decltype(setTag)::value;
-                    constexpr int NR = 2 + RS;
+                    constexpr int NR = 2 - GONE + RS;
+                    constexpr int G0 = GONE == 2 ? 0 : 2;
                     ResPre<sig_t> q[4];
 #pragma unroll
                     for (int r = 0; r < NR; ++r) q[r] = ((SET >> r) & 1u) ? res_pre<MODE, true>(f.ra[r], f.rb[r], f.rc[r], f.z1[r], f.z2[r])
                                                                           : res_pre<MODE, false>(f.ra[r], f.rb[r], f.rc[r], f.z1[r], f.z2[r]);
-                    const sig_t pa5 = f.cur[0], pa6 = f.cur[1], bypass = f.cur[2], outGain = f.cur[3];
-                    if constexpr (RS == 2) mid(q[0], q[1], q[2], q[3], pa5, pa6, bypass, outGain);
+                    const sig_t pa5 = f.cur[0], pa6 = f.cur[GONE == 2 ? 0 : 1], bypass = f.cur[G0], outGain = f.cur[G0 + 1];
+                    (void)pa5; (void)pa6;
+                    if constexpr (GONE == 2) mid(bypass, outGain);
+                    else if constexpr (GONE == 1) mid(q[0], pa6, bypass, outGain);
+                    else if constexpr (RS == 2) mid(q[0], q[1], q[2], q[3], pa5, pa6, bypass, outGain);
                     else mid(q[0], q[1], pa5, pa6, bypass, outGain);
                     sig_t o = PIPE(pipeO, c, i);
                     const sig_t y = PIPE(pipeA, c, i);
 #pragma unroll
                     for (int r = 0; r < RS; ++r) o = res_post<MODE>(q[r], o, f.z1[r], f.z2[r]);
                     sig_t par = PIPE(pipeB, c, i);
-                    sig_t w = res_post<MODE>(q[RS], y, f.z1[RS], f.z2[RS]);
-                    par += (w - y) * pa5;
-                    w = res_post<MODE>(q[RS + 1], y, f.z1[RS + 1], f.z2[RS + 1]);
-                    par += (w - y) * pa6;
+                    if constexpr (GONE == 0) {
+                        const sig_t w = res_post<MODE>(q[RS], y, f.z1[RS], f.z2[RS]);
+                        par += (w - y) * pa5;
+                    }
+                    if constexpr (GONE <= 1) {
+                        constexpr int R6 = RS + 1 - GONE;
+                        const sig_t w = res_post<MODE>(q[R6], y, f.z1[R6], f.z2[R6]);
+                        par += (w - y) * pa6;
+                    }
                     par = fade_value(par, y, bypass);
                     const sig_t mix = o + par;
                     const sig_t v = (mix * outGain) * (sig_t)4000.0;
@@ -1581,6 +1632,11 @@
                 [&]() __attribute__((always_inline)) { it += kChunk; if ((it % kTile) == 0) flush_tile(it - kTile, it); },
                 make_sync(std::integral_constant<int, L::kBufs>{}, I2{}, I0{}, 2, 4, 0));
             if ((it % kTile) != 0) flush_tile(it - (it % kTile), it);
+            };
+            constexpr bool kLight = KLATT_FLAT_LAYOUT == 2;
+            if (kLight && (KLATT_DEAD_TERMS & 32) && (deadSet2 & (UTT2_PARALLEL5 | UTT2_PARALLEL6)) == (UTT2_PARALLEL5 | UTT2_PARALLEL6)) finalStage(std::integral_constant<int, kLight ? 2 : 0>{});
+            else if (kLight && (KLATT_DEAD_TERMS & 16) && (deadSet2 & UTT2_PARALLEL5)) finalStage(std::integral_constant<int, kLight ? 1 : 0>{});
+            else finalStage(std::integral_constant<int, 0>{});
         }
     } else if (!NOISE && !NASAL && (stage == 1 || stage == 2)) {
         using D = StageDesc<6, 3, -1, false, false>;
diff --git a/nvspeechplayer_amd/speechPlayer.py b/nvspeechplayer_amd/speechPlayer.py
--- a/nvspeechplayer_amd/speechPlayer.py
+++ b/nvspeechplayer_amd/speechPlayer.py
@@ -2013,9 +2013,11 @@
         return ms
 
     def kernelInfo(self):
-        info = np.zeros(23, dtype=np.int32)
+        info = np.zeros(27, dtype=np.int32)
         self._check(self._dll.speechPlayer_batch_kernelInfo(self._h, info.ctypes.data, len(info)))
         dead = dict(waves_without_parallel1=int(info[20]), waves_without_turbulence=int(info[21]), waves_without_aspiration=int(info[22]))
+        dead.update(stages_without_nasal=int(info[23]), stages_without_parallel5=int(info[24]), stages_without_parallel56=int(info[25]),
+                    stages_without_parallel1to4=int(info[26]))
         return dict(vgprs=int(info[0]), lds_bytes=int(info[1]), wavefronts=int(info[2]), cus=int(info[3]),
                     workgroups_per_cu_by_lds=int(info[4]), scratch_bytes=int(info[5]),
                     stage_parallel_chunk=int(info[6]), noisy_group=bool(info[7]),
```

New measurement: 200.8 billion, median of 6. +5.7%, better.
